# globc/mrAudio

Hardware: AMD Instinct MI355X
Metric: clips/s encode+fuse+score, 32-clip x 32-frame synthetic (higher is better)
Workload: dtype f16

## Files before the change

include/mra.h:

```cpp
#ifndef MRA_H_
#define MRA_H_

#include <stddef.h>
#include <stdint.h>

#ifdef __cplusplus
extern "C" {
#endif

#define MRA_OK 0
#define MRA_EINVAL (-1)
#define MRA_ESTATE (-2)
#define MRA_EHIP (-3)
#define MRA_ENOMEM (-4)
#define MRA_ENAME (-5)

#define MRA_F32 0
#define MRA_F16 1
#define MRA_BF16 2

typedef struct mra_qformer mra_qformer;

typedef struct mra_cfg {
  int32_t hidden;
// ... 112 lines not shown
typedef struct mra_vit_cfg {
  int32_t dim;
  int32_t heads;
  int32_t mlp;
  int32_t depth;
  int32_t patch;
  int32_t img;
  float ln_eps;
  int32_t op_dtype;
  int32_t residual_dtype;
} mra_vit_cfg;
void mra_vit_cfg_default(mra_vit_cfg* cfg);
int mra_vit_create(const mra_vit_cfg* cfg, mra_vit** out);
void mra_vit_destroy(mra_vit* h);
int mra_vit_load(mra_vit* h, const char* name, const void* src, int32_t dtype, const int64_t* shape, int32_t ndim, void* stream);
int mra_vit_missing(mra_vit* h);
size_t mra_vit_workspace_bytes(mra_vit* h, int32_t frames);
int mra_vit_forward(mra_vit* h, const void* frames, int32_t dtype, int32_t n, void* out, void* workspace, size_t workspace_bytes,
                    void* stream);
double mra_vit_flops(mra_vit* h, int32_t frames);
int mra_vit_set_option(mra_vit* h, const char* name, int32_t value);

#define MRA_BEATS_GATE_Q 0
#define MRA_BEATS_GATE_INPUT 1
typedef struct mra_beats mra_beats;
typedef struct mra_beats_cfg {
  int32_t dim;
  int32_t heads;
  int32_t ffn;
  int32_t layers;
  int32_t embed_dim;
  int32_t patch;
  int32_t mel_bins;
  int32_t conv_pos;
  int32_t conv_pos_groups;
  int32_t num_buckets;
  int32_t max_distance;
  float ln_eps;
  float deep_norm_alpha;
  int32_t gate_from;
  int32_t op_dtype;
} mra_beats_cfg;
void mra_beats_cfg_default(mra_beats_cfg* cfg);
int mra_beats_create(const mra_beats_cfg* cfg, mra_beats** out);
void mra_beats_destroy(mra_beats* h);
int mra_beats_load(mra_beats* h, const char* name, const void* src, int32_t dtype, const int64_t* shape, int32_t ndim, void* stream);
int mra_beats_missing(mra_beats* h);
size_t mra_beats_workspace_bytes(mra_beats* h, int32_t n, int32_t frames);
int mra_beats_forward(mra_beats* h, const void* fbank, int32_t dtype, int32_t n, int32_t frames, void* out, void* workspace,
                      size_t workspace_bytes, void* stream);
double mra_beats_flops(mra_beats* h, int32_t n, int32_t frames);
int mra_beats_set_option(mra_beats* h, const char* name, int32_t value);

typedef struct mra_fbank mra_fbank;
int mra_fbank_create(mra_fbank** out);
void mra_fbank_destroy(mra_fbank* h);
int mra_fbank_forward(mra_fbank* h, const float* wave, int64_t total_samples, const int64_t* segs, int32_t n_seg, int32_t frame_length,
                      void* out, int32_t out_dtype, void* stream);
double mra_fbank_flops(mra_fbank* h, int32_t n_seg, int32_t frame_length);

int64_t mra_debug_gemm_launches(int32_t family, int32_t epilogue);

int mra_debug_vit_attention(mra_vit* h, const void* qkv, int32_t n, void* ctx, void* stream);
size_t mra_debug_shared_kv_workspace_bytes(int32_t enc_items, int32_t prompts, int32_t heads, int32_t kv, int32_t core);
int mra_debug_shared_kv_attention(const void* q, const void* k, const void* v, int32_t dtype, int32_t enc_items, int32_t prompts,
                                  int32_t heads, int32_t kv, int32_t core, void* ctx, void* workspace, size_t workspace_bytes, void* stream);
int mra_debug_beats_attention(mra_beats* h, int32_t layer, const void* qkv, const void* gate_src, int32_t n, int32_t tokens, void* ctx,
                              void* stream);
int mra_debug_beats_posconv(mra_beats* h, float* x, int32_t n, int32_t tokens, void* stream);
int mra_debug_attention_bwd(const void* q, const void* k, const void* v, const void* o, const void* d_o, const float* lse, int32_t dtype,
                            int32_t kv_items, int32_t share, int32_t heads, int32_t q_rows, int32_t kv, void* dq, void* dk, void* dv, void* stream);

int mra_debug_self_attention(const void* qkv, const int64_t* mask, int32_t dtype, int32_t items, int32_t S, int32_t heads, void* ctx, float* lse,
                             void* stream);
int mra_debug_ln_rows(const float* x, const int64_t* x_view, int32_t rows, int32_t H, const float* const* params, int32_t lane_rows, int32_t period,
                      int32_t split, float eps, float* y32, const int64_t* y32_view, void* y16, const int64_t* y16_view, int32_t dtype, void* stream);
int mra_debug_embed_ln(const int64_t* ids, int32_t items, int32_t L, int32_t Q, int32_t H, int32_t vocab, const float* query, int64_t query_item_stride,
                       const float* word, const float* pos, const float* gain, const float* bias, float eps, float* h32, void* h16, float* pre32,
                       int32_t dtype, void* stream);
int mra_debug_modality_ln(const void* x, int32_t x_dtype, const int64_t* item_index, int32_t items, int32_t tokens, int32_t E, const float* gain,
                          const float* bias, float eps, void* out, int32_t dtype, void* stream);
int mra_debug_softmax_rows(const float* S, int64_t ld_s, void* P, int64_t ld_p, int32_t rows, int32_t kv, int32_t kvp, float scale, int32_t dtype,
                           void* stream);
int mra_debug_fold_rowfactor(const float* stat_m, const float* stat_l, float* factors, int32_t rows, int32_t R, int32_t ntiles, void* P, int64_t ld_p,
                             int32_t tile_cols, int32_t kvp, int32_t* hist, void* stream);
int mra_debug_softmax_rescale(void* P, int64_t ld_p, const float* stat_m, const float* stat_l, int32_t rows, int32_t ntiles, int32_t tile_cols,
                              int32_t kvp, int32_t dtype, int32_t* hist, void* stream);
int mra_debug_transpose_pad(const void* src, void* dst, int32_t R, int32_t C, int32_t ld_d, int64_t src_bs, int64_t dst_bs, int32_t batch, int32_t dtype,
                            void* stream);
int mra_debug_split(int32_t kind, const float* src, const int64_t* src_view, int32_t rows, int32_t C, int32_t chunk, int32_t parts, void* dst,
                    int32_t dtype, void* stream);

int mra_debug_gemm_tn_group(int32_t njobs, const void* const* dY, const int64_t* y_views, const int64_t* y_block_stride, const void* const* X,
                            const int64_t* x_views, const int64_t* x_block_stride, float* const* dW, float* const* db, const int32_t* M,
                            const int32_t* N, const int32_t* K, const int32_t* ldw, const int32_t* accumulate, int32_t dtype, void* stream);
int mra_debug_ln_bwd(const void* const* ptrs_a, const int64_t* views_a, int32_t rows_a, float eps_a, const void* const* ptrs_b, const int64_t* views_b,
                     int32_t rows_b, float eps_b, int32_t H, int32_t dtype, void* stream);
int mra_debug_embed_bwd(const float* demb, const int64_t* ids, int32_t items, int32_t L, int32_t Q, int32_t H, int32_t vocab, float* dquery, float* dpos,
                        float* dword, void* stream);
size_t mra_debug_transpose16_batch_scratch_bytes(int32_t njobs);
int mra_debug_transpose16_batch(const void* const* src, void* const* dst, const int32_t* R, const int32_t* C, int32_t njobs, int32_t dtype, void* scratch,
                                size_t scratch_bytes, void* stream);
int mra_debug_gemm_gelu(int32_t nprob, const void* const* A, const int64_t* a_views, const void* const* W, const float* const* bias, void* const* C,
                        const int64_t* c_views, void* const* aux, const int32_t* M, const int32_t* N, const int32_t* K, int32_t backward, int32_t tile_cfg,
                        int32_t dtype, void* stream);

typedef struct mra_gemm_desc {
  uint64_t struct_bytes;
  const void* A; const void* W; const float* bias; void* C; const float* R;
  int64_t a_view[3], c_view[3], r_view[3];
  int32_t M, N, K;
  int32_t kv_tokens, kv_items, kv_heads;
  int32_t batch, bias_bs;
  int64_t a_bs, w_bs, c_bs_bytes;
  int32_t n_ragged, w_ld, k_rows, w_kwrap;
  const float* ln_gain; const float* ln_bias; float* ln_y32; void* ln_y16; uint32_t* ln_counter;
  int64_t ln_y32_view[3], ln_y16_view[3];
  float ln_eps, alpha;
  float* stat_m; float* stat_l; const float* pscale;
  int32_t ps_ntiles, tile_cfg, persist, reserved;
  uint64_t a_bytes, w_bytes, bias_bytes, c_bytes, r_bytes, ln_gain_bytes, ln_bias_bytes, ln_y32_bytes, ln_y16_bytes, ln_counter_bytes, stat_m_bytes,
      stat_l_bytes, pscale_bytes;
  float* col_scale; int64_t cs_bs; int32_t col_stats; float cs_eps;
  uint64_t col_scale_bytes;
  void* aux; uint64_t aux_bytes;
} mra_gemm_desc;
int mra_debug_gemm(const mra_gemm_desc* probs, int32_t nprob, int32_t epilogue, int32_t dtype, void* stream);
int mra_debug_gemm_plan(const mra_gemm_desc* probs, int32_t nprob, int32_t epilogue, int32_t dtype, int32_t cus, int32_t* out);

int mra_debug_vit_fold_weight(const void* W, size_t w_bytes, const float* gain, size_t gain_bytes, const float* beta, size_t beta_bytes, const float* bias,
                              size_t bias_bytes, void* Wf, size_t wf_bytes, float* cs, size_t cs_bytes, float* bf, size_t bf_bytes, int32_t N, int32_t K,
                              int32_t dtype, void* stream);
int mra_debug_vit_group_stats(const float* groups, size_t groups_bytes, int64_t M, int32_t G, int32_t group_cols, float eps, float* stats,
                              size_t stats_bytes, void* stream);
int mra_debug_vit_row_stats(const void* x, size_t x_bytes, int32_t x_dtype, int64_t M, int32_t D, float eps, float* stats, size_t stats_bytes, void* x16,
                            size_t x16_bytes, int32_t dtype, void* stream);

#ifdef __cplusplus
}
#endif
#endif
```

mraudio_amd/_lib.py:

```python
from __future__ import annotations

import ctypes as C
import os

import torch

MRA_F32, MRA_F16, MRA_BF16 = 0, 1, 2
_ERR = {-1: "MRA_EINVAL", -2: "MRA_ESTATE", -3: "MRA_EHIP", -4: "MRA_ENOMEM", -5: "MRA_ENAME"}

LIB_NAME = "libmra_hip.so"
LIB_PATH = os.path.join(os.path.dirname(os.path.abspath(__file__)), LIB_NAME)


class mra_cfg(C.Structure):
    _fields_ = [
        ("hidden", C.c_int32), ("heads", C.c_int32), ("inter", C.c_int32), ("layers", C.c_int32),
        ("cross_freq", C.c_int32), ("enc_width", C.c_int32), ("n_query", C.c_int32), ("vocab", C.c_int32),
        ("max_pos", C.c_int32), ("ln_eps", C.c_float), ("enc_ln_eps", C.c_float), ("llm_hidden", C.c_int32),
        ("op_dtype", C.c_int32),
    ]


class mra_vit_cfg(C.Structure):
    _fields_ = [("dim", C.c_int32), ("heads", C.c_int32), ("mlp", C.c_int32), ("depth", C.c_int32), ("patch", C.c_int32),
                ("img", C.c_int32), ("ln_eps", C.c_float), ("op_dtype", C.c_int32), ("residual_dtype", C.c_int32)]


MRA_BEATS_GATE_Q, MRA_BEATS_GATE_INPUT = 0, 1


class mra_beats_cfg(C.Structure):
    _fields_ = [("dim", C.c_int32), ("heads", C.c_int32), ("ffn", C.c_int32), ("layers", C.c_int32), ("embed_dim", C.c_int32),
                ("patch", C.c_int32), ("mel_bins", C.c_int32), ("conv_pos", C.c_int32), ("conv_pos_groups", C.c_int32),
                ("num_buckets", C.c_int32), ("max_distance", C.c_int32), ("ln_eps", C.c_float), ("deep_norm_alpha", C.c_float),
                ("gate_from", C.c_int32), ("op_dtype", C.c_int32)]


class mra_gemm_desc(C.Structure):
    _fields_ = [
        ("struct_bytes", C.c_uint64),
        ("A", C.c_void_p), ("W", C.c_void_p), ("bias", C.c_void_p), ("C", C.c_void_p), ("R", C.c_void_p),
        ("a_view", C.c_int64 * 3), ("c_view", C.c_int64 * 3), ("r_view", C.c_int64 * 3),
        ("M", C.c_int32), ("N", C.c_int32), ("K", C.c_int32),
        ("kv_tokens", C.c_int32), ("kv_items", C.c_int32), ("kv_heads", C.c_int32),
        ("batch", C.c_int32), ("bias_bs", C.c_int32),
        ("a_bs", C.c_int64), ("w_bs", C.c_int64), ("c_bs_bytes", C.c_int64),
        ("n_ragged", C.c_int32), ("w_ld", C.c_int32), ("k_rows", C.c_int32), ("w_kwrap", C.c_int32),
        ("ln_gain", C.c_void_p), ("ln_bias", C.c_void_p), ("ln_y32", C.c_void_p), ("ln_y16", C.c_void_p), ("ln_counter", C.c_void_p),
        ("ln_y32_view", C.c_int64 * 3), ("ln_y16_view", C.c_int64 * 3),
        ("ln_eps", C.c_float), ("alpha", C.c_float),
        ("stat_m", C.c_void_p), ("stat_l", C.c_void_p), ("pscale", C.c_void_p),
        ("ps_ntiles", C.c_int32), ("tile_cfg", C.c_int32), ("persist", C.c_int32), ("reserved", C.c_int32),
        ("a_bytes", C.c_uint64), ("w_bytes", C.c_uint64), ("bias_bytes", C.c_uint64), ("c_bytes", C.c_uint64), ("r_bytes", C.c_uint64),
        ("ln_gain_bytes", C.c_uint64), ("ln_bias_bytes", C.c_uint64), ("ln_y32_bytes", C.c_uint64), ("ln_y16_bytes", C.c_uint64),
        ("ln_counter_bytes", C.c_uint64), ("stat_m_bytes", C.c_uint64), ("stat_l_bytes", C.c_uint64), ("pscale_bytes", C.c_uint64),
        ("col_scale", C.c_void_p), ("cs_bs", C.c_int64), ("col_stats", C.c_int32), ("cs_eps", C.c_float),
        ("col_scale_bytes", C.c_uint64),
        ("aux", C.c_void_p), ("aux_bytes", C.c_uint64),
    ]


PROTOTYPES = {
    "mra_cfg_default": (None, [C.POINTER(mra_cfg), C.c_int32]),
    "mra_last_error": (C.c_char_p, []),
    "mra_version": (C.c_char_p, []),
    "mra_qformer_create": (C.c_int, [C.POINTER(mra_cfg), C.POINTER(C.c_void_p)]),
    "mra_qformer_destroy": (None, [C.c_void_p]),
    "mra_qformer_load": (C.c_int, [C.c_void_p, C.c_char_p, C.c_void_p, C.c_int32, C.POINTER(C.c_int64), C.c_int32,
                                   C.c_void_p]),
    "mra_qformer_missing": (C.c_int, [C.c_void_p, C.c_char_p, C.c_size_t]),
    "mra_modality_ln": (C.c_int, [C.c_void_p, C.c_void_p, C.c_int32, C.c_void_p, C.c_int32, C.c_int32, C.c_void_p,
                                  C.c_void_p]),
    "mra_qformer_workspace_bytes": (C.c_size_t, [C.c_void_p, C.c_int32, C.c_int32, C.c_int32]),
    "mra_qformer_forward": (C.c_int, [C.c_void_p, C.c_void_p, C.c_void_p, C.c_void_p, C.c_int32, C.c_void_p, C.c_int32,
                                      C.c_int32, C.c_int32, C.c_void_p, C.c_void_p, C.c_void_p, C.c_void_p, C.c_size_t,
                                      C.c_void_p]),
    "mra_qformer_raw_features_ok": (C.c_int, [C.c_void_p, C.c_int32, C.c_int32]),
    "mra_qformer_forward_raw": (C.c_int, [C.c_void_p, C.c_void_p, C.c_void_p, C.c_void_p, C.c_int32, C.c_void_p, C.c_int32,
                                          C.c_int32, C.c_int32, C.c_void_p, C.c_void_p, C.c_void_p, C.c_void_p, C.c_size_t,
                                          C.c_void_p]),
    "mra_qformer_pair_workspace_bytes": (C.c_size_t, [C.c_void_p, C.c_void_p, C.c_int32, C.c_int32, C.c_int32, C.c_int32]),
    "mra_qformer_forward_pair": (C.c_int, [C.c_void_p, C.c_void_p, C.c_void_p, C.c_void_p, C.c_void_p, C.c_void_p, C.c_int32, C.c_int32, C.c_int32, C.c_int32,
                                           C.c_void_p, C.c_void_p, C.c_void_p, C.c_void_p, C.c_void_p, C.c_size_t, C.c_void_p]),
    "mra_qformer_forward_pair_raw": (C.c_int, [C.c_void_p, C.c_void_p, C.c_void_p, C.c_void_p, C.c_void_p, C.c_void_p, C.c_int32, C.c_int32, C.c_int32, C.c_int32,
                                               C.c_int32, C.c_void_p, C.c_void_p, C.c_void_p, C.c_void_p, C.c_void_p, C.c_size_t, C.c_void_p]),
    "mra_qformer_multi_workspace_bytes": (C.c_size_t, [C.c_void_p, C.c_int32, C.c_int32, C.c_int32, C.c_int32]),
    "mra_qformer_forward_multi": (C.c_int, [C.c_void_p, C.c_void_p, C.c_void_p, C.c_void_p, C.c_int32, C.c_int32, C.c_int32, C.c_int32,
                                            C.c_void_p, C.c_void_p, C.c_void_p, C.c_size_t, C.c_void_p]),
    "mra_qformer_set_kv_events": (C.c_int, [C.c_void_p, C.c_void_p, C.c_void_p]),
    "mra_qformer_set_kv_done_event": (C.c_int, [C.c_void_p, C.c_void_p]),
    "mra_qformer_set_cross_mode": (C.c_int, [C.c_void_p, C.c_int32]),
    "mra_qformer_set_cross_precision": (C.c_int, [C.c_void_p, C.c_int32]),
    "mra_qformer_cross_precision_report": (C.c_int, [C.c_void_p, C.POINTER(C.c_int32), C.POINTER(C.c_int32), C.POINTER(C.c_float), C.c_int32]),
    "mra_qformer_set_option": (C.c_int, [C.c_void_p, C.c_char_p, C.c_int32]),
    "mra_qformer_prepare": (C.c_int, [C.c_void_p, C.c_void_p]),
    "mra_kv_cache_bytes": (C.c_size_t, [C.c_void_p, C.c_int32, C.c_int32]),
    "mra_kv_project": (C.c_int, [C.c_void_p, C.c_void_p, C.c_int32, C.c_int32, C.c_void_p, C.c_void_p]),
    "mra_llm_proj": (C.c_int, [C.c_void_p, C.c_void_p, C.c_int32, C.c_void_p, C.c_int32, C.c_void_p, C.c_size_t,
                               C.c_void_p]),
    "mra_cosine_score": (C.c_int, [C.c_void_p, C.c_void_p, C.c_int32, C.c_int32, C.c_int32, C.c_int32, C.c_void_p,
                                   C.c_void_p, C.c_void_p]),
    "mra_fuse_logits": (C.c_int, [C.POINTER(C.c_void_p), C.POINTER(C.c_float), C.c_int32, C.c_int32, C.c_void_p,
                                  C.c_void_p]),
    "mra_span_from_logits": (C.c_int, [C.c_void_p, C.c_int32, C.c_int32, C.c_float, C.c_void_p, C.c_void_p]),
    "mra_windows_from_logits": (C.c_int, [C.c_void_p, C.c_int32, C.c_int32, C.c_float, C.c_int32, C.c_float, C.c_int32, C.c_void_p,
                                          C.c_void_p, C.c_void_p, C.c_void_p]),
    "mra_qformer_grad_bytes": (C.c_size_t, [C.c_void_p]),
    "mra_qformer_load_flat": (C.c_int32, [C.c_void_p, C.c_void_p, C.c_size_t, C.c_void_p]),
    "mra_qformer_grad_offset": (C.c_int, [C.c_void_p, C.c_char_p, C.POINTER(C.c_size_t), C.POINTER(C.c_int64)]),
    "mra_qformer_enable_training": (C.c_int, [C.c_void_p, C.c_void_p]),
    "mra_qformer_adam_step": (C.c_int, [C.c_void_p, C.c_void_p, C.c_void_p, C.c_void_p, C.c_void_p, C.c_size_t, C.c_float, C.c_float, C.c_float,
                                        C.c_float, C.c_float, C.c_int32, C.c_int32, C.c_void_p]),
    "mra_qformer_train_workspace_bytes": (C.c_size_t, [C.c_void_p, C.c_int32, C.c_int32, C.c_int32]),
    "mra_qformer_forward_train": (C.c_int, [C.c_void_p, C.c_void_p, C.c_void_p, C.c_void_p, C.c_int32, C.c_int32, C.c_int32,
                                            C.c_void_p, C.c_void_p, C.c_void_p, C.c_size_t, C.c_void_p]),
    "mra_qformer_backward": (C.c_int, [C.c_void_p, C.c_void_p, C.c_void_p, C.c_void_p, C.c_int32, C.c_int32, C.c_int32,
                                       C.c_void_p, C.c_void_p, C.c_void_p, C.c_void_p, C.c_size_t, C.c_void_p]),
    "mra_qformer_multi_train_workspace_bytes": (C.c_size_t, [C.c_void_p, C.c_int32, C.c_int32, C.c_int32, C.c_int32]),
    "mra_qformer_forward_multi_train": (C.c_int, [C.c_void_p, C.c_void_p, C.c_void_p, C.c_void_p, C.c_int32, C.c_int32, C.c_int32, C.c_int32,
                                                  C.c_void_p, C.c_void_p, C.c_void_p, C.c_size_t, C.c_void_p]),
    "mra_qformer_backward_multi": (C.c_int, [C.c_void_p, C.c_void_p, C.c_void_p, C.c_void_p, C.c_int32, C.c_int32, C.c_int32, C.c_int32,
                                             C.c_void_p, C.c_void_p, C.c_void_p, C.c_void_p, C.c_size_t, C.c_void_p]),
    "mra_qformer_backward_enc": (C.c_int, [C.c_void_p, C.c_int32, C.c_int32, C.c_int32, C.c_int32, C.c_void_p, C.c_size_t, C.c_void_p, C.c_void_p]),
    "mra_modality_ln_backward": (C.c_int, [C.c_void_p, C.c_void_p, C.c_int32, C.c_int32, C.c_int32, C.c_void_p, C.c_void_p, C.c_void_p, C.c_void_p,
                                           C.c_void_p]),
    "mra_debug_kvgrad_gemm": (C.c_int, [C.c_void_p, C.c_void_p, C.c_size_t, C.c_int32, C.c_int32, C.c_void_p, C.c_size_t, C.c_void_p]),
    "mra_qformer_flops": (C.c_double, [C.c_void_p, C.c_int32, C.c_int32, C.c_int32, C.c_int32]),
    "mra_vit_cfg_default": (None, [C.POINTER(mra_vit_cfg)]),
    "mra_vit_create": (C.c_int, [C.POINTER(mra_vit_cfg), C.POINTER(C.c_void_p)]),
    "mra_vit_destroy": (None, [C.c_void_p]),
    "mra_vit_load": (C.c_int, [C.c_void_p, C.c_char_p, C.c_void_p, C.c_int32, C.POINTER(C.c_int64), C.c_int32, C.c_void_p]),
    "mra_vit_missing": (C.c_int, [C.c_void_p]),
    "mra_vit_workspace_bytes": (C.c_size_t, [C.c_void_p, C.c_int32]),
    "mra_vit_forward": (C.c_int, [C.c_void_p, C.c_void_p, C.c_int32, C.c_int32, C.c_void_p, C.c_void_p, C.c_size_t, C.c_void_p]),
    "mra_vit_flops": (C.c_double, [C.c_void_p, C.c_int32]),
    "mra_vit_set_option": (C.c_int, [C.c_void_p, C.c_char_p, C.c_int32]),
    "mra_beats_cfg_default": (None, [C.POINTER(mra_beats_cfg)]),
    "mra_beats_create": (C.c_int, [C.POINTER(mra_beats_cfg), C.POINTER(C.c_void_p)]),
    "mra_beats_destroy": (None, [C.c_void_p]),
    "mra_beats_load": (C.c_int, [C.c_void_p, C.c_char_p, C.c_void_p, C.c_int32, C.POINTER(C.c_int64), C.c_int32, C.c_void_p]),
    "mra_beats_missing": (C.c_int, [C.c_void_p]),
    "mra_beats_workspace_bytes": (C.c_size_t, [C.c_void_p, C.c_int32, C.c_int32]),
    "mra_beats_forward": (C.c_int, [C.c_void_p, C.c_void_p, C.c_int32, C.c_int32, C.c_int32, C.c_void_p, C.c_void_p, C.c_size_t, C.c_void_p]),
    "mra_beats_flops": (C.c_double, [C.c_void_p, C.c_int32, C.c_int32]),
    "mra_beats_set_option": (C.c_int, [C.c_void_p, C.c_char_p, C.c_int32]),
    "mra_fbank_create": (C.c_int, [C.POINTER(C.c_void_p)]),
    "mra_fbank_destroy": (None, [C.c_void_p]),
    "mra_fbank_forward": (C.c_int, [C.c_void_p, C.c_void_p, C.c_int64, C.c_void_p, C.c_int32, C.c_int32, C.c_void_p, C.c_int32, C.c_void_p]),
    "mra_fbank_flops": (C.c_double, [C.c_void_p, C.c_int32, C.c_int32]),
    "mra_debug_gemm_launches": (C.c_int64, [C.c_int32, C.c_int32]),
    "mra_debug_vit_attention": (C.c_int, [C.c_void_p, C.c_void_p, C.c_int32, C.c_void_p, C.c_void_p]),
    "mra_debug_shared_kv_workspace_bytes": (C.c_size_t, [C.c_int32, C.c_int32, C.c_int32, C.c_int32, C.c_int32]),
    "mra_debug_shared_kv_attention": (C.c_int, [C.c_void_p, C.c_void_p, C.c_void_p, C.c_int32, C.c_int32, C.c_int32, C.c_int32, C.c_int32, C.c_int32,
                                                C.c_void_p, C.c_void_p, C.c_size_t, C.c_void_p]),
    "mra_debug_attention_bwd": (C.c_int, [C.c_void_p, C.c_void_p, C.c_void_p, C.c_void_p, C.c_void_p, C.c_void_p, C.c_int32, C.c_int32, C.c_int32,
                                          C.c_int32, C.c_int32, C.c_int32, C.c_void_p, C.c_void_p, C.c_void_p, C.c_void_p]),
    "mra_debug_beats_attention": (C.c_int, [C.c_void_p, C.c_int32, C.c_void_p, C.c_void_p, C.c_int32, C.c_int32, C.c_void_p, C.c_void_p]),
    "mra_debug_beats_posconv": (C.c_int, [C.c_void_p, C.c_void_p, C.c_int32, C.c_int32, C.c_void_p]),
    "mra_debug_self_attention": (C.c_int, [C.c_void_p, C.c_void_p, C.c_int32, C.c_int32, C.c_int32, C.c_int32, C.c_void_p, C.c_void_p, C.c_void_p]),
    "mra_debug_ln_rows": (C.c_int, [C.c_void_p, C.POINTER(C.c_int64), C.c_int32, C.c_int32, C.POINTER(C.c_void_p), C.c_int32, C.c_int32, C.c_int32,
                                    C.c_float, C.c_void_p, C.POINTER(C.c_int64), C.c_void_p, C.POINTER(C.c_int64), C.c_int32, C.c_void_p]),
    "mra_debug_embed_ln": (C.c_int, [C.c_void_p, C.c_int32, C.c_int32, C.c_int32, C.c_int32, C.c_int32, C.c_void_p, C.c_int64, C.c_void_p, C.c_void_p,
                                     C.c_void_p, C.c_void_p, C.c_float, C.c_void_p, C.c_void_p, C.c_void_p, C.c_int32, C.c_void_p]),
    "mra_debug_modality_ln": (C.c_int, [C.c_void_p, C.c_int32, C.c_void_p, C.c_int32, C.c_int32, C.c_int32, C.c_void_p, C.c_void_p, C.c_float,
                                        C.c_void_p, C.c_int32, C.c_void_p]),
    "mra_debug_softmax_rows": (C.c_int, [C.c_void_p, C.c_int64, C.c_void_p, C.c_int64, C.c_int32, C.c_int32, C.c_int32, C.c_float, C.c_int32,
                                         C.c_void_p]),
    "mra_debug_fold_rowfactor": (C.c_int, [C.c_void_p, C.c_void_p, C.c_void_p, C.c_int32, C.c_int32, C.c_int32, C.c_void_p, C.c_int64, C.c_int32,
                                           C.c_int32, C.c_void_p, C.c_void_p]),
    "mra_debug_softmax_rescale": (C.c_int, [C.c_void_p, C.c_int64, C.c_void_p, C.c_void_p, C.c_int32, C.c_int32, C.c_int32, C.c_int32, C.c_int32,
                                            C.c_void_p, C.c_void_p]),
    "mra_debug_transpose_pad": (C.c_int, [C.c_void_p, C.c_void_p, C.c_int32, C.c_int32, C.c_int32, C.c_int64, C.c_int64, C.c_int32, C.c_int32,
                                          C.c_void_p]),
    "mra_debug_split": (C.c_int, [C.c_int32, C.c_void_p, C.POINTER(C.c_int64), C.c_int32, C.c_int32, C.c_int32, C.c_int32, C.c_void_p, C.c_int32,
                                  C.c_void_p]),
    "mra_debug_gemm_tn_group": (C.c_int, [C.c_int32, C.POINTER(C.c_void_p), C.POINTER(C.c_int64), C.POINTER(C.c_int64), C.POINTER(C.c_void_p),
                                          C.POINTER(C.c_int64), C.POINTER(C.c_int64), C.POINTER(C.c_void_p), C.POINTER(C.c_void_p), C.POINTER(C.c_int32),
                                          C.POINTER(C.c_int32), C.POINTER(C.c_int32), C.POINTER(C.c_int32), C.POINTER(C.c_int32), C.c_int32, C.c_void_p]),
    "mra_debug_ln_bwd": (C.c_int, [C.POINTER(C.c_void_p), C.POINTER(C.c_int64), C.c_int32, C.c_float, C.POINTER(C.c_void_p), C.POINTER(C.c_int64),
                                   C.c_int32, C.c_float, C.c_int32, C.c_int32, C.c_void_p]),
    "mra_debug_embed_bwd": (C.c_int, [C.c_void_p, C.c_void_p, C.c_int32, C.c_int32, C.c_int32, C.c_int32, C.c_int32, C.c_void_p, C.c_void_p, C.c_void_p,
                                      C.c_void_p]),
    "mra_debug_transpose16_batch_scratch_bytes": (C.c_size_t, [C.c_int32]),
    "mra_debug_transpose16_batch": (C.c_int, [C.POINTER(C.c_void_p), C.POINTER(C.c_void_p), C.POINTER(C.c_int32), C.POINTER(C.c_int32), C.c_int32,
                                              C.c_int32, C.c_void_p, C.c_size_t, C.c_void_p]),
    "mra_debug_gemm_gelu": (C.c_int, [C.c_int32, C.POINTER(C.c_void_p), C.POINTER(C.c_int64), C.POINTER(C.c_void_p), C.POINTER(C.c_void_p),
                                      C.POINTER(C.c_void_p), C.POINTER(C.c_int64), C.POINTER(C.c_void_p), C.POINTER(C.c_int32), C.POINTER(C.c_int32),
                                      C.POINTER(C.c_int32), C.c_int32, C.c_int32, C.c_int32, C.c_void_p]),
    "mra_debug_gemm": (C.c_int, [C.POINTER(mra_gemm_desc), C.c_int32, C.c_int32, C.c_int32, C.c_void_p]),
    "mra_debug_gemm_plan": (C.c_int, [C.POINTER(mra_gemm_desc), C.c_int32, C.c_int32, C.c_int32, C.c_int32, C.POINTER(C.c_int32)]),
    "mra_debug_vit_fold_weight": (C.c_int, [C.c_void_p, C.c_size_t, C.c_void_p, C.c_size_t, C.c_void_p, C.c_size_t, C.c_void_p, C.c_size_t, C.c_void_p,
                                            C.c_size_t, C.c_void_p, C.c_size_t, C.c_void_p, C.c_size_t, C.c_int32, C.c_int32, C.c_int32, C.c_void_p]),
    "mra_debug_vit_group_stats": (C.c_int, [C.c_void_p, C.c_size_t, C.c_int64, C.c_int32, C.c_int32, C.c_float, C.c_void_p, C.c_size_t, C.c_void_p]),
    "mra_debug_vit_row_stats": (C.c_int, [C.c_void_p, C.c_size_t, C.c_int32, C.c_int64, C.c_int32, C.c_float, C.c_void_p, C.c_size_t, C.c_void_p,
                                          C.c_size_t, C.c_int32, C.c_void_p]),
}

GF_V1_64, GF_V1_128, GF_WS_256, GF_P8_256, GF_WS_128x384, GF_WS_176x384, GF_K128_64x128, GF_P8_TAIL, GF_P8_MIXED, GF_K128_64x64 = 0, 1, 3, 4, 5, 6, 7, 8, 9, 10
GF_RING_144x128, GF_RING_192x128, GF_RING_96x64 = 11, 12, 13
GEMM_FAMILIES = 14
EPI_OP, EPI_GELU_OP, EPI_RES_F32, EPI_F32, EPI_KV, EPI_SOFTPART, EPI_RES_OP = 0, 1, 2, 3, 4, 5, 8
EPI_RES_F32_STAT, EPI_LNF_OP, EPI_LNF_GELU_OP, EPI_RES_OP_STAT = 10, 11, 12, 13
EPI_GELU_BOTH, EPI_GELU_BWD = 6, 7
EPI_RES_LN = 9
GT_AUTO, GT_64, GT_128, GT_256 = 0, 1, 2, 3
GT_WS_128x384, GT_WS_176x384, GT_K128_64x128, GT_P8_TAIL, GT_P8_MIXED = 4, 5, 6, 7, 8
GT_RING_144x128, GT_RING_192x128, GT_RING_96x64 = 9, 10, 11
GEMM_TN_MAX_JOBS = 4


def gemm_launches(family: int, epi: int) -> int:
    return int(lib().mra_debug_gemm_launches(family, epi))

_lib = None


class MraError(RuntimeError):
    pass


def lib() -> C.CDLL:
    global _lib
    if _lib is None:
        if not os.path.exists(LIB_PATH):
            raise MraError(
                f"{LIB_PATH} is missing: build the HIP extension first "
                "(python -c 'import __graft_entry__ as g; g.build()' or make -C mraudio_amd/csrc). "
                "mraudio_amd has no CPU fallback."
            )
        handle = C.CDLL(LIB_PATH)
        for name, (res, args) in PROTOTYPES.items():
            fn = getattr(handle, name)
            fn.restype = res
            fn.argtypes = args
        _lib = handle
    return _lib


def check(rc: int, what: str) -> None:
    if rc != 0:
        msg = lib().mra_last_error().decode("utf-8", "replace")
        raise MraError(f"{what}: {_ERR.get(rc, rc)}: {msg}")


def ptr(t) -> C.c_void_p:
    return C.c_void_p(0 if t is None else t.data_ptr())


def current_stream() -> C.c_void_p:
    return C.c_void_p(torch.cuda.current_stream().cuda_stream)
# ... 15 lines not shown
```

mraudio_amd/csrc/fold.hip:

```cpp
#include "kernels.h"
#include "mra_common.h"

namespace mra {

namespace {

constexpr float LOG2E_F = 1.4426950408889634f;

template <typename T, int NV>
__global__ void __launch_bounds__(256) softmax_rows_kernel(const float* S, long long ld_s, T* P, long long ld_p, int kv, int kvp,
                                                           float sl2) {
  __shared__ float red[8];
  const int tid = threadIdx.x, lane = tid & 63, wave = tid >> 6;
  const float* s = S + (long long)blockIdx.x * ld_s;
  T* p = P + (long long)blockIdx.x * ld_p;
  constexpr int NR = NV > 0 ? NV : 1;
  f32x4 v[NR];
  float m = -3.0e38f;
  if constexpr (NV > 0) {
#pragma unroll
    for (int j = 0; j < NV; ++j) {
      const int c = 4 * (tid + j * 256);
      if (c + 3 < kv) {
        v[j] = *reinterpret_cast<const f32x4*>(s + c);
      } else {
#pragma unroll
        for (int e = 0; e < 4; ++e) v[j][e] = c + e < kv ? s[c + e] : -3.0e38f;
      }
      m = fmaxf(fmaxf(m, fmaxf(v[j][0], v[j][1])), fmaxf(v[j][2], v[j][3]));
    }
  } else {
    for (int i = tid; i < kv; i += 256) m = fmaxf(m, s[i]);
  }
  m = wave_max(m);
  if (lane == 0) red[wave] = m;
  __syncthreads();
  m = fmaxf(fmaxf(red[0], red[1]), fmaxf(red[2], red[3])) * sl2;
  float l = 0.f;
  if constexpr (NV > 0) {
#pragma unroll
    for (int j = 0; j < NV; ++j)
#pragma unroll
      for (int e = 0; e < 4; ++e) {
        v[j][e] = __builtin_amdgcn_exp2f(v[j][e] * sl2 - m);
        l += v[j][e];
      }
  } else {
    for (int i = tid; i < kv; i += 256) l += __builtin_amdgcn_exp2f(s[i] * sl2 - m);
  }
  l = wave_sum(l);
  if (lane == 0) red[4 + wave] = l;
  __syncthreads();
  const float inv = 1.0f / ((red[4] + red[5]) + (red[6] + red[7]));
  if constexpr (NV > 0) {
#pragma unroll
    for (int j = 0; j < NV; ++j) {
      const int c = 4 * (tid + j * 256);
      if (c < kvp) {
        typename Vec4<T>::type o;
#pragma unroll
        for (int e = 0; e < 4; ++e) o[e] = from_f32<T>(v[j][e] * inv);
        *reinterpret_cast<typename Vec4<T>::type*>(p + c) = o;
      }
    }
  } else {
    for (int i = tid; i < kvp; i += 256) p[i] = from_f32<T>(i < kv ? __builtin_amdgcn_exp2f(s[i] * sl2 - m) * inv : 0.f);
  }
}

template <typename T, bool PROBE>
__global__ void __launch_bounds__(256) softmax_rescale_kernel(T* P, long long ld_p, const float* stat_m, const float* stat_l, int ntiles,
                                                              int tile_cols, int kvp, int* hist) {
  __shared__ float g[128];
  const int tid = threadIdx.x;
  const float* sm = stat_m + (long long)blockIdx.x * ntiles;
  const float* sl = stat_l + (long long)blockIdx.x * ntiles;
  if (tid < 64) {
    float m = -3.0e38f;
    for (int t = tid; t < ntiles; t += 64) m = fmaxf(m, sm[t]);
    m = wave_max(m);
    float l = 0.f;
    for (int t = tid; t < ntiles; t += 64) l += __builtin_amdgcn_exp2f(sm[t] - m) * sl[t];
// ... 23 lines not shown
    *reinterpret_cast<V8*>(p + 8 * c) = v;
  }
}

template <bool PROBE>
__global__ void __launch_bounds__(256) fold_rowfactor_kernel(const float* stat_m, const float* stat_l, float* factors, int rows, int R, int ntiles,
                                                             unsigned short* P, long long ld_p, int tile_cols, int kvp, int* hist) {
  const int row = blockIdx.x * 4 + (threadIdx.x >> 6), lane = threadIdx.x & 63;
  __shared__ int bins[PROBE ? 256 : 1];
  if constexpr (PROBE) {
    bins[threadIdx.x] = 0;
    __syncthreads();
  }
  if (row < rows) {
    for (int c = ntiles * tile_cols + lane; c < kvp; c += 64) P[(long long)row * ld_p + c] = 0;
    const float* sm = stat_m + (long long)row * ntiles;
    const float* sl = stat_l + (long long)row * ntiles;
    float m = -3.0e38f;
    for (int t = lane; t < ntiles; t += 64) m = fmaxf(m, sm[t]);
    m = wave_max(m);
    float l = 0.f;
    for (int t = lane; t < ntiles; t += 64) l += __builtin_amdgcn_exp2f(sm[t] - m) * sl[t];
    l = wave_sum(l);
    const float inv = 1.0f / l;
    const int item = row / R, r = row - item * R;
    for (int t = lane; t < ntiles; t += 64) factors[((long long)item * ntiles + t) * 512 + r] = __builtin_amdgcn_exp2f(sm[t] - m) * inv;
    if constexpr (PROBE) {
      if (lane == 0) atomicAdd(&bins[(int)fminf(fmaxf(inv * 256.f, 0.f), 255.f)], 1);
    }
  }
  if constexpr (PROBE) {
    __syncthreads();
    const int n = bins[threadIdx.x];
    if (n) atomicAdd(hist + threadIdx.x, n);
  }
}

template <typename T>
__global__ void __launch_bounds__(256) transpose_pad_kernel(const T* src, T* dst, int R, int C, int ld_d, long long src_bs,
                                                            long long dst_bs) {
  __shared__ T tile[32][33];
  src += (long long)blockIdx.z * src_bs;
  dst += (long long)blockIdx.z * dst_bs;
  const int bx = blockIdx.x * 32, by = blockIdx.y * 32;
  const int tx = threadIdx.x & 31, ty = threadIdx.x >> 5;
  for (int j = ty; j < 32; j += 8)
    tile[j][tx] = (by + j < R && bx + tx < C) ? src[(long long)(by + j) * C + bx + tx] : from_f32<T>(0.f);
  __syncthreads();
  for (int j = ty; j < 32; j += 8)
    if (bx + j < C && by + tx < ld_d) dst[(long long)(bx + j) * ld_d + by + tx] = tile[tx][j];
}

template <typename T>
__global__ void __launch_bounds__(256) transpose_pad64_kernel(const T* src, T* dst, int R, int C, int ld_d, long long src_bs,
                                                              long long dst_bs) {
  __shared__ T tile[64][72];
  src += (long long)blockIdx.z * src_bs;
  dst += (long long)blockIdx.z * dst_bs;
  const int bx = blockIdx.x * 64, by = blockIdx.y * 64;
  const int ch = (threadIdx.x & 7) * 8, r0 = threadIdx.x >> 3;
  using V8 = typename Vec8<T>::type;
#pragma unroll
  for (int i = 0; i < 2; ++i) {
    const int r = r0 + 32 * i;
    V8 v;
#pragma unroll
    for (int e = 0; e < 8; ++e) v[e] = from_f32<T>(0.f);
    if (by + r < R && bx + ch < C) v = *reinterpret_cast<const V8*>(src + (long long)(by + r) * C + bx + ch);
    *reinterpret_cast<V8*>(&tile[r][ch]) = v;
  }
  __syncthreads();
#pragma unroll
  for (int i = 0; i < 2; ++i) {
    const int c = r0 + 32 * i;
    if (bx + c < C && by + ch < ld_d) {
      V8 v;
#pragma unroll
      for (int e = 0; e < 8; ++e) v[e] = tile[ch + e][c];
      *reinterpret_cast<V8*>(dst + (long long)(bx + c) * ld_d + by + ch) = v;
    }
  }
}

}

int launch_softmax_rows(const float* S, long long ld_s, void* P, long long ld_p, int rows, int kv, int kvp, float scale, int op_dtype,
                        hipStream_t stream) {
  if (rows <= 0) return 0;
  if (kv <= 0 || kvp < kv || (kvp & 3) || (ld_s & 3) || (ld_p & 3) || ld_p < kvp || ld_s < kv) return -1;
  const float sl2 = scale * LOG2E_F;
  const int nv = (kvp + 1023) / 1024;
#define MRA_SM(T, NV) hipLaunchKernelGGL((softmax_rows_kernel<T, NV>), dim3(rows), dim3(256), 0, stream, S, ld_s, (T*)P, ld_p, kv, kvp, sl2)
#define MRA_SM_T(T)                                                                                   \
  do {                                                                                                \
    if (nv <= 1) MRA_SM(T, 1); else if (nv <= 2) MRA_SM(T, 2); else if (nv <= 4) MRA_SM(T, 4);          \
    else if (nv <= 9) MRA_SM(T, 9); else if (nv <= 16) MRA_SM(T, 16); else MRA_SM(T, 0);               \
  } while (0)
  if (op_dtype == OP_F16) MRA_SM_T(f16); else MRA_SM_T(bf16);
#undef MRA_SM_T
#undef MRA_SM
  return hipGetLastError() == hipSuccess ? 0 : -4;
}

int launch_fold_rowfactor(const float* stat_m, const float* stat_l, float* factors, int rows, int R, int ntiles, void* P, long long ld_p, int tile_cols,
                          int kvp, hipStream_t stream, int* hist) {
  if (rows <= 0) return 0;
  if (ntiles <= 0 || R <= 0 || R > 512 || rows % R || !P || ld_p < kvp || ntiles * tile_cols > kvp) return -1;
  if (hist)
    hipLaunchKernelGGL(fold_rowfactor_kernel<true>, dim3((rows + 3) / 4), dim3(256), 0, stream, stat_m, stat_l, factors, rows, R, ntiles,
                       (unsigned short*)P, ld_p, tile_cols, kvp, hist);
  else
    hipLaunchKernelGGL(fold_rowfactor_kernel<false>, dim3((rows + 3) / 4), dim3(256), 0, stream, stat_m, stat_l, factors, rows, R, ntiles,
                       (unsigned short*)P, ld_p, tile_cols, kvp, (int*)nullptr);
  return hipGetLastError() == hipSuccess ? 0 : -4;
}

int launch_softmax_rescale(void* P, long long ld_p, const float* stat_m, const float* stat_l, int rows, int ntiles, int tile_cols, int kvp,
                           int op_dtype, hipStream_t stream, int* hist) {
  if (rows <= 0) return 0;
  if (ntiles <= 0 || ntiles > 128 || (tile_cols & 7) || (kvp & 7) || (ld_p & 7) || ld_p < kvp) return -1;
#define MRA_RS(T, PR) hipLaunchKernelGGL((softmax_rescale_kernel<T, PR>), dim3(rows), dim3(256), 0, stream, (T*)P, ld_p, stat_m, stat_l, ntiles, tile_cols, kvp, hist)
  if (op_dtype == OP_F16) { if (hist) MRA_RS(f16, true); else MRA_RS(f16, false); }
  else { if (hist) MRA_RS(bf16, true); else MRA_RS(bf16, false); }
#undef MRA_RS
  return hipGetLastError() == hipSuccess ? 0 : -4;
}

int launch_transpose_pad(const void* src, void* dst, int R, int C, int ld_d, long long src_bs, long long dst_bs, int batch, int op_dtype,
                         hipStream_t stream) {
  if (batch <= 0 || R <= 0 || C <= 0) return 0;
  if (ld_d < R || batch > 65535) return -1;
  if (C % 8 == 0 && ld_d % 8 == 0 && C >= 64 && ld_d >= 64) {
    const dim3 grid64((C + 63) / 64, (ld_d + 63) / 64, batch);
    if (op_dtype == OP_F16) hipLaunchKernelGGL(transpose_pad64_kernel<f16>, grid64, dim3(256), 0, stream, (const f16*)src, (f16*)dst, R, C, ld_d, src_bs, dst_bs);
    else hipLaunchKernelGGL(transpose_pad64_kernel<bf16>, grid64, dim3(256), 0, stream, (const bf16*)src, (bf16*)dst, R, C, ld_d, src_bs, dst_bs);
    return hipGetLastError() == hipSuccess ? 0 : -4;
  }
  const dim3 grid((C + 31) / 32, (ld_d + 31) / 32, batch), block(256);
  if (op_dtype == OP_F16) hipLaunchKernelGGL(transpose_pad_kernel<f16>, grid, block, 0, stream, (const f16*)src, (f16*)dst, R, C, ld_d, src_bs, dst_bs);
  else hipLaunchKernelGGL(transpose_pad_kernel<bf16>, grid, block, 0, stream, (const bf16*)src, (bf16*)dst, R, C, ld_d, src_bs, dst_bs);
  return hipGetLastError() == hipSuccess ? 0 : -4;
}

namespace {
template <typename T, typename TW, bool KEY>
__global__ void __launch_bounds__(256) fold_ln_weight_kernel(const TW* W, int E, const float* gain, const float* ln_bias, const float* bias_in,
                                                             T* dst, float* bias_out) {
  __shared__ float red[8];
  const int tid = threadIdx.x, lane = tid & 63, wave = tid >> 6;
  const int n = blockIdx.x;
  const TW* w = W + (long long)n * E;
  float s = 0.f, sb = 0.f;
  for (int e = tid; e < E; e += 256) {
    const float we = (float)w[e];
    s += we * gain[e];
    sb = __builtin_fmaf(we, ln_bias[e], sb);
  }
  s = wave_sum(s);
  sb = wave_sum(sb);
  if (lane == 0) { red[wave] = s; red[4 + wave] = sb; }
  __syncthreads();
  const float mean = ((red[0] + red[1]) + (red[2] + red[3])) / (float)E;
  if (tid == 0 && bias_out) bias_out[n] = (bias_in ? bias_in[n] : 0.f) + ((red[4] + red[5]) + (red[6] + red[7]));
  for (int e = tid; e < E; e += 256) {
    const T o = from_f32<T>((float)w[e] * gain[e] - mean);
    if (KEY) dst[((long long)(n >> 6) * E + e) * 64 + (n & 63)] = o;
    else dst[(long long)n * E + e] = o;
  }
}
}

int launch_fold_ln_weight(const void* W, int w32, int rows, int E, const float* gain, const float* ln_bias, const float* bias_in, void* dst,
                          int key_layout, float* bias_out, int op_dtype, hipStream_t stream) {
  if (rows <= 0 || E <= 0 || !W || !gain || !ln_bias || !dst || (key_layout && rows % 64)) return -1;
#define MRA_FL(T, TW, KEY) hipLaunchKernelGGL((fold_ln_weight_kernel<T, TW, KEY>), dim3(rows), dim3(256), 0, stream, (const TW*)W, E, gain, ln_bias, bias_in, (T*)dst, bias_out)
#define MRA_FL_T(T)                                                          \
  do {                                                                       \
    if (w32) { if (key_layout) MRA_FL(T, float, true); else MRA_FL(T, float, false); } \
    else { if (key_layout) MRA_FL(T, T, true); else MRA_FL(T, T, false); }   \
  } while (0)
  if (op_dtype == OP_F16) MRA_FL_T(f16); else MRA_FL_T(bf16);
#undef MRA_FL_T
#undef MRA_FL
  return hipGetLastError() == hipSuccess ? 0 : -4;
}

}
```

mraudio_amd/csrc/gemm.hip:

```cpp
#include <atomic>
#include <cstdlib>
#include <initializer_list>
#include <mutex>
#include <set>
#include <type_traits>
#include <utility>

#include "kernels.h"
#include "mra_common.h"

namespace mra {

namespace {

__device__ __forceinline__ long long view_off(const RowView& v, int m) {
  int item = m / v.rpi;
  int r = m - item * v.rpi;
  return (long long)item * v.item_stride + (long long)r * v.ld;
}

template <int TN, int TM>
__device__ __forceinline__ GemmProb tile_of(const GemmArgs& args, int id, int& n0, int& m0);

template <int TN, int TM>
// ... 475 lines not shown
  constexpr int NT = WGN * WGM * 64;
  constexpr int WTN = TN / WGN, WTM = TM / WGM;
  constexpr int FN = WTN / 16, FM = WTM / 16;
  constexpr int IW = TN * 8 / NT, IX = TM * 8 / NT;
  static_assert(TN * 8 % NT == 0 && TM * 8 % NT == 0, "tile/threads mismatch");
  constexpr int BUF = (TN + TM) * ROWB;
  extern __shared__ __attribute__((aligned(16))) char smem[];
  const int tid = threadIdx.x;
  const int lane = tid & 63;
  const int wave = __builtin_amdgcn_readfirstlane(tid >> 6);
  const int wn0 = (wave / WGM) * WTN;
  const int wm0 = (wave % WGM) * WTM;
  int n0, m0;
  const GemmProb& P = pick_tile<TN, TM>(args, n0, m0);
  const int K = P.K, M = P.M;

  const char* srcW[IW];
  const char* srcX[IX];
#pragma unroll
  for (int i = 0; i < IW; ++i) {
    const int q = tid + i * NT;
    const int row = q >> 3, c = (q & 7) ^ ((row >> 1) & 7);
    srcW[i] = (const char*)P.W + ((long long)min(n0 + row, P.N - 1) * K + c * 8) * 2;
  }
#pragma unroll
  for (int i = 0; i < IX; ++i) {
    const int q = tid + i * NT;
    const int row = q >> 3, c = (q & 7) ^ ((row >> 1) & 7);
    const int m = min(m0 + row, M - 1);
    srcX[i] = (const char*)P.A + (view_off(P.a, m) + c * 8) * 2;
  }
  const int wave_q0 = wave * 64;
  auto stage = [&](int buf, int kt) {
    char* base = smem + buf * BUF;
    const long long koff = (long long)kt * ROWB;
#pragma unroll
    for (int i = 0; i < IW; ++i) glds16(srcW[i] + koff, base + (wave_q0 + i * NT) * 16);
#pragma unroll
    for (int i = 0; i < IX; ++i) glds16(srcX[i] + koff, base + TN * ROWB + (wave_q0 + i * NT) * 16);
  };
  int foff[2];
#pragma unroll
  for (int ks = 0; ks < 2; ++ks) {
    const int r = lane & 15;
    const int c = (4 * ks + (lane >> 4)) ^ ((r >> 1) & 7);
    foff[ks] = r * ROWB + c * 16;
  }
  f32x4 acc[FN][FM];
#pragma unroll
  for (int i = 0; i < FN; ++i)
#pragma unroll
    for (int j = 0; j < FM; ++j) acc[i][j] = f32x4{0.f, 0.f, 0.f, 0.f};

  const int nk = K / BK;
  stage(0, 0);
  for (int kt = 0; kt < nk; ++kt) {
    asm volatile("s_waitcnt vmcnt(0)" ::: "memory");
    __syncthreads();
    if (kt + 1 < nk) stage((kt + 1) & 1, kt + 1);
    const char* wb = smem + (kt & 1) * BUF + wn0 * ROWB;
    const char* xb = smem + (kt & 1) * BUF + TN * ROWB + wm0 * ROWB;
#pragma unroll
    for (int ks = 0; ks < 2; ++ks) {
      typename Vec8<T>::type a[FN], b[FM];
#pragma unroll
      for (int i = 0; i < FN; ++i) a[i] = lds_read8<T>(wb + i * 16 * ROWB + foff[ks]);
#pragma unroll
      for (int j = 0; j < FM; ++j) b[j] = lds_read8<T>(xb + j * 16 * ROWB + foff[ks]);
#pragma unroll
      for (int i = 0; i < FN; ++i)
#pragma unroll
        for (int j = 0; j < FM; ++j) acc[i][j] = mfma16<T>(a[i], b[j], acc[i][j]);
    }
  }
  if constexpr (EPI == EPI_OP || EPI == EPI_GELU_OP || EPI == EPI_KV || EPI == EPI_RES_OP) {
    __syncthreads();
    epilogue_lds16<T, TN, TM, FN, FM, NT, EPI, (FN * FM <= 16)>(P, acc, smem, n0, m0, wn0, wm0, tid);
  } else {
    if constexpr (FN * FM > 16) epilogue_lean<T, FN, FM, EPI>(P, acc, n0 + wn0, m0 + wm0, lane);
    else epilogue<T, FN, FM, EPI>(P, acc, n0 + wn0, m0 + wm0, lane);
  }
}

template <typename T, int EPI, bool NODMA = false, int TN = 256, int TM = 256, int WGM = 4, bool NTW = false, bool WKM = false, bool PSC = false, int CS = 0>
__global__ void __launch_bounds__(768) gemm_ws_kernel(const GemmArgs args) {
  constexpr int BK = 64, ROWB = BK * 2;
  constexpr int WGN = 8 / WGM, WTN = TN / WGN, WTM = TM / WGM, FN = WTN / 16, FM = WTM / 16;
  constexpr int BUF = (TN + TM) * ROWB;
  constexpr int PS_TILE = 176, GT_OFF = 2 * BUF, GT_SLICE = 2048;
  static_assert(!PSC || (TM <= 512 && PS_TILE % 8 == 0), "factor slices hold 512 rows; an 8-k fragment piece never straddles a tile");
  constexpr int NCHUNK = (TN + TM) * 8, NLD = (NCHUNK + 255) / 256;
  constexpr bool STAGED = (EPI == EPI_OP || EPI == EPI_GELU_OP || EPI == EPI_KV || EPI == EPI_RES_OP) && TN % 64 == 0;
  static_assert(WTN % 16 == 0 && WTM % 16 == 0 && TN % 16 == 0 && NCHUNK % 64 == 0, "tile must split over the waves; whole waves per DMA piece");
  static_assert(CS == 0 || (EPI == EPI_SOFTPART && !WKM && !PSC && TN * 4 <= BUF && TN <= 192), "column factors: the scores launch only; three per lane of one wave");
  constexpr int NWS = (TN * 8 + 255) / 256;
  extern __shared__ __attribute__((aligned(16))) char smem[];
  const int tid = threadIdx.x;
  const int lane = tid & 63;
  const int wave = __builtin_amdgcn_readfirstlane(tid >> 6);
  int n0, m0;
  const GemmProb& P = pick_tile<TN, TM>(args, n0, m0);
  const int K = P.K, M = P.M;
  const int nk = K / BK;

  if (wave >= 8) {
    const int lt = tid - 512;
    const char* src[NLD];
    int wrow[NLD];
#pragma unroll
    for (int i = 0; i < NLD; ++i) {
      const int q = min(lt + i * 256, NCHUNK - 1);
      const int row = q >> 3, c = (q & 7) ^ ((row >> 1) & 7);
      wrow[i] = 0;
      if (WKM && q < TN * 8) {
        wrow[i] = q / (TN / 8);
        src[i] = (const char*)P.W + ((long long)n0 + (q - wrow[i] * (TN / 8)) * 8) * 2;
      } else if (row < TN) {
        const long long ldw = P.w_kwrap > 0 ? (long long)P.w_kwrap * BK : K;
        src[i] = (const char*)P.W + ((long long)min(n0 + row, P.N - 1) * ldw + c * 8) * 2;
      } else {
        const int m = min(m0 + row - TN, M - 1);
        src[i] = (const char*)P.A + (view_off(P.a, m) + c * 8) * 2;
      }
    }
    const int wq0 = (wave - 8) * 64;
    const int kwrap = P.w_kwrap > 0 ? P.w_kwrap : 0x7fffffff;
    auto stage = [&](int buf, int kt) {
      char* base = smem + buf * BUF;
      const long long koff = (long long)kt * ROWB;
      const long long koffw = (long long)(kt >= kwrap ? kt - kwrap : kt) * ROWB;
#pragma unroll
      for (int i = 0; i < NLD; ++i)
        if (i * 256 + wq0 < NCHUNK) {
          if (WKM && i * 256 + wq0 < TN * 8) {
            const long long krow = min(kt * BK + wrow[i], P.k_rows - 1);
            glds16_nt(src[i] + krow * P.w_ld * 2, base + (wq0 + i * 256) * 16);
          } else if ((i * 256 + wq0) / 8 < TN) {
            if (NTW) glds16_nt(src[i] + koffw, base + (wq0 + i * 256) * 16);
            else glds16(src[i] + koffw, base + (wq0 + i * 256) * 16);
          } else {
            glds16(src[i] + koff, base + (wq0 + i * 256) * 16);
          }
        }
    };
    int gt_next = 0;
    auto stage_factors = [&](int kt) {
      if constexpr (PSC) {
        if (wave != 8) return;
        const int t_hi = (kt * BK + BK - 1) / PS_TILE;
        for (; gt_next <= t_hi; ++gt_next) {
          const char* sg = (const char*)(P.pscale + (long long)min(gt_next, P.ps_ntiles - 1) * 512) + lane * 16;
          char* dg = smem + GT_OFF + (gt_next & 3) * GT_SLICE;
          glds16(sg, dg);
          glds16(sg + 1024, dg + 1024);
        }
      }
    };
    float* const cscale = CS != 0 ? P.col_scale + (long long)(P.batch_row0 / M) * P.cs_bs : nullptr;
    float csv[3] = {0.f, 0.f, 0.f};
    if constexpr (CS == 1) {
      if (wave == 8) {
#pragma unroll
        for (int k = 0; k < 3; ++k) csv[k] = cscale[min(n0 + min(lane + 64 * k, TN - 1), P.N - 1)];
      }
    }
    float cmean[NWS], cm2[NWS];
#pragma unroll
    for (int i = 0; i < NWS; ++i) cmean[i] = cm2[i] = 0.f;
    stage(0, 0);
    stage_factors(0);
    for (int kt = 0; kt < nk; ++kt) {
      asm volatile("s_waitcnt vmcnt(0)" ::: "memory");
      __builtin_amdgcn_s_barrier();
      asm volatile("" ::: "memory");
      if (kt + 1 < nk && !(NODMA && kt >= 1)) { stage((kt + 1) & 1, kt + 1); stage_factors(kt + 1); }
      if constexpr (CS == 2) {
        const unsigned cb = (unsigned)(size_t)(__attribute__((address_space(3))) char*)smem + (kt & 1) * BUF + lt * 16;
        i32x4 raw[NWS];
#pragma unroll
        for (int i = 0; i < NWS; ++i)
          if (i * 256 + wq0 < TN * 8) asm volatile("ds_read_b128 %0, %1 offset:%2" : "=v"(raw[i]) : "v"(cb), "n"(i * 4096) : "memory");
        const float fk = 1.0f / (float)(kt + 1), fq = 8.0f * (float)kt * fk;
#pragma unroll
        for (int i = 0; i < NWS; ++i)
          if (i * 256 + wq0 < TN * 8) {
            asm volatile("s_waitcnt lgkmcnt(0)" : "+v"(raw[i])::"memory");
            const typename Vec8<T>::type v = __builtin_bit_cast(typename Vec8<T>::type, raw[i]);
            float x[8], sum = 0.f;
#pragma unroll
            for (int e = 0; e < 8; ++e) { x[e] = (float)v[e]; sum += x[e]; }
            const float m8 = sum * 0.125f;
            float q8 = 0.f;
#pragma unroll
            for (int e = 0; e < 8; ++e) { const float d = x[e] - m8; q8 = __builtin_fmaf(d, d, q8); }
            const float dl = m8 - cmean[i];
            cmean[i] = __builtin_fmaf(dl, fk, cmean[i]);
            cm2[i] = cm2[i] + q8 + dl * dl * fq;
          }
      }
    }
    if constexpr (CS != 0) {
      float* scol = reinterpret_cast<float*>(smem + (nk & 1) * BUF);
      if constexpr (CS == 2) {
        float cnt = 8.0f * (float)nk;
#pragma unroll
        for (int sw = 1; sw < 8; sw <<= 1) {
#pragma unroll
          for (int i = 0; i < NWS; ++i) {
            const float om = __shfl_xor(cmean[i], sw), oq = __shfl_xor(cm2[i], sw);
            const float dl = om - cmean[i];
            cmean[i] = __builtin_fmaf(dl, 0.5f, cmean[i]);
            cm2[i] = cm2[i] + oq + dl * dl * (0.5f * cnt);
          }
          cnt *= 2.0f;
        }
#pragma unroll
        for (int i = 0; i < NWS; ++i)
          if (i * 256 + wq0 < TN * 8 && (lane & 7) == 0) scol[(lt + i * 256) >> 3] = 1.0f / __builtin_sqrtf(cm2[i] / cnt + P.cs_eps);
      } else if (wave == 8) {
#pragma unroll
        for (int k = 0; k < 3; ++k)
          if (lane + 64 * k < TN) scol[lane + 64 * k] = csv[k];
      }
      __syncthreads();
      if constexpr (CS == 2) {
        if (wave == 8) {
#pragma unroll
          for (int k = 0; k < 3; ++k)
            if (lane + 64 * k < TN && n0 + lane + 64 * k < P.N) cscale[n0 + lane + 64 * k] = scol[lane + 64 * k];
        }
      }
    }
    if constexpr (STAGED) {
      __syncthreads();
      __syncthreads();
    }
    return;
  }

  const int wn0 = (wave / WGM) * WTN;
  const int wm0 = (wave % WGM) * WTM;
  int foff[2];
#pragma unroll
  for (int ks = 0; ks < 2; ++ks) {
    const int r = lane & 15;
    const int c = (4 * ks + (lane >> 4)) ^ ((r >> 1) & 7);
    foff[ks] = r * ROWB + c * 16;
  }
  const unsigned wtr = (unsigned)(size_t)(__attribute__((address_space(3))) char*)smem +
                       (8 * (lane >> 4) + ((lane & 15) >> 2)) * (TN * 2) + (lane & 3) * 8;
  static_assert(!WKM || WGN == 1, "K-major weights: one column of compute waves");
  f32x4 acc[FN][FM];
  if constexpr (EPI == EPI_RES_F32) {
    accumulators_from_residual<FN, FM>(P, acc, n0 + wn0, m0 + wm0, lane);
  } else {
#pragma unroll
    for (int i = 0; i < FN; ++i)
#pragma unroll
      for (int j = 0; j < FM; ++j) acc[i][j] = f32x4{0.f, 0.f, 0.f, 0.f};
  }

  for (int kt = 0; kt < nk; ++kt) {
    __builtin_amdgcn_s_barrier();
    asm volatile("" ::: "memory");
    const char* wb = smem + (kt & 1) * BUF + wn0 * ROWB;
    const char* xb = smem + (kt & 1) * BUF + TN * ROWB + wm0 * ROWB;
#pragma unroll
    for (int ks = 0; ks < 2; ++ks) {
      typename Vec8<T>::type b[FM];
#pragma unroll
      for (int j = 0; j < FM; ++j) b[j] = lds_read8<T>(xb + j * 16 * ROWB + foff[ks]);
      if constexpr (PSC) {
        const int t = (kt * BK + ks * 32 + 8 * (lane >> 4)) / PS_TILE;
        const float* gt = reinterpret_cast<const float*>(smem + GT_OFF + (t & 3) * GT_SLICE) + wm0 + (lane & 15);
#pragma unroll
        for (int j = 0; j < FM; ++j) {
          const float gf = gt[j * 16];
          if constexpr (sizeof(T) == 2 && __is_same(T, f16)) {
            b[j] = b[j] * (f16)gf;
          } else {
#pragma unroll
            for (int e = 0; e < 8; ++e) b[j][e] = from_f32<T>((float)b[j][e] * gf);
          }
        }
      }
      if constexpr (WKM) {
        constexpr int WP = TN * 2;
        const unsigned tb = wtr + (kt & 1) * BUF + ks * 32 * WP;
        i16x4 f[2][2];
        asm volatile("ds_read_b64_tr_b16 %0, %2\n\tds_read_b64_tr_b16 %1, %2 offset:%3" : "=&v"(f[0][0]), "=&v"(f[0][1]) : "v"(tb), "n"(4 * WP) : "memory");
        static_assert(FN * 32 + 4 * WP < 65536, "fragment offsets must fit the ds_read offset field");
#pragma unroll
        for (int i = 0; i < FN; ++i) {
          if (i + 1 < FN) {
            asm volatile("ds_read_b64_tr_b16 %0, %2 offset:%3\n\tds_read_b64_tr_b16 %1, %2 offset:%4"
                         : "=&v"(f[(i + 1) & 1][0]), "=&v"(f[(i + 1) & 1][1]) : "v"(tb), "n"((i + 1) * 32), "n"((i + 1) * 32 + 4 * WP) : "memory");
            asm volatile("s_waitcnt lgkmcnt(2)" : "+v"(f[i & 1][0]), "+v"(f[i & 1][1])::"memory");
          } else {
            asm volatile("s_waitcnt lgkmcnt(0)" : "+v"(f[i & 1][0]), "+v"(f[i & 1][1])::"memory");
          }
          const i16x4 c0 = f[i & 1][0], c1 = f[i & 1][1];
          i16x8 v;
          v[0] = c0[0]; v[1] = c0[1]; v[2] = c0[2]; v[3] = c0[3]; v[4] = c1[0]; v[5] = c1[1]; v[6] = c1[2]; v[7] = c1[3];
          const typename Vec8<T>::type a_cur = __builtin_bit_cast(typename Vec8<T>::type, v);
#pragma unroll
          for (int j = 0; j < FM; ++j) acc[i][j] = mfma16<T>(a_cur, b[j], acc[i][j]);
        }
      } else {
      typename Vec8<T>::type a_cur = lds_read8<T>(wb + foff[ks]);
#pragma unroll
      for (int i = 0; i < FN; ++i) {
        typename Vec8<T>::type a_nxt = a_cur;
        if (i + 1 < FN) a_nxt = lds_read8<T>(wb + (i + 1) * 16 * ROWB + foff[ks]);
#pragma unroll
        for (int j = 0; j < FM; ++j) acc[i][j] = mfma16<T>(a_cur, b[j], acc[i][j]);
        a_cur = a_nxt;
      }
      }
    }
  }
  if constexpr (EPI == EPI_SOFTPART) {
    static_assert(EPI != EPI_SOFTPART || WGN == 1, "the softmax-partial epilogue needs whole tile rows in one wave");
    if constexpr (CS != 0) {
      __syncthreads();
      epilogue_softpart<T, FN, FM, true>(P, acc, n0, m0 + wm0, n0 / TN, P.batch_row0, lane, reinterpret_cast<const float*>(smem + (nk & 1) * BUF));
    } else {
    epilogue_softpart<T, FN, FM>(P, acc, n0, m0 + wm0, n0 / TN, P.batch_row0, lane);
    }
  } else if constexpr (STAGED) {
    __syncthreads();
    epilogue_lds16<T, TN, TM, FN, FM, 512, EPI>(P, acc, smem, n0, m0, wn0, wm0, tid);
  } else {
    epilogue_lean<T, FN, FM, EPI, EPI == EPI_RES_F32>(P, acc, n0 + wn0, m0 + wm0, lane);
  }
}

template <typename T, int EPI, bool TAIL>
__device__ __forceinline__ void gemm_p8_tile(const GemmProb& P, int n0, int m0, unsigned long long* dbg = nullptr) {
  constexpr int TN = TAIL ? 128 : 256, TM = TAIL ? 512 : 256, BK = 64, ROWB = BK * 2, WTN = 128, WTM = 64, FN = 8, FM = 4;
  constexpr int WHALF = (TAIL ? 64 : 128) * ROWB, XHALF = (TAIL ? 256 : 128) * ROWB;
  constexpr int BUF = 2 * WHALF + 2 * XHALF;
  constexpr int WP = WHALF / 8192, XP = XHALF / 8192;
  constexpr bool STAGED = EPI == EPI_OP || EPI == EPI_GELU_OP || EPI == EPI_KV || EPI == EPI_RES_OP || EPI == EPI_RES_OP_STAT || EPI == EPI_LNF_OP || EPI == EPI_LNF_GELU_OP;
  constexpr bool RESF32 = EPI == EPI_RES_F32 || EPI == EPI_RES_F32_STAT;
// ... 619 lines not shown
constexpr bool has_epi(unsigned mask, int epi) { return epi >= 0 && epi < 16 && (mask >> epi & 1); }
template <int... E, typename F>
int with_epi(Epis<E...>, int epi, F&& f) {
  int rc = -2;
  (void)((epi == E && ((rc = f(std::integral_constant<int, E>{})), true)) || ...);
  return rc;
}
using EpiDirect = Epis<EPI_OP, EPI_GELU_OP, EPI_RES_F32, EPI_F32, EPI_KV, EPI_GELU_BOTH, EPI_GELU_BWD, EPI_RES_OP>;
#ifdef MRA_GEMM_EXPERIMENTS
using EpiV1_256 = EpiDirect;
#else
using EpiV1_256 = Epis<>;
#endif
using EpiP8 = Epis<EPI_OP, EPI_GELU_OP, EPI_KV, EPI_RES_OP, EPI_RES_OP_STAT, EPI_RES_F32, EPI_RES_F32_STAT, EPI_LNF_OP, EPI_LNF_GELU_OP, EPI_F32>;
using EpiP8Persist = Epis<EPI_OP, EPI_GELU_OP, EPI_LNF_OP, EPI_LNF_GELU_OP, EPI_KV>;
using EpiP8Tail = Epis<EPI_RES_OP, EPI_RES_F32, EPI_F32>;
using EpiP8Mixed = Epis<EPI_OP, EPI_RES_OP, EPI_RES_OP_STAT, EPI_RES_F32, EPI_RES_F32_STAT, EPI_F32>;
using EpiWs128 = Epis<EPI_OP, EPI_F32>;
using EpiWs176 = Epis<EPI_F32, EPI_SOFTPART, EPI_OP>;
using EpiRing16 = Epis<EPI_OP, EPI_GELU_OP>;
using EpiRing96 = Epis<EPI_OP, EPI_GELU_OP, EPI_RES_F32, EPI_F32, EPI_RES_LN>;

template <int TN, int TM, int WGN, int WGM, int STAGES, int EPI>
constexpr bool ring_fits() {
  constexpr int osz = (EPI == EPI_RES_F32 || EPI == EPI_F32 || EPI == EPI_RES_LN) ? 4 : 2;
  return WGN * WGM * (TN / WGN / 16) * (TM / WGM / 16) * 1024 + TM * (TN * osz + 16) <= STAGES * (TN + TM) * 128 && STAGES * (TN + TM) * 128 <= 160 * 1024;
}
template <int TN, int TM, int WGN, int WGM, int STAGES, int... E>
constexpr bool ring_fits(Epis<E...>) { return (ring_fits<TN, TM, WGN, WGM, STAGES, E>() && ...); }
static_assert(ring_fits<144, 128, 1, 4, 4>(EpiRing16{}) && !ring_fits<144, 128, 1, 4, 4, EPI_F32>(), "ring 144 x 128");
static_assert(ring_fits<192, 128, 2, 2, 4>(EpiRing16{}) && !ring_fits<192, 128, 2, 2, 4, EPI_F32>(), "ring 192 x 128");
static_assert(ring_fits<96, 64, 2, 2, 7>(EpiRing96{}), "ring 96 x 64");

enum : unsigned {
  T_RAGGED = 1, T_MASK = 2, T_BATCH = 4, T_GROUPS = 8,
  T_WLD = 16, T_KWRAP = 32,
  T_F32_16B = 64,
  T_PLAIN = T_RAGGED | T_MASK | T_BATCH | T_GROUPS,
};
struct TileDesc {
  int tile;
  int tn, tm;
  int threads, lds;
  int kstep;
  unsigned allow;
  unsigned epis;
};
constexpr TileDesc kTiles[GEMM_FAMILIES] = {
     {GT_64, 64, 64, 256, 2 * (64 + 64) * 128, 64, T_PLAIN, epi_mask(EpiDirect{})},
     {GT_128, 128, 128, 256, 2 * (128 + 128) * 128, 64, T_PLAIN, epi_mask(EpiDirect{})},
     {GT_256, 256, 256, 512, 2 * (256 + 256) * 128, 64, T_PLAIN, epi_mask(EpiV1_256{})},
     {GT_256, 256, 256, 768, 2 * (256 + 256) * 128, 64, T_PLAIN, epi_mask(EpiDirect{})},
     {GT_256, 256, 256, 512, 2 * (256 + 256) * 128 + 8 * 256, 128, T_PLAIN, epi_mask(EpiP8{})},
     {GT_WS_128x384, 128, 384, 768, 2 * (128 + 384) * 128, 64, T_PLAIN | T_KWRAP, epi_mask(EpiWs128{})},
     {GT_WS_176x384, 176, 384, 768, 2 * (176 + 384) * 128, 64, T_PLAIN | T_KWRAP | T_WLD, epi_mask(EpiWs176{})},
     {GT_K128_64x128, 64, 128, 256, 2 * (64 + 128) * 256, 128, T_PLAIN, epi_mask(EpiDirect{})},
     {GT_P8_TAIL, 128, 512, 512, 2 * (128 + 512) * 128, 128, T_GROUPS, epi_mask(EpiP8Tail{})},
     {GT_P8_MIXED, 256, 256, 512, 2 * (128 + 512) * 128, 128, 0, epi_mask(EpiP8Mixed{})},
     {GT_64, 64, 64, 256, 2 * (64 + 64) * 256, 128, T_PLAIN, epi_mask(EpiDirect{})},
     {GT_RING_144x128, 144, 128, 512, 4 * (144 + 128) * 128, 64, T_GROUPS | T_F32_16B, epi_mask(EpiRing16{})},
     {GT_RING_192x128, 192, 128, 512, 4 * (192 + 128) * 128, 64, T_GROUPS | T_F32_16B, epi_mask(EpiRing16{})},
     {GT_RING_96x64, 96, 64, 512, 7 * (96 + 64) * 128, 64, T_GROUPS | T_F32_16B, epi_mask(EpiRing96{})},
};

#ifdef MRA_GEMM_EXPERIMENTS
#include "gemm_experiments.inc"
#endif

template <typename T>
int launch_family(const GemmPlan& pl, int epi, hipStream_t stream) {
  const GemmArgs& a = pl.args;
  auto go = [&](auto kfn) { return launch_k(kfn, a, pl.threads, pl.lds, stream, pl.grid); };
  switch (pl.family) {
    case GF_V1_64: return with_epi(EpiDirect{}, epi, [&](auto e) { return go(gemm_kernel<T, 64, 64, 2, 2, e()>); });
    case GF_V1_128: return with_epi(EpiDirect{}, epi, [&](auto e) { return go(gemm_kernel<T, 128, 128, 2, 2, e()>); });
    case GF_V1_256: return with_epi(EpiV1_256{}, epi, [&](auto e) { return go(gemm_kernel<T, 256, 256, 2, 4, e()>); });
    case GF_WS_256: return with_epi(EpiDirect{}, epi, [&](auto e) { return go(gemm_ws_kernel<T, e()>); });
    case GF_P8_256:
      if (pl.persistent) return with_epi(EpiP8Persist{}, epi, [&](auto e) { return go(gemm_p8_persist_kernel<T, e()>); });
      return with_epi(EpiP8{}, epi, [&](auto e) { return go(gemm_p8_kernel<T, e()>); });
    case GF_WS_128x384: return with_epi(EpiWs128{}, epi, [&](auto e) { return go(gemm_ws_kernel<T, e(), false, 128, 384>); });
    case GF_WS_176x384:
      if (a.p[0].w_ld > 0) {
        if (a.p[0].pscale) return go(gemm_ws_kernel<T, EPI_OP, false, 176, 384, 8, true, true, true>);
        return go(gemm_ws_kernel<T, EPI_OP, false, 176, 384, 8, true, true>);
      }
      if (a.p[0].col_scale) {
        if (a.p[0].col_stats) return go(gemm_ws_kernel<T, EPI_SOFTPART, false, 176, 384, 8, true, false, false, 2>);
        return go(gemm_ws_kernel<T, EPI_SOFTPART, false, 176, 384, 8, true, false, false, 1>);
      }
      return with_epi(EpiWs176{}, epi, [&](auto e) { return go(gemm_ws_kernel<T, e(), false, 176, 384, 8, true>); });
    case GF_K128_64x128: return with_epi(EpiDirect{}, epi, [&](auto e) { return go(gemm_k128_kernel<T, 64, 128, 2, 2, e()>); });
    case GF_P8_TAIL: return with_epi(EpiP8Tail{}, epi, [&](auto e) { return go(gemm_p8_kernel<T, e(), true>); });
    case GF_P8_MIXED: return with_epi(EpiP8Mixed{}, epi, [&](auto e) { return go(gemm_p8_mixed_kernel<T, e()>); });
    case GF_K128_64x64: return with_epi(EpiDirect{}, epi, [&](auto e) { return go(gemm_k128_kernel<T, 64, 64, 2, 2, e()>); });
    case GF_RING_144x128: return with_epi(EpiRing16{}, epi, [&](auto e) { return go(gemm_ring_kernel<T, 144, 128, 1, 4, 4, e()>); });
    case GF_RING_192x128: return with_epi(EpiRing16{}, epi, [&](auto e) { return go(gemm_ring_kernel<T, 192, 128, 2, 2, 4, e()>); });
    case GF_RING_96x64: return with_epi(EpiRing96{}, epi, [&](auto e) { return go(gemm_ring_kernel<T, 96, 64, 2, 2, 7, e()>); });
  }
  return -2;
}

template <typename T>
int launch_t(const GemmPlan& pl, int epi, hipStream_t stream) {
#ifdef MRA_GEMM_EXPERIMENTS
  int rc;
  if (g_variant != 5 && g_variant != 1 && pl.tile <= GT_256 && launch_experiment<T>(pl.args, pl.tile, epi, g_variant, stream, &rc)) return rc;
#endif
  return counted(pl.family, epi, launch_family<T>(pl, epi, stream));
}

int device_cus() {
  static std::atomic<int> memo[64];
  int dev = 0;
  if (hipGetDevice(&dev) != hipSuccess || dev < 0 || dev >= 64) return 0;
  int cus = memo[dev].load(std::memory_order_relaxed);
  if (!cus && hipDeviceGetAttribute(&cus, hipDeviceAttributeMultiprocessorCount, dev) == hipSuccess) memo[dev].store(cus, std::memory_order_relaxed);
  return cus;
}

int pick_tile(const GemmProb* probs, int ngroups) {
  if (g_force_tile > GT_AUTO) return g_force_tile;
  if (probs[0].tile_cfg > GT_AUTO) return probs[0].tile_cfg;
  for (int t : {256, 128}) {
    long long tiles = 0;
    bool ok = true;
    for (int g = 0; g < ngroups; ++g) {
      if (probs[g].N % t && !probs[g].n_ragged && !probs[g].n_mask) ok = false;
      tiles += (long long)((probs[g].M + t - 1) / t) * ((probs[g].N + t - 1) / t) * (probs[g].batch > 1 ? probs[g].batch : 1);
    }
    if (ok && tiles >= (t == 256 ? 512 : 384)) return t == 256 ? GT_256 : GT_128;
  }
  return GT_64;
}

int pick_family(int tile, const GemmProb* probs, int ngroups, int epi) {
  bool even = true, deep = true;
  for (int g = 0; g < ngroups; ++g) {
    even = even && probs[g].K % 128 == 0;
    deep = deep && probs[g].K % 128 == 0 && probs[g].K >= 2048;
  }
  if (tile == GT_256) {
    if (g_variant == 1) return GF_V1_256;
    return g_p8 && even && has_epi(kTiles[GF_P8_256].epis, epi) ? GF_P8_256 : GF_WS_256;
  }
  if (tile == GT_64 && g_variant != 1 && deep) return GF_K128_64x64;
  for (int f = 0; f < GEMM_FAMILIES; ++f)
    if (kTiles[f].tile == tile) return f;
  return -1;
}

inline bool misaligned(const RowView& v, int mask) { return (v.ld & mask) || (v.item_stride & mask); }

bool operand_rules(const GemmProb& p, int epi) {
  if (p.M <= 0 || p.N <= 0 || p.K <= 0 || p.K % 64 || p.batch < 0) return false;
  if (p.a.rpi <= 0 || (epi != EPI_KV && p.c.rpi <= 0)) return false;
  if ((epi == EPI_OP || epi == EPI_GELU_OP || epi == EPI_RES_OP) && misaligned(p.c, 7)) return false;
  if (p.n_ragged && (p.bias || p.n_mask)) return false;
  if (p.n_mask && (p.N & 3)) return false;
  return true;
}

bool epilogue_rules(const GemmProb& p, int ngroups, int epi) {
  const bool f32 = epi == EPI_RES_F32 || epi == EPI_F32;
  if (p.n_mask && !f32 && ((epi != EPI_RES_OP && epi != EPI_OP && epi != EPI_GELU_OP) || (p.N & 63))) return false;
  if (p.n_ragged && (epi == EPI_KV || epi == EPI_RES_F32)) return false;
  switch (epi) {
    case EPI_KV: return p.kv_tokens > 0 && p.kv_heads > 0 && p.kv_items > 0;
    case EPI_RES_F32: return p.R && p.r.rpi > 0;
    case EPI_RES_OP: return p.aux && !p.n_ragged;
    case EPI_GELU_BOTH:
    case EPI_GELU_BWD: return p.aux && !misaligned(p.c, 3) && !p.n_ragged;
    case EPI_SOFTPART: return p.stat_m && p.stat_l && !p.bias && !(p.c.ld & 3) && (!p.col_stats || (p.col_scale && !p.w_kwrap && p.cs_eps >= 0.f));
    case EPI_RES_LN:
      return p.R && p.r.rpi > 0 && p.ln_gain && p.ln_bias && p.ln_counter && (p.ln_y32 || p.ln_y16) && p.N % 256 == 0 && p.N <= 1024 &&
             (!p.ln_y32 || (p.ln_y32v.rpi > 0 && !misaligned(p.ln_y32v, 3))) && (!p.ln_y16 || (p.ln_y16v.rpi > 0 && !misaligned(p.ln_y16v, 3)));
    case EPI_RES_F32_STAT:
    case EPI_RES_OP_STAT:
    case EPI_LNF_OP:
    case EPI_LNF_GELU_OP:
      if (ngroups != 1 || p.batch > 1 || p.n_mask || p.n_ragged || !p.ln_y32) return false;
      if (epi == EPI_RES_OP_STAT) return p.N % 64 == 0 && p.aux && !misaligned(p.c, 7);
      if (epi == EPI_RES_F32_STAT) return p.R && p.r.rpi > 0 && p.N % 128 == 0 && p.ln_y16 && p.ln_y16v.rpi > 0 && !misaligned(p.ln_y16v, 7) && !misaligned(p.c, 3);
      return p.ln_gain && !misaligned(p.c, 7);
  }
  return true;
}

bool tile_rules(const TileDesc& d, int family, const GemmProb& p, int ngroups, int epi) {
  if (p.K % d.kstep) return false;
  if ((p.n_ragged && !(d.allow & T_RAGGED)) || (p.n_mask && !(d.allow & T_MASK)) || (p.batch > 1 && !(d.allow & T_BATCH)) || (ngroups > 1 && !(d.allow & T_GROUPS))) return false;
  if (family == GF_P8_TAIL ? p.N != 128 : family == GF_P8_MIXED ? (p.N % 256 != 128 || p.N < 384) : (p.N % d.tn && !p.n_ragged && !p.n_mask)) return false;
  if ((d.allow & T_F32_16B) && (epi == EPI_RES_F32 || epi == EPI_F32 || epi == EPI_RES_LN) && misaligned(p.c, 3)) return false;
  if (p.w_ld && (!(d.allow & T_WLD) || epi != EPI_OP || (p.w_ld & 7) || p.k_rows <= 0 || p.N % d.tn)) return false;
  if (p.w_kwrap && (!(d.allow & T_KWRAP) || p.w_kwrap < 0 || p.w_ld || 2 * p.w_kwrap * 64 != p.K)) return false;
  if (p.col_scale && (epi != EPI_SOFTPART || family != GF_WS_176x384 || p.w_ld || ngroups != 1)) return false;
  if (p.pscale && (!p.w_ld || p.M > d.tm || p.ps_ntiles <= 0 || p.K > p.ps_ntiles * d.tn + 4 * d.tn)) return false;
  return true;
}

}

bool ensure_lds(const void* fn, size_t lds) {
  static std::mutex mu;
  static std::set<std::pair<const void*, int>> done;
  int dev = 0;
  (void)hipGetDevice(&dev);
  std::lock_guard<std::mutex> g(mu);
  if (done.count({fn, dev})) return true;
  if (hipFuncSetAttribute(fn, hipFuncAttributeMaxDynamicSharedMemorySize, (int)lds) != hipSuccess) return false;
  done.insert({fn, dev});
  return true;
}

long long gemm_launch_count(int family, int epi) {
  if (family < 0 || family >= GEMM_FAMILIES || epi < 0 || epi >= 16) return -1;
  return g_launches[family][epi].load(std::memory_order_relaxed);
}
#ifdef MRA_GEMM_EXPERIMENTS
void gemm_force_config(int tile) { g_force_tile = tile; }
void gemm_force_variant(int v) { g_variant = v; }
void gemm_set_tile_order(int order) { g_order = order; }
void gemm_set_eight_phase(int on) { g_p8 = on; }
void gemm_set_debug_buffer(unsigned long long* p) { g_dbg = p; }
#endif

int gemm_plan(const GemmProb* probs, int ngroups, int epi, int op_dtype, GemmPlan* out) {
  if (ngroups < 1 || ngroups > GEMM_MAX_GROUPS) return -1;
  (void)op_dtype;
  GemmPlan& pl = *out;
  pl.tile = pick_tile(probs, ngroups);
  if (pl.tile >= GEMM_TILES) return -1;
  for (int g = 0; g < ngroups; ++g)
    if (!operand_rules(probs[g], epi) || !epilogue_rules(probs[g], ngroups, epi)) return -1;
  pl.family = pick_family(pl.tile, probs, ngroups, epi);
  const TileDesc& d = kTiles[pl.family];
  GemmArgs& a = pl.args;
  a.ngroups = ngroups;
  int tiles = 0;
  for (int g = 0; g < ngroups; ++g) {
    GemmProb& p = a.p[g] = probs[g];
    if (!tile_rules(d, pl.family, p, ngroups, epi)) return -1;
    p.mtiles = (p.M + d.tm - 1) / d.tm;
    p.ntiles = (p.N + d.tn - 1) / d.tn;
    p.tile_begin = tiles;
    if (pl.family == GF_P8_MIXED) tiles += (p.mtiles + 1) / 2 * (2 * (p.N >> 8) + 1);
    else tiles += p.mtiles * p.ntiles * (p.batch > 1 ? p.batch : 1);
  }
  if (!has_epi(d.epis, epi)) return -2;
  for (int g = ngroups; g < GEMM_MAX_GROUPS; ++g) a.p[g] = a.p[0];
  a.total_tiles = tiles;
  a.dbg = g_dbg;
  a.order = g_order ? g_order : probs[0].order;
  pl.threads = d.threads;
  pl.lds = d.lds + (a.p[0].pscale ? 4 * 2048 : 0);
  pl.persistent = pl.family == GF_P8_256 && a.p[0].persist && ngroups == 1 && a.p[0].batch <= 1 && has_epi(epi_mask(EpiP8Persist{}), epi) && pl.cus >= 8 && tiles > pl.cus;
  pl.grid = pl.persistent ? pl.cus & ~7 : tiles;
  return 0;
}

int launch_gemm(const GemmProb* probs, int ngroups, int epi, int op_dtype, hipStream_t stream) {
  GemmPlan pl;
  pl.cus = ngroups >= 1 && probs[0].persist ? device_cus() : 0;
  const int rc = gemm_plan(probs, ngroups, epi, op_dtype, &pl);
  if (rc) return rc;
  return op_dtype == OP_F16 ? launch_t<f16>(pl, epi, stream) : launch_t<bf16>(pl, epi, stream);
}

}
```

mraudio_amd/csrc/kernels.h:

```cpp
#pragma once
#include <hip/hip_runtime.h>
#include <stdint.h>

namespace mra {

enum OpDtype { OP_F16 = 0, OP_BF16 = 1 };

enum GemmEpi {
  EPI_OP = 0,
  EPI_GELU_OP = 1,
  EPI_RES_F32 = 2,
  EPI_F32 = 3,
  EPI_KV = 4,
  EPI_GELU_BOTH = 6,
  EPI_GELU_BWD = 7,
  EPI_RES_OP = 8,
  EPI_RES_LN = 9,
  EPI_RES_F32_STAT = 10,
  EPI_RES_OP_STAT = 13,
  EPI_LNF_OP = 11,
  EPI_LNF_GELU_OP = 12,
  EPI_SOFTPART = 5,
};

enum GemmTile {
  GT_AUTO = 0,
  GT_64 = 1,
  GT_128 = 2,
  GT_256 = 3,
  GT_WS_128x384 = 4,
  GT_WS_176x384 = 5,
  GT_K128_64x128 = 6,
  GT_P8_TAIL = 7,
  GT_P8_MIXED = 8,
  GT_RING_144x128 = 9,
  GT_RING_192x128 = 10,
  GT_RING_96x64 = 11,
  GEMM_TILES = 12
};

struct RowView {
  long long item_stride;
  int rpi;
  int ld;
};

struct GemmProb {
  const void* A;
  const void* W;
  const float* bias;
  void* C;
  const float* R;
  void* aux;
  RowView a, c, r;
  int M, N, K;
  int kv_tokens, kv_items, kv_heads;
  int batch;
  long long a_bs, w_bs, c_bs_bytes;
  int bias_bs;
  int n_ragged;
  int n_mask;
  int w_ld, k_rows;
  const float* ln_gain;
  const float* ln_bias;
  float ln_eps;
  float* ln_y32;
  void* ln_y16;
  RowView ln_y32v, ln_y16v;
  unsigned* ln_counter;
  int w_kwrap;
  float alpha;
  float* stat_m;
  float* stat_l;
  const float* pscale;
  int ps_ntiles;
  float* col_scale;
  long long cs_bs;
  int col_stats;
  float cs_eps;
  int tile_cfg;
  int order;
  int persist;
  int tile_begin;
  int mtiles, ntiles;
  int batch_row0;
};

constexpr int GEMM_MAX_GROUPS = 4;
struct GemmArgs {
  GemmProb p[GEMM_MAX_GROUPS];
  int ngroups;
  int total_tiles;
  unsigned long long* dbg;
  int order;
};

int launch_gemm(const GemmProb* probs, int ngroups, int epi, int op_dtype, hipStream_t stream);
struct GemmPlan {
  int cus;
  int tile;
  int family;
  int threads, lds;
  int persistent;
  int grid;
  GemmArgs args;
};
int gemm_plan(const GemmProb* probs, int ngroups, int epi, int op_dtype, GemmPlan* out);
enum GemmFamily {
  GF_V1_64 = 0, GF_V1_128 = 1, GF_V1_256 = 2,
  GF_WS_256 = 3,
  GF_P8_256 = 4,
  GF_WS_128x384 = 5, GF_WS_176x384 = 6,
  GF_K128_64x128 = 7,
  GF_P8_TAIL = 8, GF_P8_MIXED = 9,
  GF_K128_64x64 = 10,
  GF_RING_144x128 = 11, GF_RING_192x128 = 12, GF_RING_96x64 = 13,
  GEMM_FAMILIES = 14
};
long long gemm_launch_count(int family, int epi);
#ifdef MRA_GEMM_EXPERIMENTS
void gemm_force_config(int tile);
void gemm_set_debug_buffer(unsigned long long* dev_buf);
void gemm_set_eight_phase(int on);
void gemm_set_tile_order(int order);
void gemm_force_variant(int v);
#endif

struct GemmTnArgs {
  const void* dY;
  const void* X;
  float* dW;
  RowView yv, xv;
  long long y_block_stride, x_block_stride;
  int M, N, K;
  int ldw;
  int accumulate;
  float* db;
};
int launch_gemm_tn(const GemmTnArgs& a, int op_dtype, hipStream_t stream);
constexpr int GEMM_TN_MAX_JOBS = 4;
struct GemmTnGroup {
  GemmTnArgs j[GEMM_TN_MAX_JOBS];
  int njobs;
  int nb_begin[GEMM_TN_MAX_JOBS + 1];
};
int launch_gemm_tn_group(const GemmTnArgs* jobs, int njobs, int op_dtype, hipStream_t stream);
int launch_kvgrad_gemm(const void* dkv, const void* W, float* d_enc, int Ne, int kv, int heads, int nsel, int E, int op_dtype, hipStream_t stream);
int launch_modality_ln_bwd(const void* x, int x_dtype, int items, int tokens, int E, const float* gain, float eps, const float* d_out, float* d_x,
                           float* d_gain, float* d_bias, hipStream_t stream);
int launch_colsum(const void* dY, long long block_stride, RowView yv, int M, int N, float* db, int accumulate, int op_dtype,
                  hipStream_t stream);

struct LnBwdArgs {
  const float* dy; RowView dyv;
  const float* x; RowView xv;
  const float* gamma;
  float eps;
  int rows;
  float* dx; RowView dxv;
  const float* add; RowView addv;
  void* dx16; RowView dx16v;
  float* dgamma; float* dbeta;
};
int launch_ln_bwd(const LnBwdArgs& a, int H, int op_dtype, hipStream_t stream);
int launch_ln_bwd2(const LnBwdArgs& a, const LnBwdArgs* b, int H, int op_dtype, hipStream_t stream);
int launch_gelu(const void* u, const void* df, void* out, long long n, int backward, int op_dtype, hipStream_t stream);
struct AttnBwdArgs {
  const void *Q, *K, *V, *O, *dO;
  void *dQ, *dK, *dV;
  long long q_item_stride, o_item_stride, dq_item_stride;
  int q_ld, o_ld, dq_ld;
  long long k_item_stride, k_head_stride, v_item_stride, v_head_stride;
  int k_ld, v_ld;
  long long dk_item_stride, dk_head_stride, dv_item_stride, dv_head_stride;
  int dk_ld, dv_ld;
  const long long* mask; int mask_ld;
  const float* lse;
  int items, heads, q_rows, kv_len;
  float scale;
  int kv_share;
};
int launch_attn_bwd(const AttnBwdArgs& a, int op_dtype, hipStream_t stream);
constexpr size_t ATTN_BWD_LDS_LIMIT = 160 * 1024;
size_t attn_bwd_mfma_lds_bytes(int q_rows, int kv_share);
int attn_bwd_max_share(int q_rows);
#ifdef MRA_GEMM_EXPERIMENTS
void attn_bwd_force_valu(int on);
#endif
int launch_embed_bwd(const float* demb, const long long* ids, int items, int L, int Q, int H, int vocab, float* dquery, float* dpos,
                     float* dword, hipStream_t stream);
int launch_transpose16(const void* src, void* dst, int R, int C, int op_dtype, hipStream_t stream);
struct TrJob { const void* src; void* dst; int R, C, tile_begin, tiles_x; };
int launch_transpose16_batch(const TrJob* jobs_dev, int njobs, int total_tiles, int op_dtype, hipStream_t stream);
int launch_add_f32(const float* x, float* y, long long n, hipStream_t stream);
struct FlatSeg;
struct AdamScalars { float beta1, beta2, eps, weight_decay, step_size, inv_sqrt_bc2; int zero_grad; };
struct AdamMatJob { unsigned long long off; void* dst; void* dstT; int R, C, ldT, tile_begin, tiles_x; };
int launch_adam_mats(float* master, float* grad, float* m, float* v, const AdamMatJob* jobs_dev, int njobs, int total_tiles, AdamScalars sc, int op_dtype,
                     hipStream_t stream);
int launch_adam_flat(float* master, float* grad, float* m, float* v, const FlatSeg* segs, int nseg, AdamScalars sc, hipStream_t stream);

int launch_softmax_rows(const float* S, long long ld_s, void* P, long long ld_p, int rows, int kv, int kvp, float scale, int op_dtype,
                        hipStream_t stream);
int launch_fold_rowfactor(const float* stat_m, const float* stat_l, float* factors, int rows, int R, int ntiles, void* P, long long ld_p, int tile_cols,
                          int kvp, hipStream_t stream, int* hist = nullptr);
int launch_softmax_rescale(void* P, long long ld_p, const float* stat_m, const float* stat_l, int rows, int ntiles, int tile_cols, int kvp,
                           int op_dtype, hipStream_t stream, int* hist = nullptr);
int launch_transpose_pad(const void* src, void* dst, int R, int C, int ld_d, long long src_bs, long long dst_bs, int batch, int op_dtype,
                         hipStream_t stream);

int launch_fold_ln_weight(const void* W, int w32, int rows, int E, const float* gain, const float* ln_bias, const float* bias_in, void* dst,
                          int key_layout, float* bias_out, int op_dtype, hipStream_t stream);

struct FoldStreamArgs {
  const void* qp;
  void* qpb;
  const void* enc;
  void* p;
  void* u;
  float* stat_m;
  float* stat_l;
  void* gexp;
  float* ginv;
  int items, kv, kvp, E;
  float alpha;
  int phase;
};
bool fold_stream_supported(int rows, int E, int kv, int kvp, int op_dtype);
int fold_stream_stat_ld(int kvp);
int launch_fold_stream(const FoldStreamArgs& a, hipStream_t stream);

struct AttnArgs {
  const void* Q;
  const void* K;
  const void* V;
  void* O;
  long long q_item_stride, o_item_stride;
  int q_ld, o_ld;
  long long k_item_stride, k_head_stride;
  long long v_item_stride, v_head_stride;
  int k_ld, v_ld;
  const long long* mask;
  int mask_ld;
  int items, heads, q_rows, kv_len;
  float scale;
  int nsplit;
  float* part;
  float* lse;
  int kv_share = 1;
};
size_t attn_partial_bytes(int items, int heads, int q_rows, int nsplit);
int attn_pick_split(int items, int heads, int q_rows, int kv_len);
int launch_attention(const AttnArgs& a, int op_dtype, hipStream_t stream);
int attn_shared_pick_split(int kv_items, int kv_share, int heads, int kv_len);
int launch_attention_shared(const AttnArgs& a, int op_dtype, hipStream_t stream);

int launch_ln_rows(const float* x, RowView xv, int rows, int H, const float* gain, const float* bias, float eps,
                   float* y32, RowView y32v, void* y16, RowView y16v, int op_dtype, hipStream_t stream);
int launch_ln_rows2(const float* x, RowView xv, int rows, int H, const float* gain, const float* bias, const float* gain2,
                    const float* bias2, int period, int split, float eps, float* y32, RowView y32v, void* y16, RowView y16v,
                    int op_dtype, hipStream_t stream);
int launch_ln_rows4(const float* x, RowView xv, int rows, int H, const float* gain, const float* bias, const float* gain2, const float* bias2,
                    int lane_rows, const float* gain3, const float* bias3, const float* gain4, const float* bias4, int period, int split,
                    float eps, float* y32, RowView y32v, void* y16, RowView y16v, int op_dtype, hipStream_t stream);
int launch_modality_ln(const void* x, int x_dtype, const long long* item_index, int items, int tokens, int E,
                       const float* gain, const float* bias, float eps, void* out, int op_dtype, hipStream_t stream);
int launch_embed_ln(const long long* ids, int items, int L, int Q, int H, int vocab, const float* query,
                    long long query_item_stride, const float* word,
                    const float* pos, const float* gain, const float* bias, float eps, float* h32, void* h16,
                    float* pre32 , int op_dtype, hipStream_t stream);
struct FlatSeg { unsigned long long src_off; void* dst; int n; int dtype; };
constexpr int FLAT_SEG = 16384;
int launch_convert_flat(const float* master, const FlatSeg* segs, int nseg, hipStream_t stream);
int launch_convert(const void* src, int src_dtype, void* dst, int dst_dtype , long long n,
                   hipStream_t stream);
int launch_copy_rows_f32(const float* src, RowView sv, float* dst, RowView dv, int rows, int H, hipStream_t stream);
int launch_split_rows(const float* src, RowView sv, int rows, int C, int chunk, int parts, void* dst, int op_dtype, hipStream_t stream);
int launch_split_weight(const float* W, int rows, int C, void* dst, int op_dtype, hipStream_t stream);
int launch_split_key_weight(const float* W, int heads, int E, void* dst, int op_dtype, hipStream_t stream);

bool ensure_lds(const void* fn, size_t lds);

int launch_cosine_score(const float* z, const float* t, int t_rows, int items, int Q, int H, float eps, float* sim,
                        float* logit, hipStream_t stream);
int launch_fuse_logits(const float* const* logits, const float* weights, int nmod, int n, float* out,
                       hipStream_t stream);
int launch_span(const float* logits, int videos, int clips, float alpha, int* spans, hipStream_t stream);
int launch_windows(const float* logits, int videos, int clips, float alpha, int top_k, float nms_thd, int max_len, int* windows,
// ... 4 lines not shown
```

mraudio_amd/csrc/mra_abi.hip:

```cpp
#include <cstdio>
#include <cstdlib>

#include "mra_handle.h"

using namespace mra;
using namespace mra_host;

namespace mra_host {
thread_local std::string g_err;
}

namespace {

size_t layout_params(mra_qformer* h, char* base) {
  const mra_cfg& c = h->cfg;
  const size_t H = c.hidden, I = c.inter, E = c.enc_width;
  Carver cv(base);
  size_t goff = 0;
  auto reg = [&](const std::string& name, void* p, int dtype, long long numel) {
    Param pr;
    pr.ptr = p;
    pr.dtype = dtype;
    pr.numel = numel;
    pr.goff = goff;
// ... 31 lines not shown
  }
  int cl = 0;
  for (int i = 0; i < c.layers; ++i) {
    LayerW& L = h->layers[i];
    const std::string p = "bert.encoder.layer." + std::to_string(i) + ".";
    char* wqkv = cv.take<char>(3 * H * H, 2);
    L.wqkv = wqkv;
    L.bqkv = cv.take<float>(3 * H);
    const char* names[3] = {"query", "key", "value"};
    for (int j = 0; j < 3; ++j) {
      reg(p + "attention.self." + names[j] + ".weight", wqkv ? wqkv + (size_t)j * H * H * 2 : nullptr, opd, H * H);
      reg(p + "attention.self." + names[j] + ".bias", L.bqkv ? L.bqkv + j * H : nullptr, MRA_F32, H);
    }
    L.wo = cv.take<char>(H * H, 2);
    L.bo = cv.take<float>(H);
    L.ln1g = cv.take<float>(H);
    L.ln1b = cv.take<float>(H);
    reg(p + "attention.output.dense.weight", L.wo, opd, H * H);
    reg(p + "attention.output.dense.bias", L.bo, MRA_F32, H);
    reg(p + "attention.output.LayerNorm.weight", L.ln1g, MRA_F32, H);
    reg(p + "attention.output.LayerNorm.bias", L.ln1b, MRA_F32, H);
    L.cross_index = -1;
    if (i % c.cross_freq == 0) {
      L.cross_index = cl;
      L.wcq = cv.take<char>(H * H, 2);
      L.wcq32 = cv.take<float>(H * H);
      L.bcq = cv.take<float>(H);
      L.wco = cv.take<char>(H * H, 2);
      L.bco = cv.take<float>(H);
      L.lncg = cv.take<float>(H);
      L.lncb = cv.take<float>(H);
      reg(p + "crossattention.self.query.weight", L.wcq, opd, H * H);
      h->params[p + "crossattention.self.query.weight"].copy32 = L.wcq32;
      reg(p + "crossattention.self.query.bias", L.bcq, MRA_F32, H);
      char* wkv = (char*)h->wkv;
      reg(p + "crossattention.self.key.weight", wkv ? wkv + (size_t)(cl * 2 + 0) * H * E * 2 : nullptr, opd, H * E);
      h->params[p + "crossattention.self.key.weight"].copy32 = h->wk32 ? h->wk32 + (size_t)cl * H * E : nullptr;
      reg(p + "crossattention.self.key.bias", h->bkv ? h->bkv + (size_t)(cl * 2 + 0) * H : nullptr, MRA_F32, H);
      reg(p + "crossattention.self.value.weight", wkv ? wkv + (size_t)(cl * 2 + 1) * H * E * 2 : nullptr, opd, H * E);
      reg(p + "crossattention.self.value.bias", h->bkv ? h->bkv + (size_t)(cl * 2 + 1) * H : nullptr, MRA_F32, H);
      reg(p + "crossattention.output.dense.weight", L.wco, opd, H * H);
      reg(p + "crossattention.output.dense.bias", L.bco, MRA_F32, H);
      reg(p + "crossattention.output.LayerNorm.weight", L.lncg, MRA_F32, H);
      reg(p + "crossattention.output.LayerNorm.bias", L.lncb, MRA_F32, H);
      ++cl;
    }
    L.wit = cv.take<char>(I * H, 2);
    L.bit = cv.take<float>(I);
    L.wot = cv.take<char>(H * I, 2);
    L.bot = cv.take<float>(H);
    L.lntg = cv.take<float>(H);
    L.lntb = cv.take<float>(H);
    L.wiq = cv.take<char>(I * H, 2);
    L.biq = cv.take<float>(I);
    L.woq = cv.take<char>(H * I, 2);
    L.boq = cv.take<float>(H);
    L.lnqg = cv.take<float>(H);
    L.lnqb = cv.take<float>(H);
    reg(p + "intermediate.dense.weight", L.wit, opd, I * H);
    reg(p + "intermediate.dense.bias", L.bit, MRA_F32, I);
    reg(p + "output.dense.weight", L.wot, opd, H * I);
    reg(p + "output.dense.bias", L.bot, MRA_F32, H);
    reg(p + "output.LayerNorm.weight", L.lntg, MRA_F32, H);
    reg(p + "output.LayerNorm.bias", L.lntb, MRA_F32, H);
    reg(p + "intermediate_query.dense.weight", L.wiq, opd, I * H);
    reg(p + "intermediate_query.dense.bias", L.biq, MRA_F32, I);
    reg(p + "output_query.dense.weight", L.woq, opd, H * I);
    reg(p + "output_query.dense.bias", L.boq, MRA_F32, H);
    reg(p + "output_query.LayerNorm.weight", L.lnqg, MRA_F32, H);
    reg(p + "output_query.LayerNorm.bias", L.lnqb, MRA_F32, H);
  }
  h->grad_bytes = goff;
  return cv.off;
}

struct CrossPlan {
  enum Form { KV_CACHE, FOLD, FOLD_STREAM } form;
  bool precise;
  bool probe;
  bool kmajor;
  bool softpart;
  bool inreg;
  bool raw;
  int scores_tile, penc_tile;
};

CrossPlan cross_plan(const mra_qformer* h, int kv, bool precise, bool probe, bool raw = false) {
  const mra_cfg& c = h->cfg;
  const int R = c.heads * c.n_query;
  CrossPlan x{};
  x.precise = precise;
  x.probe = probe;
  const bool fold = h->ncross > 0 && (precise || probe || h->cross_mode == 2 || (h->cross_mode == 0 && kv >= 2048));
  const bool stream = fold && !precise && !probe && h->fold_stream && fold_stream_supported(R, c.enc_width, kv, fold_kvp(kv), h->op());
  x.form = stream ? CrossPlan::FOLD_STREAM : fold ? CrossPlan::FOLD : CrossPlan::KV_CACHE;
  x.kmajor = R == 384 && c.enc_width % 176 == 0;
  x.softpart = R == 384;
  x.inreg = (h->inreg_rescale || probe) && x.softpart && x.kmajor;
  x.scores_tile = R == 384 ? GT_WS_176x384 : GT_128;
  x.penc_tile = x.kmajor ? GT_WS_176x384 : (R == 384 ? h->fold_tile : GT_128);
  x.raw = raw && x.form == CrossPlan::FOLD && x.softpart && x.kmajor && x.inreg && !precise && !probe;
  return x;
}

struct Work {
  float *hA32, *hB32, *pre32, *hC32, *part;
  char *hA16, *hB16, *qkv16, *ctx16, *qc16, *hC16, *ffn16, *kv16;
  char *encT, *qp16, *p16, *u16;
  char* qpb16;
  char *hs16, *qs16;
  float *qc32, *qp32;
  unsigned* lncnt;
  size_t lncnt_bytes;
  float* s32;
  float* stat;
  float* gfac;
  float* rt;
  float *st_m, *st_l, *ginv;
  char* gexp;
  int nsplit;
};

struct Lane {
  mra_qformer* h;
  const void* enc;
  int kv;
  CrossPlan plan;
  const float* query;
  long long query_stride;
  float *out_query, *out_full, *out_cls;
  Work w;
  int share = 1;
};

void layout_chain(Carver& cv, Work& w, size_t NN, size_t n0, size_t S, size_t H, size_t I, size_t Q) {
  auto f32 = [&](size_t per_item) { float* p = cv.take<float>(NN * per_item); return p ? p + n0 * per_item : p; };
  auto op = [&](size_t per_item) { char* p = cv.take<char>(NN * per_item, 2); return p ? p + n0 * per_item * 2 : p; };
  w.hA32 = f32(S * H);
  w.hB32 = f32(S * H);
  w.pre32 = f32(S * H);
  w.hC32 = f32(Q * H);
  w.hA16 = op(S * H);
  w.hB16 = op(S * H);
  w.qkv16 = op(S * 3 * H);
  w.ctx16 = op(S * H);
  w.qc16 = op(Q * H);
  w.hC16 = op(Q * H);
  w.ffn16 = op(S * I);
  w.lncnt_bytes = 2 * (NN * S / 64 + 2) * sizeof(unsigned);
  w.lncnt = cv.take<unsigned>(w.lncnt_bytes / sizeof(unsigned));
}

void layout_cross(const mra_qformer* h, const CrossPlan& x, Carver& cv, Work& w, int N, int Kv, int share = 1) {
  const mra_cfg& c = h->cfg;
  const size_t H = c.hidden, Q = c.n_query, E = c.enc_width, R = (size_t)c.heads * Q, kvp = fold_kvp(Kv);
  if (x.form == CrossPlan::FOLD_STREAM) {
    const size_t sld = fold_stream_stat_ld((int)kvp);
    w.qp16 = cv.take<char>((size_t)N * R * E, 2);
    w.qpb16 = cv.take<char>((size_t)N * R * E, 2);
    w.st_m = cv.take<float>((size_t)N * R * sld);
    w.st_l = cv.take<float>((size_t)N * R * sld);
    w.gexp = cv.take<char>((size_t)N * R * sld, 2);
    w.ginv = cv.take<float>((size_t)N * R);
    w.p16 = cv.take<char>((size_t)N * R * kvp, 2);
    w.u16 = cv.take<char>((size_t)N * R * E, 2);
  } else if (x.form == CrossPlan::FOLD) {
    if (!x.kmajor) w.encT = cv.take<char>((size_t)N * E * kvp, 2);
    w.qp16 = cv.take<char>((size_t)N * R * E * (x.precise ? 2 : 1), 2);
    if (x.precise) {
      w.hs16 = cv.take<char>((size_t)N * Q * 3 * H, 2);
      w.qs16 = cv.take<char>((size_t)N * Q * 3 * H, 2);
      w.qc32 = cv.take<float>((size_t)N * Q * H);
      w.qp32 = cv.take<float>((size_t)N * R * E);
    }
    if (!x.softpart) w.s32 = cv.take<float>((size_t)N * R * kvp);
    w.stat = cv.take<float>((size_t)2 * N * R * ((Kv + 175) / 176));
    if (x.inreg) w.gfac = cv.take<float>((size_t)N * ((Kv + 175) / 176) * 512);
    w.p16 = cv.take<char>((size_t)N * R * kvp, 2);
    w.u16 = cv.take<char>((size_t)N * R * E, 2);
    if (x.raw) w.rt = cv.take<float>((size_t)N * kvp);
  } else {
    w.kv16 = cv.take<char>((size_t)h->ncross * 2 * N * Kv * H, 2);
  }
  w.nsplit = share > 1 && h->multi_core == 1 ? attn_shared_pick_split(N, share, c.heads, Kv) : attn_pick_split(N * share, c.heads, (int)Q, Kv);
}

size_t layout_lanes(Lane* lanes, int nl, char* base, int N, int L, long long** mask2 = nullptr) {
  const mra_cfg& c = lanes[0].h->cfg;
  const size_t S = (size_t)c.n_query + L;
  Carver cv(base);
  const Carver chain = cv;
  for (int l = 0; l < nl; ++l) {
    lanes[l].w = Work{};
    cv = chain;
    layout_chain(cv, lanes[l].w, (size_t)nl * N, (size_t)l * N, S, c.hidden, c.inter, c.n_query);
  }
  for (int l = 0; l < nl; ++l) {
    Work& w = lanes[l].w;
    layout_cross(lanes[l].h, lanes[l].plan, cv, w, N / lanes[l].share, lanes[l].kv, lanes[l].share);
    float* part = cv.take<float>(attn_partial_bytes(N, c.heads, c.n_query, w.nsplit) / sizeof(float) + (nl > 1 ? 64 : 0));
    w.part = w.nsplit > 1 ? part : nullptr;
  }
  long long* m2 = nl > 1 ? cv.take<long long>((size_t)nl * N * S) : nullptr;
  if (mask2) *mask2 = m2;
  return cv.off;
}

Lane make_lane(mra_qformer* h, const void* enc, int kv, bool precise, bool probe, bool raw = false) {
  Lane x{};
  x.h = h;
  x.enc = enc;
  x.kv = kv;
  x.plan = cross_plan(h, kv, precise, probe, raw);
  x.query = h->query;
  return x;
}

size_t work_bytes(Lane x, int N, int L) { return layout_lanes(&x, 1, nullptr, N, L); }

int cross_core(const Lane& lane, const LayerW& Lw, int N, hipStream_t stream) {
  const mra_qformer* h = lane.h;
  const CrossPlan& x = lane.plan;
  const Work& w = lane.w;
  const void* enc = lane.enc;
  const int kv = lane.kv;
  const mra_cfg& c = h->cfg;
  const int Q = c.n_query, H = c.hidden, E = c.enc_width, R = c.heads * Q, kvp = fold_kvp(kv), op = h->op();
  const size_t esz = 2;
  const RowView qc_rows = plain(N * Q, H);
  const int ci = Lw.cross_index;
  int rc = 0;
  if (x.form == CrossPlan::KV_CACHE) {
    AttnArgs a = kv_cross_attn_args(c, w.qc16, w.kv16, ci, w.ctx16, N / lane.share, kv, w.nsplit, w.part);
    a.items = N;
    a.kv_share = lane.share;
    rc = lane.share > 1 && h->multi_core == 1 ? launch_attention_shared(a, op, stream) : launch_attention(a, op, stream);
    return rc ? chk(rc, "cross attention") : MRA_OK;
  }
  const bool timed = ci == 0 && h->kv_ev0 && h->kv_ev1;
  if (timed) (void)hipEventRecord(h->kv_ev0, stream);
  int* hist = x.probe ? h->auto_hist + (size_t)ci * 256 : nullptr;
  GemmProb d{};
  if (x.precise) {
    rc = launch_split_rows(w.qc32, qc_rows, N * Q, H, 64, 3, w.qs16, op, stream);
    if (rc) return chk(rc, "split cross query");
    d.A = w.qs16; d.a = plain(N * Q, 3 * H); d.a_bs = 192;
    d.W = h->arena_p + (size_t)ci * precise_layer_bytes(h) + precise_wk_off(h); d.w_bs = (long long)E * 192;
    d.C = w.qp32; d.c = items_view((long long)R * E, Q, E); d.c_bs_bytes = (long long)Q * E * 4;
    d.M = N * Q; d.N = E; d.K = 192; d.batch = c.heads; d.tile_cfg = (N * Q) % 128 == 0 && E % 128 == 0 ? GT_128 : GT_64;
    rc = launch_gemm(&d, 1, EPI_F32, op, stream);
    if (rc) return chk(rc, "fold q' gemm (split precision)");
    rc = launch_split_rows(w.qp32, plain(N * R, E), N * R, E, E, 2, w.qp16, op, stream);
    if (rc) return chk(rc, "split q'");
  } else {
    d.A = w.qc16; d.a = qc_rows; d.a_bs = 64;
    d.W = x.raw ? fold_raw_wk(h, ci) : h->arena_f + (size_t)ci * H * E * esz; d.w_bs = (long long)E * 64;
    d.C = w.qp16; d.c = items_view((long long)R * E, Q, E); d.c_bs_bytes = (long long)Q * E * esz;
    d.M = N * Q; d.N = E; d.K = 64; d.batch = c.heads; d.tile_cfg = (N * Q) % 128 == 0 && E % 128 == 0 ? GT_128 : GT_64;
    rc = launch_gemm(&d, 1, EPI_OP, op, stream);
    if (rc) return chk(rc, "fold q' gemm");
  }
  if (x.form == CrossPlan::FOLD_STREAM) {
    FoldStreamArgs fs{};
    fs.qp = w.qp16; fs.qpb = w.qpb16; fs.enc = enc; fs.p = w.p16; fs.u = w.u16;
    fs.stat_m = w.st_m; fs.stat_l = w.st_l; fs.gexp = w.gexp; fs.ginv = w.ginv;
    fs.items = N; fs.kv = kv; fs.kvp = kvp; fs.E = E;
    fs.alpha = 0.125f * 1.4426950408889634f; fs.phase = 3;
    rc = launch_fold_stream(fs, stream);
    if (rc) return chk(rc, "fold scores / P.enc (streaming kernels)");
  } else {
    GemmProb sc{};
    sc.A = w.qp16; sc.a = plain(R, E); sc.a_bs = (long long)R * E;
    sc.W = enc; sc.w_bs = (long long)kv * E;
    sc.M = R; sc.N = kv; sc.K = E; sc.batch = N; sc.n_ragged = 1;
    if (x.precise) {
      sc.a = plain(R, 2 * E); sc.a_bs = (long long)R * 2 * E; sc.K = 2 * E; sc.w_kwrap = E / 64;
    }
    sc.tile_cfg = x.scores_tile;
    const int ntiles = (kv + 175) / 176;
    if (x.softpart) {
      sc.C = w.p16; sc.c = plain(R, kvp); sc.c_bs_bytes = (long long)R * kvp * esz;
      sc.alpha = 0.125f * 1.4426950408889634f;
      sc.stat_m = w.stat; sc.stat_l = w.stat + (size_t)N * R * ntiles;
      if (x.raw) {
        sc.col_scale = w.rt; sc.cs_bs = kvp; sc.col_stats = ci == 0; sc.cs_eps = c.enc_ln_eps;
      }
      rc = launch_gemm(&sc, 1, EPI_SOFTPART, op, stream);
      if (rc) return chk(rc, "fold scores gemm (softmax partials)");
      if (x.inreg) {
        rc = launch_fold_rowfactor(sc.stat_m, sc.stat_l, w.gfac, N * R, R, ntiles, w.p16, kvp, 176, kvp, stream, hist);
        if (rc) return chk(rc, "fold row factors");
      } else {
        rc = launch_softmax_rescale(w.p16, kvp, sc.stat_m, sc.stat_l, N * R, ntiles, 176, kvp, op, stream, hist);
        if (rc) return chk(rc, "fold softmax rescale");
      }
    } else {
      sc.C = w.s32; sc.c = plain(R, kvp); sc.c_bs_bytes = (long long)R * kvp * 4;
      rc = launch_gemm(&sc, 1, EPI_F32, op, stream);
      if (rc) return chk(rc, "fold scores gemm");
      rc = launch_softmax_rows(w.s32, kvp, w.p16, kvp, N * R, kv, kvp, 0.125f, op, stream);
      if (rc) return chk(rc, "fold softmax");
    }
    GemmProb pv{};
    pv.A = w.p16; pv.a = plain(R, kvp); pv.a_bs = (long long)R * kvp;
    if (x.kmajor) {
      pv.W = enc; pv.w_bs = (long long)kv * E; pv.w_ld = E; pv.k_rows = kv;
    } else {
      pv.W = w.encT; pv.w_bs = (long long)E * kvp;
    }
    pv.C = w.u16; pv.c = plain(R, E); pv.c_bs_bytes = (long long)R * E * esz;
    pv.M = R; pv.N = E; pv.K = kvp; pv.batch = N;
    pv.tile_cfg = x.penc_tile;
    if (x.inreg) { pv.pscale = w.gfac; pv.ps_ntiles = ntiles; }
    rc = launch_gemm(&pv, 1, EPI_OP, op, stream);
    if (rc) return chk(rc, "fold p.enc gemm");
  }
  GemmProb cx{};
  cx.A = w.u16; cx.a = items_view((long long)R * E, Q, E); cx.a_bs = (long long)Q * E;
  cx.W = (const char*)h->wkv + (size_t)(ci * 2 + 1) * H * E * esz; cx.w_bs = (long long)64 * E;
  cx.bias = h->bkv + (size_t)(ci * 2 + 1) * H; cx.bias_bs = 64;
  if (x.raw) { cx.W = fold_raw_wv(h, ci); cx.bias = fold_raw_bv(h, ci); }
  cx.C = w.ctx16; cx.c = qc_rows; cx.c_bs_bytes = 64 * esz;
  cx.M = N * Q; cx.N = 64; cx.K = E; cx.batch = c.heads; cx.tile_cfg = E % 128 == 0 && N * Q >= 512 ? GT_K128_64x128 : GT_64;
  rc = launch_gemm(&cx, 1, EPI_OP, op, stream);
  if (rc) return chk(rc, "fold context gemm");
  if (timed) (void)hipEventRecord(h->kv_ev1, stream);
  return MRA_OK;
}

}

namespace mra_host {
int kv_project(const mra_qformer* h, const void* enc, int N, int kv, void* kv_cache, hipStream_t stream) {
  const mra_cfg& c = h->cfg;
  GemmProb p{};
  p.A = enc;
  p.a = plain(N * kv, c.enc_width);
  p.W = h->wkv;
  p.bias = h->bkv;
  p.C = kv_cache;
  p.c = plain(1, 1);
  p.M = N * kv;
  p.N = h->ncross * 2 * c.hidden;
  p.K = c.enc_width;
  p.kv_tokens = kv;
  p.kv_items = N;
  p.kv_heads = c.heads;
  p.persist = 1;
  return launch_gemm(&p, 1, EPI_KV, h->op(), stream);
}

}

extern "C" {

const char* mra_last_error(void) { return g_err.c_str(); }
const char* mra_version(void) { return "mraudio_amd 0.1 (gfx950)"; }
int64_t mra_debug_gemm_launches(int32_t family, int32_t epilogue) { return gemm_launch_count(family, epilogue); }

void mra_cfg_default(mra_cfg* c, int32_t enc_width) {
  c->hidden = 768;
  c->heads = 12;
  c->inter = 3072;
  c->layers = 12;
  c->cross_freq = 2;
  c->enc_width = enc_width;
  c->n_query = 32;
  c->vocab = 30523;
  c->max_pos = 512;
  c->ln_eps = 1e-12f;
  c->enc_ln_eps = 1e-5f;
  c->llm_hidden = 4096;
  c->op_dtype = MRA_F16;
}

int mra_qformer_create(const mra_cfg* cfg, mra_qformer** out) {
  if (!cfg || !out) return fail(MRA_EINVAL, "null argument");
  const mra_cfg& c = *cfg;
  if (c.hidden <= 0 || c.hidden % 256 || c.hidden > 1024) return fail(MRA_EINVAL, "hidden must be a multiple of 256, <= 1024");
  if (c.heads <= 0 || c.hidden != c.heads * 64) return fail(MRA_EINVAL, "head_dim must be 64");
  if (c.n_query != 32) return fail(MRA_EINVAL, "n_query must be 32");
  if (c.inter <= 0 || c.inter % 256) return fail(MRA_EINVAL, "inter must be a multiple of 256");
  if (c.enc_width <= 0 || c.enc_width % 64) return fail(MRA_EINVAL, "enc_width must be a multiple of 64");
  if (c.layers <= 0 || c.cross_freq <= 0 || c.vocab <= 0 || c.max_pos <= 0) return fail(MRA_EINVAL, "bad layer/vocab config");
  if (c.llm_hidden < 0 || c.llm_hidden % 256) return fail(MRA_EINVAL, "llm_hidden must be 0 or a multiple of 256");
  if (c.op_dtype != MRA_F16 && c.op_dtype != MRA_BF16) return fail(MRA_EINVAL, "op_dtype must be MRA_F16 or MRA_BF16");
  mra_qformer* h = new mra_qformer();
  h->cfg = c;
  HIP_TRY(hipGetDevice(&h->device));
  h->arena_bytes = layout_params(h, nullptr);
  hipError_t e = hipMalloc((void**)&h->arena, h->arena_bytes);
  if (e != hipSuccess) {
    delete h;
    return fail(MRA_ENOMEM, std::string("hipMalloc of parameter arena: ") + hipGetErrorString(e));
  }
  layout_params(h, h->arena);
  if (h->ncross > 0) {
    e = hipMalloc((void**)&h->arena_f, fold_arena_bytes(h));
    if (e != hipSuccess) {
      mra_qformer_destroy(h);
      return fail(MRA_ENOMEM, std::string("fold weight arena: ") + hipGetErrorString(e));
    }
  }
  std::vector<FlatSeg> segs;
  for (auto& kv : h->params) {
    if (kv.first.rfind("bert.", 0) != 0) continue;
// ... 175 lines not shown
    if (ln_fuse) HIP_TRY(hipMemsetAsync(w.lncnt, 0, w.lncnt_bytes, stream));
    if (x.plan.form != CrossPlan::KV_CACHE) {
      if (x.plan.form == CrossPlan::FOLD && !x.plan.kmajor) {
        const int E = hl->cfg.enc_width, kvp = fold_kvp(x.kv);
        rc = launch_transpose_pad(x.enc, x.w.encT, x.kv, E, kvp, (long long)x.kv * E, (long long)E * kvp, N, op, stream);
        if (rc) return chk(rc, "enc transpose");
      }
      if ((rc = mra_qformer_prepare(hl, stream))) return rc;
    } else if (hl->ncross > 0) {
      const bool timed = !pair && hl->kv_ev0 && hl->kv_ev1;
      if (timed) (void)hipEventRecord(hl->kv_ev0, stream);
      rc = kv_project(hl, x.enc, N / x.share, x.kv, x.w.kv16, stream);
      if (rc) return chk(rc, "kv projection gemm");
      if (timed) (void)hipEventRecord(hl->kv_ev1, stream);
    }
    if (!pair && hl->kv_done) (void)hipEventRecord(hl->kv_done, stream);
  }
  const long long* mask = (const long long*)attention_mask;
  if (pair && mask) {
    HIP_TRY(hipMemcpyAsync(mask2, mask, (size_t)N * S * 8, hipMemcpyDeviceToDevice, stream));
    HIP_TRY(hipMemcpyAsync(mask2 + (size_t)N * S, mask, (size_t)N * S * 8, hipMemcpyDeviceToDevice, stream));
    mask = mask2;
  }

  const bool want_text_last = lanes[0].out_full != nullptr;
  bool want_cls_last = false;
  for (int l = 0; l < nl; ++l) want_cls_last |= !want_text_last && lanes[l].out_cls;

  for (int i = 0; i < c.layers; ++i) {
    const LayerW* Lw[2] = {&lanes[0].h->layers[i], &lanes[nl - 1].h->layers[i]};
    const bool last = i == c.layers - 1;
    {
      GemmProb p[2] = {};
      for (int l = 0; l < nl; ++l) {
        p[l].A = lanes[l].w.hA16; p[l].a = all_rows;
        p[l].W = Lw[l]->wqkv; p[l].bias = Lw[l]->bqkv;
        p[l].C = lanes[l].w.qkv16; p[l].c = plain(N * S, 3 * H);
        p[l].M = N * S; p[l].N = 3 * H; p[l].K = H;
        p[l].tile_cfg = N * S >= 1024 ? GT_128 : GT_AUTO;
        if ((lanes[l].h->chain_ring & 1) && N * S >= 1024 && (3 * H) % 144 == 0) p[l].tile_cfg = GT_RING_144x128;
      }
      rc = launch_gemm(p, nl, EPI_OP, op, stream);
      if (rc) return chk(rc, "qkv gemm");
    }
    rc = launch_attention(self_attn_args(c, w.qkv16, w.ctx16, mask, nl * N, S), op, stream);
    if (rc) return chk(rc, "self attention");
    {
      GemmProb p[2] = {};
      for (int l = 0; l < nl; ++l) {
        p[l].A = lanes[l].w.ctx16; p[l].a = all_rows;
        p[l].W = Lw[l]->wo; p[l].bias = Lw[l]->bo;
        p[l].R = lanes[l].w.hA32; p[l].r = all_rows;
        p[l].C = lanes[l].w.pre32; p[l].c = all_rows;
        p[l].M = N * S; p[l].N = H; p[l].K = H;
        if ((lanes[l].h->chain_ring & 4) && N * S >= 1024 && H % 96 == 0) p[l].tile_cfg = GT_RING_96x64;
      }
      if (ln_fuse && p[0].tile_cfg == GT_RING_96x64) {
        p[0].ln_gain = Lw[0]->ln1g; p[0].ln_bias = Lw[0]->ln1b; p[0].ln_eps = c.ln_eps;
        p[0].ln_y32 = w.hB32; p[0].ln_y32v = all_rows; p[0].ln_y16 = w.hB16; p[0].ln_y16v = all_rows; p[0].ln_counter = w.lncnt;
        rc = launch_gemm(p, 1, EPI_RES_LN, op, stream);
        if (rc) return chk(rc, "attn out gemm + ln");
      } else {
        rc = launch_gemm(p, nl, EPI_RES_F32, op, stream);
        if (rc) return chk(rc, "attn out gemm");
        rc = launch_ln_rows4(w.pre32, all_lanes, nl * N * S, H, Lw[0]->ln1g, Lw[0]->ln1b, nullptr, nullptr, N * S, Lw[1]->ln1g, Lw[1]->ln1b, nullptr,
                             nullptr, 1, 1, c.ln_eps, w.hB32, all_lanes, w.hB16, all_lanes, op, stream);
        if (rc) return chk(rc, "attn ln");
      }
    }
    const bool cross = Lw[0]->cross_index >= 0;
    const RowView fqv = cross ? qc_rows : q_view;
    if (cross) {
      if (lanes[0].plan.precise) {
        rc = launch_split_rows(w.hB32, q_view, N * Q, H, H, 3, w.hs16, op, stream);
        if (rc) return chk(rc, "split query rows");
        GemmProb p{};
        p.A = w.hs16; p.a = plain(N * Q, 3 * H);
        p.W = h->arena_p + (size_t)Lw[0]->cross_index * precise_layer_bytes(h); p.bias = Lw[0]->bcq;
        p.C = w.qc32; p.c = qc_rows;
        p.M = N * Q; p.N = H; p.K = 3 * H;
        rc = launch_gemm(&p, 1, EPI_F32, op, stream);
      } else {
        GemmProb p[2] = {};
        for (int l = 0; l < nl; ++l) {
          p[l].A = lanes[l].w.hB16; p[l].a = q_view;
          p[l].W = Lw[l]->wcq; p[l].bias = Lw[l]->bcq;
          p[l].C = lanes[l].w.qc16; p[l].c = qc_rows;
          p[l].M = N * Q; p[l].N = H; p[l].K = H;
        }
        rc = launch_gemm(p, nl, EPI_OP, op, stream);
      }
      if (rc) return chk(rc, "cross q gemm");
      for (int l = 0; l < nl; ++l)
        if ((rc = cross_core(lanes[l], *Lw[l], N, stream))) return rc;
      GemmProb o[2] = {};
      for (int l = 0; l < nl; ++l) {
        o[l].A = lanes[l].w.ctx16; o[l].a = qc_rows;
        o[l].W = Lw[l]->wco; o[l].bias = Lw[l]->bco;
        o[l].R = lanes[l].w.hB32; o[l].r = q_view;
        o[l].C = lanes[l].w.pre32; o[l].c = qc_rows;
        o[l].M = N * Q; o[l].N = H; o[l].K = H;
      }
      if (ln_fuse && N * Q >= 512) {
        o[0].tile_cfg = GT_RING_96x64;
        o[0].ln_gain = Lw[0]->lncg; o[0].ln_bias = Lw[0]->lncb; o[0].ln_eps = c.ln_eps;
        o[0].ln_y32 = w.hC32; o[0].ln_y32v = qc_rows; o[0].ln_y16 = w.hC16; o[0].ln_y16v = qc_rows; o[0].ln_counter = w.lncnt;
        rc = launch_gemm(o, 1, EPI_RES_LN, op, stream);
        if (rc) return chk(rc, "cross out gemm + ln");
      } else {
        rc = launch_gemm(o, nl, EPI_RES_F32, op, stream);
        if (rc) return chk(rc, "cross out gemm");
        const RowView pre_v = items_view((long long)N * S * H, N * Q, H), qc_lanes = plain(nl * N * Q, H);
        rc = launch_ln_rows4(w.pre32, pre_v, nl * N * Q, H, Lw[0]->lncg, Lw[0]->lncb, nullptr, nullptr, N * Q, Lw[1]->lncg, Lw[1]->lncb, nullptr, nullptr,
                             1, 1, c.ln_eps, w.hC32, qc_lanes, w.hC16, qc_lanes, op, stream);
        if (rc) return chk(rc, "cross ln");
      }
    }
    int text_rows = 0;
    RowView tv = t_view;
    if (L > 0) {
      if (!last || want_text_last) text_rows = N * L;
      else if (want_cls_last) { text_rows = N; tv = cls_view; }
    }
    const int ng = text_rows > 0 ? 2 * nl : nl;
    {
      GemmProb g[4] = {};
      for (int l = 0; l < nl; ++l) {
        const Work& v = lanes[l].w;
        GemmProb& q = g[l];
        q.A = cross ? v.hC16 : v.hB16; q.a = fqv;
        q.W = Lw[l]->wiq; q.bias = Lw[l]->biq;
        q.C = v.ffn16; q.c = plain(N * Q, I);
        q.M = N * Q; q.N = I; q.K = H;
        GemmProb& t = g[nl + l];
        t.A = v.hB16 + t_off16; t.a = tv;
        t.W = Lw[l]->wit; t.bias = Lw[l]->bit;
        t.C = v.ffn16 + (size_t)N * Q * I * esz; t.c = plain(text_rows, I);
        t.M = text_rows; t.N = I; t.K = H;
      }
      if ((h->chain_ring & 2) && N * Q >= 512 && I % 192 == 0) g[0].tile_cfg = GT_RING_192x128;
      rc = launch_gemm(g, ng, EPI_GELU_OP, op, stream);
      if (rc) return chk(rc, "ffn up gemm");
    }
    bool ffn_ln_fused = false;
    {
      GemmProb g[4] = {};
      for (int l = 0; l < nl; ++l) {
        const Work& v = lanes[l].w;
        GemmProb& q = g[l];
        q.A = v.ffn16; q.a = plain(N * Q, I);
        q.W = Lw[l]->woq; q.bias = Lw[l]->boq;
        q.R = cross ? v.hC32 : v.hB32; q.r = fqv;
        q.C = v.pre32; q.c = q_view;
        q.M = N * Q; q.N = H; q.K = I;
        GemmProb& t = g[nl + l];
        t.A = v.ffn16 + (size_t)N * Q * I * esz; t.a = plain(text_rows, I);
        t.W = Lw[l]->wot; t.bias = Lw[l]->bot;
        t.R = v.hB32 + t_off32; t.r = tv;
        t.C = v.pre32 + t_off32; t.c = tv;
        t.M = text_rows; t.N = H; t.K = I;
      }
      g[0].tile_cfg = N * Q >= 512 && I % 128 == 0 ? GT_K128_64x128 : GT_AUTO;
      if ((h->chain_ring & 4) && N * Q >= 512 && H % 96 == 0) g[0].tile_cfg = GT_RING_96x64;
      ffn_ln_fused = ln_fuse && !last && g[0].tile_cfg == GT_RING_96x64;
      if (ffn_ln_fused) {
        g[0].ln_gain = Lw[0]->lnqg; g[0].ln_bias = Lw[0]->lnqb; g[0].ln_eps = c.ln_eps;
        g[0].ln_y32 = w.hA32; g[0].ln_y32v = q_view; g[0].ln_y16 = w.hA16; g[0].ln_y16v = q_view; g[0].ln_counter = w.lncnt;
        g[1].ln_gain = Lw[0]->lntg; g[1].ln_bias = Lw[0]->lntb; g[1].ln_eps = c.ln_eps;
        g[1].ln_y32 = w.hA32 + t_off32; g[1].ln_y32v = tv; g[1].ln_y16 = w.hA16 + t_off16; g[1].ln_y16v = tv;
        g[1].ln_counter = w.lncnt + (N * Q + 63) / 64;
        rc = launch_gemm(g, ng, EPI_RES_LN, op, stream);
        if (rc) return chk(rc, "ffn down gemm + ln");
      } else {
// ... 354 lines not shown
  }
  h->fold_stale = false;
  return MRA_OK;
}

int mra_qformer_set_cross_mode(mra_qformer* h, int32_t mode) {
  if (!h) return fail(MRA_EINVAL, "null handle");
  if (mode < 0 || mode > 5)
    return fail(MRA_EINVAL, "cross mode must be 0 (automatic), 1 (K/V cache), 2 (folded), 3 (folded, 128x384 loader-wave tiles), 4 (folded, streaming kernels) or 5 (folded, separate rescale pass)");
  h->cross_mode = mode >= 3 ? 2 : mode;
  h->fold_tile = mode == 3 ? GT_WS_128x384 : GT_128;
  h->fold_stream = mode == 4;
  h->inreg_rescale = mode != 5;
  return MRA_OK;
}

int mra_qformer_set_cross_precision(mra_qformer* h, int32_t mode) {
  if (!h) return fail(MRA_EINVAL, "null handle");
  if (mode < 0 || mode > 2)
    return fail(MRA_EINVAL, "cross precision must be 0 (operand dtype), 1 (split: hi + lo pairs along the score chain) or 2 (auto: chosen by a probe)");
  if (mode >= 1) {
    const mra_cfg& c = h->cfg;
    if (h->ncross == 0) return fail(MRA_EINVAL, "no cross-attention layers");
    if (!cross_plan(h, 1, true, false).softpart)
      return fail(MRA_EINVAL, "split precision needs heads * n_query == 384 (the 176 x 384 scores tile)");
    if (!h->arena_p || (mode == 2 && !h->auto_hist)) {
      int dev = 0;
      HIP_TRY(hipGetDevice(&dev));
      if (dev != h->device) return fail(MRA_EINVAL, "handle belongs to another device");
    }
    if (!h->arena_p) {
      const hipError_t e = hipMalloc((void**)&h->arena_p, (size_t)h->ncross * precise_layer_bytes(h));
      if (e != hipSuccess) return fail(MRA_ENOMEM, std::string("split-precision weight arena: ") + hipGetErrorString(e));
      h->precise_stale = true;
    }
    if (mode == 2 && !h->auto_hist) {
      const size_t hist_bytes = (size_t)h->ncross * 256 * sizeof(int);
      hipError_t e = hipMalloc((void**)&h->auto_hist, hist_bytes);
      if (e != hipSuccess) return fail(MRA_ENOMEM, std::string("auto-precision histograms: ") + hipGetErrorString(e));
      e = hipHostMalloc((void**)&h->auto_hist_host, hist_bytes, hipHostMallocDefault);
      if (e != hipSuccess) return fail(MRA_ENOMEM, std::string("auto-precision pinned histograms: ") + hipGetErrorString(e));
      h->auto_median.assign(h->ncross, -1.f);
    }
  }
  h->cross_auto = mode == 2;
  h->auto_stale = true;
  h->cross_precise = mode == 1;
  return MRA_OK;
}

int mra_qformer_cross_precision_report(mra_qformer* h, int32_t* resolved, int32_t* probes, float* median_pmax, int32_t n_layers) {
  if (!h) return fail(MRA_EINVAL, "null handle");
  if (median_pmax && n_layers < h->ncross) return fail(MRA_EINVAL, "median_pmax needs one float per cross layer (" + std::to_string(h->ncross) + ")");
  if (resolved) *resolved = h->cross_auto ? (h->auto_stale ? -1 : h->auto_resolved) : h->cross_precise;
  if (probes) *probes = h->auto_probes;
  if (median_pmax)
    for (int ci = 0; ci < h->ncross; ++ci) median_pmax[ci] = ci < (int)h->auto_median.size() ? h->auto_median[ci] : -1.f;
  return MRA_OK;
}

int mra_qformer_set_option(mra_qformer* h, const char* name, int32_t value) {
  if (!h || !name) return fail(MRA_EINVAL, "null argument");
  const std::string key(name);
  if (key == "train_ring") {
    if (value < 0 || value > 7) return fail(MRA_EINVAL, "train_ring is a mask of bits 0-2");
    h->train_ring = value;
    return MRA_OK;
  }
  if (key == "raw_features") {
    if (value < 0 || value > 1) return fail(MRA_EINVAL, "raw_features is 0 or 1");
    h->raw_features = value != 0;
    return MRA_OK;
  }
  if (key == "auto_split_pmax_milli") {
    if (value < 0 || value > 1000) return fail(MRA_EINVAL, "auto_split_pmax_milli is a threshold on p_max in [0, 1000] thousandths");
    h->auto_tau_milli = value;
    return MRA_OK;
  }
  if (key == "chain_ring") {
    if (value < 0 || value > 15) return fail(MRA_EINVAL, "chain_ring is a mask of bits 0-3");
    h->chain_ring = value;
    return MRA_OK;
  }
  if (key == "multi_core") {
    if (value < 0 || value > 1) return fail(MRA_EINVAL, "multi_core is 0 (attn_kernel with kv_share) or 1 (shared-stream core)");
    h->multi_core = value;
    return MRA_OK;
  }
  return fail(MRA_ENAME, "unknown option: " + key);
}

int mra_qformer_set_kv_done_event(mra_qformer* h, void* ev) {
  if (!h) return fail(MRA_EINVAL, "null handle");
  h->kv_done = reinterpret_cast<hipEvent_t>(ev);
  return MRA_OK;
}

size_t mra_kv_cache_bytes(mra_qformer* h, int32_t items, int32_t kv) {
  if (!h || items <= 0 || kv <= 0) return 0;
  return (size_t)h->ncross * 2 * items * kv * h->cfg.hidden * 2;
}

int mra_kv_project(mra_qformer* h, const void* enc, int32_t items, int32_t kv, void* kv_cache, void* stream) {
  if (!h) return fail(MRA_EINVAL, "null handle");
  if (items < 0 || kv < 0) return fail(MRA_EINVAL, "negative size");
  if (items == 0 || kv == 0 || h->ncross == 0) return MRA_OK;
  if (!enc || !kv_cache) return fail(MRA_EINVAL, "null argument");
  if ((long long)items * kv > 0x7fffffffLL) return fail(MRA_EINVAL, "items * kv exceeds int32");
  return chk(kv_project(h, enc, items, kv, kv_cache, as_stream(stream)), "kv projection gemm");
}

int mra_llm_proj(mra_qformer* h, const float* z, int32_t rows, void* out, int32_t out_dtype, void* workspace,
                 size_t workspace_bytes, void* stream_) {
  if (!h) return fail(MRA_EINVAL, "null handle");
  if (rows < 0) return fail(MRA_EINVAL, "negative rows");
  if (rows == 0) return MRA_OK;
  const mra_cfg& c = h->cfg;
  if (c.llm_hidden <= 0 || !h->params["llm_proj.weight"].loaded || !h->params["llm_proj.bias"].loaded)
    return fail(MRA_ESTATE, "llm_proj not loaded");
  if (!z || !out || !workspace) return fail(MRA_EINVAL, "null argument");
  const size_t need = align_up((size_t)rows * c.hidden * 2);
  if (workspace_bytes < need) return fail(MRA_ENOMEM, "workspace too small: need " + std::to_string(need));
  const int op = h->op();
  if (out_dtype != MRA_F32 && out_dtype != c.op_dtype) return fail(MRA_EINVAL, "out_dtype must be f32 or the operand dtype");
  hipStream_t stream = as_stream(stream_);
  int rc = launch_convert(z, MRA_F32, workspace, c.op_dtype, (long long)rows * c.hidden, stream);
  if (rc) return chk(rc, "convert z");
  GemmProb p{};
  p.A = workspace; p.a = plain(rows, c.hidden);
  p.W = h->wllm; p.bias = h->bllm;
  p.C = out; p.c = plain(rows, c.llm_hidden);
  p.M = rows; p.N = c.llm_hidden; p.K = c.hidden;
  return chk(launch_gemm(&p, 1, out_dtype == MRA_F32 ? EPI_F32 : EPI_OP, op, stream), "llm_proj gemm");
}

int mra_cosine_score(const float* z, const float* t, int32_t t_rows, int32_t items, int32_t n_query, int32_t hidden,
                     float* sim, float* logit, void* stream) {
  if (items < 0) return fail(MRA_EINVAL, "negative items");
  if (items == 0) return MRA_OK;
  if (!z || !t || !logit) return fail(MRA_EINVAL, "null argument");
  return chk(launch_cosine_score(z, t, t_rows, items, n_query, hidden, 1e-8f, sim, logit, as_stream(stream)), "cosine_score");
}

int mra_fuse_logits(const float* const* logits, const float* weights, int32_t nmod, int32_t n, float* out, void* stream) {
  if (n < 0) return fail(MRA_EINVAL, "negative n");
  if (!logits || !out) return fail(MRA_EINVAL, "null argument");
  for (int m = 0; m < nmod && m < 4; ++m)
    if (!logits[m]) return fail(MRA_EINVAL, "null logits pointer");
  return chk(launch_fuse_logits(logits, weights, nmod, n, out, as_stream(stream)), "fuse_logits");
}

int mra_span_from_logits(const float* logits, int32_t videos, int32_t clips, float alpha, int32_t* spans, void* stream) {
  if (videos < 0) return fail(MRA_EINVAL, "negative videos");
  if (videos == 0) return MRA_OK;
  if (!logits || !spans) return fail(MRA_EINVAL, "null argument");
  return chk(launch_span(logits, videos, clips, alpha, spans, as_stream(stream)), "span_from_logits");
}

int mra_windows_from_logits(const float* logits, int32_t videos, int32_t clips, float alpha, int32_t top_k, float nms_thd,
                            int32_t max_len, int32_t* windows, float* scores, int32_t* counts, void* stream) {
  if (videos < 0) return fail(MRA_EINVAL, "negative videos");
  if (videos == 0) return MRA_OK;
  if (!logits || !windows || !scores || !counts) return fail(MRA_EINVAL, "null argument");
  if (clips < 1 || clips > 4096) return fail(MRA_EINVAL, "clips must be in 1..4096");
  if (top_k < 1 || top_k > 64) return fail(MRA_EINVAL, "top_k must be in 1..64");
  if (!(nms_thd >= 0.f && nms_thd < 1.f)) return fail(MRA_EINVAL, "nms_thd must be in [0, 1)");
// ... 264 lines not shown
    jobs[i] = TrJob{src[i], dst[i], R[i], C[i], (int)tiles, tx};
    tiles += (long long)tx * ty;
    if (tiles > 0x7fffffffLL) return fail(MRA_EINVAL, "too many tiles");
  }
  HIP_TRY(hipMemcpy(scratch, jobs, (size_t)njobs * sizeof(TrJob), hipMemcpyHostToDevice));
  return chk(launch_transpose16_batch((const TrJob*)scratch, njobs, (int)tiles, op, as_stream(stream)), "transpose16_batch");
}

int mra_debug_gemm_gelu(int32_t nprob, const void* const* A, const int64_t* a_views, const void* const* W, const float* const* bias, void* const* C,
                        const int64_t* c_views, void* const* aux, const int32_t* M, const int32_t* N, const int32_t* K, int32_t backward, int32_t tile_cfg,
                        int32_t dtype, void* stream) {
  int op;
  if (nprob < 1 || nprob > 2) return fail(MRA_EINVAL, "one or two problems");
  if (!dbg_op(dtype, &op)) return fail(MRA_EINVAL, "dtype must be f16 or bf16");
  if (tile_cfg != GT_AUTO && tile_cfg != GT_64 && tile_cfg != GT_128 && tile_cfg != GT_256) return fail(MRA_EINVAL, "tile_cfg must be GT_AUTO, GT_64, GT_128 or GT_256");
  if (!A || !a_views || !W || !C || !c_views || !aux || !M || !N || !K) return fail(MRA_EINVAL, "null argument array");
  GemmProb ps[2];
  for (int i = 0; i < nprob; ++i) {
    GemmProb& p = ps[i];
    p = GemmProb{};
    if (!A[i] || !W[i] || !C[i] || !aux[i]) return fail(MRA_EINVAL, "null A, W, C or aux");
    if (!dbg_view8(a_views + 3 * i, &p.a)) return fail(MRA_EINVAL, "the A view needs rows per item > 0 and strides that are multiples of 8");
    if (!dbg_view(c_views + 3 * i, &p.c)) return fail(MRA_EINVAL, "the C view needs rows per item > 0 and strides that are multiples of 4");
    if (!dbg_aligned(A[i], 16) || !dbg_aligned(W[i], 16) || !dbg_aligned(C[i], 8) || !dbg_aligned(aux[i], 8) || (bias && !dbg_aligned(bias[i], 16)))
      return fail(MRA_EINVAL, "misaligned buffer");
    p.A = A[i]; p.W = W[i]; p.bias = bias ? bias[i] : nullptr; p.C = C[i]; p.aux = aux[i];
    p.M = M[i]; p.N = N[i]; p.K = K[i];
    if (p.M > 0 && (p.a.ld < p.K || p.c.ld < p.N)) return fail(MRA_EINVAL, "row stride below the row length");
  }
  ps[0].tile_cfg = tile_cfg;
  const int epi = backward ? EPI_GELU_BWD : EPI_GELU_BOTH;
  GemmPlan pl;
  pl.cus = 0;
  const int rc = gemm_plan(ps, nprob, epi, op, &pl);
  if (rc) return fail(MRA_EINVAL, rc == -2 ? "the tile has no such epilogue" : "gemm_plan refuses the problem (M, N > 0, K % 64, N % tile)");
  return chk(launch_gemm(ps, nprob, epi, op, as_stream(stream)), "gemm gelu");
}

namespace {
typedef unsigned __int128 u128;

u128 dbg_extent(const RowView& v, long long rows, long long cols) {
  if (rows <= 0 || cols <= 0) return 0;
  const long long last_item = (rows - 1) / v.rpi, last_row = (rows - 1) % v.rpi;
  u128 far = (u128)last_item * (u128)v.item_stride + (u128)last_row * (u128)v.ld;
  if (last_item > 0) {
    const u128 full = (u128)(last_item - 1) * (u128)v.item_stride + (u128)(v.rpi - 1) * (u128)v.ld;
    if (full > far) far = full;
  }
  return far + (u128)cols;
}
bool dbg_fits(u128 elements, size_t esz, u128 extra_bytes, uint64_t have) { return elements * esz + extra_bytes <= (u128)have; }

const char* dbg_gemm_prob(const mra_gemm_desc& d, int epi, GemmProb* out) {
  GemmProb& p = *out;
  p = GemmProb{};
  if (d.struct_bytes != sizeof(mra_gemm_desc)) return "struct_bytes is not sizeof(mra_gemm_desc)";
  if (!d.A || !d.W || !d.C) return "null A, W or C";
  if (d.M <= 0 || d.N <= 0 || d.K <= 0) return "M, N and K must be positive";
  if (d.batch < 0 || d.batch > 65535 || d.a_bs < 0 || d.w_bs < 0 || d.c_bs_bytes < 0 || d.bias_bs < 0) return "negative batch count or batch stride (batch <= 65535)";
  if (d.n_ragged < 0 || d.n_ragged > 1 || d.persist < 0 || d.persist > 1 || d.w_ld < 0 || d.k_rows < 0 || d.w_kwrap < 0 || d.ps_ntiles < 0)
    return "n_ragged and persist are 0 or 1; w_ld, k_rows, w_kwrap and ps_ntiles are not negative";
  if (d.tile_cfg < GT_AUTO || d.tile_cfg >= GEMM_TILES || d.tile_cfg == GT_P8_TAIL) return "tile_cfg outside the forwards' tiles";
  if (!dbg_view8(d.a_view, &p.a)) return "the A view needs rows per item > 0 and strides that are non-negative multiples of 8";
  if (epi == EPI_KV) p.c = RowView{0, 1, 1};
  else if (!dbg_view(d.c_view, &p.c)) return "the C view needs rows per item > 0 and strides that are non-negative multiples of 4";
  const bool res = epi == EPI_RES_F32 || epi == EPI_RES_LN || epi == EPI_RES_F32_STAT;
  const bool resop = epi == EPI_RES_OP || epi == EPI_RES_OP_STAT, lnf = epi == EPI_LNF_OP || epi == EPI_LNF_GELU_OP;
  if ((resop || lnf || epi == EPI_RES_F32_STAT) && (d.batch > 1 || d.n_ragged)) return "the ViT's epilogues (8, 10 .. 13) take one plain problem: no batch, no n_ragged";
  if (res && (!d.R || !dbg_view(d.r_view, &p.r))) return "the residual needs a pointer and a view with strides that are multiples of 4";
  if (!dbg_aligned(d.A, 16) || !dbg_aligned(d.W, 16) || !dbg_aligned(d.C, 16) || !dbg_aligned(d.bias, 16) || (res && !dbg_aligned(d.R, 16)))
    return "A, W, C, R and bias must be 16-byte aligned";
  if (d.batch > 1 && ((d.a_bs & 7) || (d.w_bs & 7) || (d.c_bs_bytes & 15) || (d.bias_bs & 3)))
    return "batch strides: a_bs and w_bs multiples of 8 elements, c_bs_bytes of 16 bytes, bias_bs of 4 floats";
  if (d.batch > 1 && (epi == EPI_KV || epi == EPI_RES_LN)) return "EPI_KV and EPI_RES_LN take no batch";
  if (p.a.ld < d.K) return "A row stride below K";
  if (d.w_ld && d.w_ld < d.N) return "w_ld below N";
  p.A = d.A; p.W = d.W; p.bias = d.bias; p.C = d.C; p.R = res ? d.R : nullptr;
  p.M = d.M; p.N = d.N; p.K = d.K;
  p.kv_tokens = d.kv_tokens; p.kv_items = d.kv_items; p.kv_heads = d.kv_heads;
  p.batch = d.batch; p.a_bs = d.a_bs; p.w_bs = d.w_bs; p.c_bs_bytes = d.c_bs_bytes; p.bias_bs = d.bias_bs;
  p.n_ragged = d.n_ragged; p.w_ld = d.w_ld; p.k_rows = d.k_rows; p.w_kwrap = d.w_kwrap;
  p.tile_cfg = d.tile_cfg; p.persist = d.persist;
  if (epi == EPI_KV) {
    if (d.kv_tokens <= 0 || d.kv_items <= 0 || d.kv_heads <= 0 || d.kv_heads > 1024) return "EPI_KV needs kv_tokens, kv_items and kv_heads > 0";
    if (d.N % (d.kv_heads * 64)) return "EPI_KV: N must be a multiple of kv_heads * 64";
    if ((long long)d.M > (long long)d.kv_items * d.kv_tokens) return "EPI_KV: M exceeds kv_items * kv_tokens";
  }
  if (epi == EPI_RES_LN) {
    if (!d.ln_gain || !d.ln_bias || !d.ln_counter || (!d.ln_y32 && !d.ln_y16)) return "EPI_RES_LN needs gain, bias, counters and an output";
    if ((d.ln_y32 && !dbg_view(d.ln_y32_view, &p.ln_y32v)) || (d.ln_y16 && !dbg_view(d.ln_y16_view, &p.ln_y16v)))
      return "a LayerNorm output view needs rows per item > 0 and strides that are multiples of 4";
    if (!dbg_aligned(d.ln_gain, 16) || !dbg_aligned(d.ln_bias, 16) || !dbg_aligned(d.ln_y32, 16) || !dbg_aligned(d.ln_y16, 16) || !dbg_aligned(d.ln_counter, 4))
      return "the LayerNorm buffers must be 16-byte aligned (counters: 4)";
    if (!(d.ln_eps >= 0.f)) return "ln_eps must not be negative";
    p.ln_gain = d.ln_gain; p.ln_bias = d.ln_bias; p.ln_eps = d.ln_eps; p.ln_y32 = d.ln_y32; p.ln_y16 = d.ln_y16; p.ln_counter = d.ln_counter;
  }
  if (resop) {
    if (!d.aux || !dbg_aligned(d.aux, 16)) return "EPI_RES_OP / EPI_RES_OP_STAT need aux (16-byte aligned)";
    p.aux = d.aux;
  }
  if (epi == EPI_RES_F32_STAT || epi == EPI_RES_OP_STAT) {
    if (!d.ln_y32 || !dbg_aligned(d.ln_y32, 8)) return "the statistics epilogues need ln_y32 (8-byte aligned)";
    if (!d.bias) return "the statistics epilogues need a bias";
    p.ln_y32 = d.ln_y32;
  }
  if (epi == EPI_RES_F32_STAT) {
    if (!d.ln_y16 || !dbg_aligned(d.ln_y16, 16) || !dbg_view8(d.ln_y16_view, &p.ln_y16v))
      return "EPI_RES_F32_STAT needs ln_y16 (16-byte aligned) and a view of it with strides that are multiples of 8";
    p.ln_y16 = d.ln_y16;
  }
  if (lnf) {
    if (!d.ln_y32 || !dbg_aligned(d.ln_y32, 8)) return "EPI_LNF_* need ln_y32 = (mean, rstd) per row (8-byte aligned)";
    if (!d.ln_gain || !dbg_aligned(d.ln_gain, 16)) return "EPI_LNF_* need ln_gain = the column sums (16-byte aligned)";
    p.ln_y32 = d.ln_y32; p.ln_gain = d.ln_gain;
  }
  if (epi == EPI_SOFTPART) {
    if (!d.stat_m || !d.stat_l || !dbg_aligned(d.stat_m, 4) || !dbg_aligned(d.stat_l, 4)) return "EPI_SOFTPART needs stat_m and stat_l (4-byte aligned)";
    if (!(d.alpha > 0.f) || !(d.alpha < 3.0e38f)) return "EPI_SOFTPART needs a finite alpha > 0";
    p.alpha = d.alpha; p.stat_m = d.stat_m; p.stat_l = d.stat_l;
  }
  if (d.pscale) {
    if (!dbg_aligned(d.pscale, 16)) return "pscale must be 16-byte aligned";
    if (d.M > 384) return "pscale needs M <= 384 (one row tile)";
    p.pscale = d.pscale; p.ps_ntiles = d.ps_ntiles;
  }
  if (d.col_scale || d.col_stats) {
    if (epi != EPI_SOFTPART) return "col_scale belongs to EPI_SOFTPART";
    if (!d.col_scale || !dbg_aligned(d.col_scale, 4)) return "col_scale must be given (4-byte aligned) with col_stats";
    if (d.col_stats < 0 || d.col_stats > 1 || d.cs_bs < 0 || !(d.cs_eps >= 0.f)) return "col_stats is 0 or 1; cs_bs and cs_eps are not negative";
    if (d.batch > 1 && d.cs_bs < d.N) return "cs_bs below N";
    p.col_scale = d.col_scale; p.cs_bs = d.cs_bs; p.col_stats = d.col_stats; p.cs_eps = d.cs_eps;
  }
  return nullptr;
}

const char* dbg_gemm_epi_ok(int epi) {
  switch (epi) {
    case EPI_OP: case EPI_GELU_OP: case EPI_RES_F32: case EPI_F32: case EPI_KV: case EPI_SOFTPART: case EPI_RES_LN: return nullptr;
    case EPI_RES_OP: case EPI_RES_F32_STAT: case EPI_LNF_OP: case EPI_LNF_GELU_OP: case EPI_RES_OP_STAT: return nullptr;
  }
  return "epilogue must be one of 0 .. 5 and 8 .. 13 (csrc/kernels.h): the training step's EPI_GELU_BOTH / EPI_GELU_BWD have an entry of their own";
}

int dbg_tile_cols(int family) {
  switch (family) {
    case GF_V1_64: case GF_K128_64x128: case GF_K128_64x64: return 64;
    case GF_V1_128: case GF_WS_128x384: case GF_P8_TAIL: return 128;
    case GF_V1_256: case GF_WS_256: case GF_P8_256: case GF_P8_MIXED: return 256;
    case GF_WS_176x384: return 176;
    case GF_RING_144x128: return 144;
    case GF_RING_192x128: return 192;
    case GF_RING_96x64: return 96;
  }
  return 0;
}

const char* dbg_gemm_footprint(const mra_gemm_desc& d, const GemmProb& p, const GemmPlan& pl, int g, int epi) {
  const long long nb = d.batch > 1 ? d.batch : 1;
  const long long ntiles = pl.args.p[g].ntiles;
  const long long cols = (d.n_ragged || epi == EPI_SOFTPART) ? ntiles * dbg_tile_cols(pl.family) : d.N;
  const size_t csz = (epi == EPI_RES_F32 || epi == EPI_F32 || epi == EPI_RES_LN || epi == EPI_RES_F32_STAT) ? 4 : 2;
  if ((d.n_ragged || epi == EPI_SOFTPART) && (cols < d.N || ntiles != (d.N + dbg_tile_cols(pl.family) - 1) / dbg_tile_cols(pl.family))) return "unknown tile";
  if (!dbg_fits(dbg_extent(p.a, d.M, d.K) + (u128)(nb - 1) * (u128)d.a_bs, 2, 0, d.a_bytes)) return "A: the view, K and the batch stride leave a_bytes";
  u128 w = d.w_ld ? (u128)(d.k_rows - 1) * (u128)d.w_ld + (u128)d.N : (u128)d.N * (u128)(d.w_kwrap ? d.K / 2 : d.K);
  if (!dbg_fits(w + (u128)(nb - 1) * (u128)d.w_bs, 2, 0, d.w_bytes)) return "W: N, K (w_ld, k_rows, w_kwrap) and the batch stride leave w_bytes";
  if (d.bias && !dbg_fits((u128)d.N + (u128)(nb - 1) * (u128)d.bias_bs, 4, 0, d.bias_bytes)) return "bias: N and the batch stride leave bias_bytes";
  if (epi == EPI_KV) {
    const u128 n = (u128)(d.N / (d.kv_heads * 64)) * (u128)d.kv_items * (u128)d.kv_heads * (u128)d.kv_tokens * 64;
    if (!dbg_fits(n, 2, 0, d.c_bytes)) return "C: the head-major scatter leaves c_bytes";
  } else {
    if (p.c.ld < cols) return "C row stride below the columns written (ceil(N / tile) * tile with n_ragged and EPI_SOFTPART)";
    if (!dbg_fits(dbg_extent(p.c, d.M, cols), csz, (u128)(nb - 1) * (u128)d.c_bs_bytes, d.c_bytes)) return "C: the view, the columns written and the batch stride leave c_bytes";
  }
  if (p.R) {
    if (p.r.ld < d.N) return "R row stride below N";
    if (!dbg_fits(dbg_extent(p.r, d.M, d.N), 4, 0, d.r_bytes)) return "R: the view leaves r_bytes";
  }
  if (p.aux) {
    if (!dbg_fits(dbg_extent(p.c, d.M, cols), 2, 0, d.aux_bytes)) return "aux: the C view and the columns written leave aux_bytes";
    const uintptr_t c0 = (uintptr_t)d.C, a0 = (uintptr_t)d.aux;
    const u128 span = dbg_extent(p.c, d.M, cols) * 2;
    if (a0 != c0 && (u128)a0 < (u128)c0 + span && (u128)c0 < (u128)a0 + span) return "aux overlaps C without being C";
  }
  if (epi == EPI_RES_F32_STAT || epi == EPI_RES_OP_STAT) {
    const int gw = epi == EPI_RES_F32_STAT ? 128 : 64;
    if (d.N % gw) return "the statistics epilogues need N to be a multiple of the group width (128 in fp32, 64 in the operand dtype)";
    if (!dbg_fits((u128)d.M * (u128)(d.N / gw) * 2, 4, 0, d.ln_y32_bytes)) return "ln_y32: M x (N / group width) x 2 floats leave ln_y32_bytes";
  }
  if (epi == EPI_RES_F32_STAT && (p.ln_y16v.ld < d.N || !dbg_fits(dbg_extent(p.ln_y16v, d.M, d.N), 2, 0, d.ln_y16_bytes)))
    return "ln_y16: row stride below N, or the view leaves ln_y16_bytes";
  if (epi == EPI_LNF_OP || epi == EPI_LNF_GELU_OP) {
    if (!dbg_fits((u128)d.M * 2, 4, 0, d.ln_y32_bytes)) return "ln_y32: M x 2 floats of (mean, rstd) leave ln_y32_bytes";
    if (!dbg_fits((u128)d.N, 4, 0, d.ln_gain_bytes)) return "ln_gain: N floats of column sums leave ln_gain_bytes";
  }
  if (epi == EPI_SOFTPART) {
    const u128 n = (u128)nb * (u128)d.M * (u128)ntiles;
    if (!dbg_fits(n, 4, 0, d.stat_m_bytes) || !dbg_fits(n, 4, 0, d.stat_l_bytes)) return "stat_m / stat_l: batch * M * ntiles floats leave their sizes";
  }
  if (p.pscale && !dbg_fits((u128)nb * (u128)d.ps_ntiles * 512, 4, 0, d.pscale_bytes)) return "pscale: batch * ps_ntiles * 512 floats leave pscale_bytes";
  if (p.col_scale && !dbg_fits((u128)d.N + (u128)(nb - 1) * (u128)d.cs_bs, 4, 0, d.col_scale_bytes)) return "col_scale: N floats and the batch stride leave col_scale_bytes";
  if (epi == EPI_RES_LN) {
    if (!dbg_fits((u128)d.N, 4, 0, d.ln_gain_bytes) || !dbg_fits((u128)d.N, 4, 0, d.ln_bias_bytes)) return "ln_gain / ln_bias: N floats leave their sizes";
    if (p.ln_y32 && (p.ln_y32v.ld < d.N || !dbg_fits(dbg_extent(p.ln_y32v, d.M, d.N), 4, 0, d.ln_y32_bytes))) return "ln_y32: row stride below N, or the view leaves ln_y32_bytes";
    if (p.ln_y16 && (p.ln_y16v.ld < d.N || !dbg_fits(dbg_extent(p.ln_y16v, d.M, d.N), 2, 0, d.ln_y16_bytes))) return "ln_y16: row stride below N, or the view leaves ln_y16_bytes";
    if (!dbg_fits((u128)((d.M + 63) / 64), 4, 0, d.ln_counter_bytes)) return "ln_counter: ceil(M / 64) counters leave ln_counter_bytes";
  }
  return nullptr;
}

int dbg_gemm_prepare(const mra_gemm_desc* probs, int32_t nprob, int32_t epi, int32_t dtype, int cus, GemmProb* ps, GemmPlan* pl, int* op) {
  if (nprob < 1 || nprob > GEMM_MAX_GROUPS) return fail(MRA_EINVAL, "1 .. 4 problems");
  if (!dbg_op(dtype, op)) return fail(MRA_EINVAL, "dtype must be f16 or bf16");
  if (const char* e = dbg_gemm_epi_ok(epi)) return fail(MRA_EINVAL, e);
  if (nprob > 1 && (epi == EPI_RES_OP || epi >= EPI_RES_F32_STAT)) return fail(MRA_EINVAL, "the ViT's epilogues (8, 10 .. 13) take one problem");
  if (!probs) return fail(MRA_EINVAL, "null descriptor array");
  for (int i = 0; i < nprob; ++i)
    if (const char* e = dbg_gemm_prob(probs[i], epi, &ps[i])) return fail(MRA_EINVAL, "problem " + std::to_string(i) + ": " + e);
  pl->cus = cus;
  const int rc = gemm_plan(ps, nprob, epi, *op, pl);
  if (rc) return fail(MRA_EINVAL, rc == -2 ? "the tile has no such epilogue" : "gemm_plan refuses the launch (K % 64, K % 128 on the 128-deep and eight-phase tiles, N % tile, N % 256 == 128 and N >= 384 on the mixed tile, what the tile or the epilogue allows)");
  for (int i = 0; i < nprob; ++i)
    if (const char* e = dbg_gemm_footprint(probs[i], ps[i], *pl, i, epi)) return fail(MRA_EINVAL, "problem " + std::to_string(i) + ": " + e);
  if (epi == EPI_RES_LN)
    for (int i = 0; i < nprob; ++i)
      for (int j = i + 1; j < nprob; ++j) {
        const uintptr_t a0 = (uintptr_t)ps[i].ln_counter, a1 = a0 + 4 * (uintptr_t)((ps[i].M + 63) / 64);
        const uintptr_t b0 = (uintptr_t)ps[j].ln_counter, b1 = b0 + 4 * (uintptr_t)((ps[j].M + 63) / 64);
        if (a0 < b1 && b0 < a1) return fail(MRA_EINVAL, "the counter ranges of two EPI_RES_LN problems overlap");
      }
  return MRA_OK;
}
}

int mra_debug_gemm(const mra_gemm_desc* probs, int32_t nprob, int32_t epilogue, int32_t dtype, void* stream) {
  GemmProb ps[GEMM_MAX_GROUPS];
  static thread_local GemmPlan pl;
  int op;
  if (const int rc = dbg_gemm_prepare(probs, nprob, epilogue, dtype, 0, ps, &pl, &op)) return rc;
  return chk(launch_gemm(ps, nprob, epilogue, op, as_stream(stream)), "debug gemm");
}

int mra_debug_kvgrad_gemm(mra_qformer* h, const void* dkv, size_t dkv_bytes, int32_t enc_items, int32_t kv, float* d_enc, size_t d_enc_bytes,
                          void* stream) {
  if (enc_items < 0 || kv < 0) return fail(MRA_EINVAL, "negative size");
  if (enc_items > 0 && kv > 0 && (!dkv || !d_enc)) return fail(MRA_EINVAL, "null dkv or d_enc");
  if (!h) return fail(MRA_EINVAL, "null handle");
  if (enc_items == 0 || kv == 0) return MRA_OK;
  if (h->ncross <= 0) return fail(MRA_ESTATE, "the handle has no cross-attention layer");
  if ((long long)enc_items * kv > 0x7fffffffLL - 64) return fail(MRA_EINVAL, "enc_items * kv exceeds int32");
  if (!dbg_aligned(dkv, 16) || !dbg_aligned(d_enc, 4)) return fail(MRA_EINVAL, "dkv must be 16-byte aligned (d_enc: 4)");
  const size_t rows = (size_t)enc_items * kv;
  const size_t need_dkv = (size_t)h->ncross * 2 * rows * h->cfg.hidden * 2, need_out = rows * h->cfg.enc_width * 4;
  if (dkv_bytes < need_dkv) return fail(MRA_EINVAL, "dkv_bytes below the cache's footprint of " + std::to_string(need_dkv) + " bytes");
  if (d_enc_bytes < need_out) return fail(MRA_EINVAL, "d_enc_bytes below the output's footprint of " + std::to_string(need_out) + " bytes");
  return chk(launch_kvgrad_gemm(dkv, h->wkv, d_enc, enc_items, kv, h->cfg.heads, h->ncross * 2, h->cfg.enc_width, h->op(), as_stream(stream)),
             "kvgrad gemm");
}

int mra_debug_gemm_plan(const mra_gemm_desc* probs, int32_t nprob, int32_t epilogue, int32_t dtype, int32_t cus, int32_t* out) {
  GemmProb ps[GEMM_MAX_GROUPS];
  static thread_local GemmPlan pl;
  int op;
  if (!out) return fail(MRA_EINVAL, "null out");
  if (cus < 0) return fail(MRA_EINVAL, "negative cus");
  if (const int rc = dbg_gemm_prepare(probs, nprob, epilogue, dtype, cus, ps, &pl, &op)) return rc;
  const int32_t r[7] = {pl.tile, pl.family, pl.threads, pl.lds, pl.grid, pl.persistent, pl.args.total_tiles};
  for (int i = 0; i < 7; ++i) out[i] = r[i];
  return MRA_OK;
}

}
```

mraudio_amd/csrc/mra_handle.h:

```cpp
#pragma once
#include <hip/hip_runtime.h>

#include <algorithm>
#include <cstdlib>
#include <cstring>
#include <map>
#include <string>
#include <vector>

#include "../../include/mra.h"
#include "kernels.h"
#include "mra_common.h"

namespace mra_host {

using namespace mra;

extern thread_local std::string g_err;

inline int fail(int code, const std::string& msg) {
  g_err = msg;
  return code;
}

// ... 36 lines not shown
    T* p = base ? reinterpret_cast<T*>(base + off) : nullptr;
    off += align_up(count * elem);
    return p;
  }
};

inline RowView plain(int rows, int ld) { return RowView{0, rows > 0 ? rows : 1, ld}; }
inline RowView items_view(long long item_stride, int rpi, int ld) { return RowView{item_stride, rpi, ld}; }
inline hipStream_t as_stream(void* s) { return reinterpret_cast<hipStream_t>(s); }
inline int chk(int rc, const char* what) {
  if (rc == 0) return 0;
  return fail(rc == -1 ? MRA_EINVAL : MRA_EHIP, std::string(what) + " failed (rc " + std::to_string(rc) + ")");
}

inline Param* find_param(Registry& reg, const std::string& key, const std::string& layer_prefix, int nlayers) {
  auto it = reg.find(key);
  if (it == reg.end() && key.rfind(layer_prefix, 0) == 0) {
    const size_t p0 = layer_prefix.size(), dot = key.find('.', p0);
    if (dot != std::string::npos) {
      const int li = atoi(key.substr(p0, dot - p0).c_str());
      if (li < 0 || li >= nlayers) { fail(MRA_ENAME, "layer index out of range: " + key); return nullptr; }
      it = reg.find(layer_prefix + std::to_string(li) + key.substr(dot));
    }
  }
  if (it == reg.end()) { fail(MRA_ENAME, "unknown parameter name: " + key); return nullptr; }
  return &it->second;
}
inline int check_numel(const std::string& key, const Param& pr, const int64_t* shape, int ndim) {
  long long numel = 1;
  for (int i = 0; i < ndim; ++i) numel *= shape[i];
  return numel == pr.numel ? 0 : fail(MRA_EINVAL, "parameter " + key + ": expected " + std::to_string(pr.numel) + " elements, got " + std::to_string(numel));
}
inline int count_missing(const Registry& reg) {
  int n = 0;
  for (auto& kv : reg) n += kv.second.required && !kv.second.loaded;
  return n;
}
template <typename H, typename Layout>
int create_arena(H* h, Layout layout, const char* what) {
  HIP_TRY(hipGetDevice(&h->device));
  h->arena_bytes = layout(h, nullptr);
  hipError_t e = hipMalloc((void**)&h->arena, h->arena_bytes);
  if (e != hipSuccess) { h->arena = nullptr; return fail(MRA_ENOMEM, std::string("hipMalloc of the ") + what + " parameter arena: " + hipGetErrorString(e)); }
  layout(h, h->arena);
  e = hipMemsetAsync(h->arena, 0, h->arena_bytes, 0);
  if (e != hipSuccess) { (void)hipFree(h->arena); h->arena = nullptr; return fail(MRA_EHIP, std::string("hipMemsetAsync: ") + hipGetErrorString(e)); }
  return MRA_OK;
}

template <typename T0, typename... Ts, typename F>
auto with_type(int i, F&& f) {
  if constexpr (sizeof...(Ts) == 0) return f(T0{});
  else return i == 0 ? f(T0{}) : with_type<Ts...>(i - 1, f);
}
template <typename F> auto with_op(int op, F&& f) { return with_type<f16, bf16>(op, f); }
template <typename F> auto with_src(int dtype, F&& f) { return with_type<float, f16, bf16>(dtype, f); }
template <typename F> auto with_f32_f16(int dtype, F&& f) { return with_type<float, f16>(dtype, f); }

}

struct mra_qformer {
  mra_cfg cfg;
  int device = 0;
  int ncross = 0;
  char* arena = nullptr;
  size_t arena_bytes = 0;
  std::map<std::string, mra_host::Param> params;
  std::vector<mra_host::LayerW> layers;
  float *word = nullptr, *pos = nullptr, *embg = nullptr, *embb = nullptr, *query = nullptr;
  float *encg = nullptr, *encb = nullptr;
  void* wkv = nullptr;
  float* bkv = nullptr;
  void* wllm = nullptr;
  float* bllm = nullptr;
  char* arena_f = nullptr;
  bool fold_stale = true;
  bool raw_features = true;
  bool inreg_rescale = true;
  int fold_tile = mra::GT_128;
  bool fold_stream = false;
  int cross_mode = 0;
  int chain_ring = 7;
  int train_ring = 4;
  int multi_core = 1;
  int cross_precise = 0;
  float* wk32 = nullptr;
  char* arena_p = nullptr;
  bool precise_stale = true;
  bool cross_auto = false;
  bool auto_stale = true;
  int auto_resolved = -1;
  int auto_probes = 0;
  int auto_tau_milli = 500;
  int* auto_hist = nullptr;
  int* auto_hist_host = nullptr;
  std::vector<float> auto_median;
  hipEvent_t kv_done = nullptr;
  hipEvent_t kv_ev0 = nullptr, kv_ev1 = nullptr;
  char* arena_t = nullptr;
  bool transposes_stale = true;
  mra::TrJob* tr_jobs = nullptr;
  int n_tr_jobs = 0, n_tr_tiles = 0;
  hipStream_t wg_stream = nullptr;
  hipEvent_t wg_ev[32] = {};
  mra::AdamMatJob* adam_jobs = nullptr;
  int n_adam_jobs = 0, n_adam_tiles = 0;
  mra::FlatSeg* adam_segs = nullptr;
  int n_adam_segs = 0;
  mra::FlatSeg* c32_segs = nullptr;
  int n_c32_segs = 0;
  size_t grad_bytes = 0;
  mra::FlatSeg* flat_segs = nullptr;
  int n_flat_segs = 0;
  int op() const { return cfg.op_dtype == MRA_BF16 ? mra::OP_BF16 : mra::OP_F16; }
};

namespace mra_host {
inline int fold_kvp(int kv) { return (std::max((kv + 127) / 128 * 128, (kv + 175) / 176 * 176) + 127) / 128 * 128; }
inline size_t fold_raw_layer_bytes(const mra_qformer* h) { return align_up((size_t)2 * h->cfg.hidden * h->cfg.enc_width * 2 + (size_t)h->cfg.hidden * 4); }
inline size_t fold_raw_off(const mra_qformer* h) { return align_up((size_t)h->ncross * h->cfg.hidden * h->cfg.enc_width * 2); }
inline char* fold_raw_wk(const mra_qformer* h, int ci) { return h->arena_f + fold_raw_off(h) + (size_t)ci * fold_raw_layer_bytes(h); }
inline char* fold_raw_wv(const mra_qformer* h, int ci) { return fold_raw_wk(h, ci) + (size_t)h->cfg.hidden * h->cfg.enc_width * 2; }
inline float* fold_raw_bv(const mra_qformer* h, int ci) { return (float*)(fold_raw_wv(h, ci) + (size_t)h->cfg.hidden * h->cfg.enc_width * 2); }
inline size_t fold_arena_bytes(const mra_qformer* h) { return fold_raw_off(h) + (size_t)h->ncross * fold_raw_layer_bytes(h); }
inline size_t precise_wk_off(const mra_qformer* h) { return align_up((size_t)h->cfg.hidden * 3 * h->cfg.hidden * 2); }
inline size_t precise_layer_bytes(const mra_qformer* h) {
  return precise_wk_off(h) + align_up((size_t)h->cfg.heads * h->cfg.enc_width * 192 * 2);
}
inline AttnArgs self_attn_args(const mra_cfg& c, const void* qkv16, void* ctx16, const long long* mask, int items, int S, float* lse = nullptr) {
  const int H = c.hidden;
  AttnArgs a{};
  a.Q = qkv16; a.K = (const char*)qkv16 + (size_t)H * 2; a.V = (const char*)qkv16 + (size_t)2 * H * 2; a.O = ctx16;
  a.q_item_stride = a.k_item_stride = a.v_item_stride = (long long)S * 3 * H; a.q_ld = a.k_ld = a.v_ld = 3 * H;
  a.k_head_stride = a.v_head_stride = 64; a.o_item_stride = (long long)S * H; a.o_ld = H;
  a.mask = mask; a.mask_ld = S;
  a.items = items; a.heads = c.heads; a.q_rows = S; a.kv_len = S; a.scale = 0.125f; a.nsplit = 1; a.lse = lse;
  return a;
}
inline AttnArgs kv_cross_attn_args(const mra_cfg& c, const void* q16, const char* kv16, int ci, void* ctx16, int items, int kv, int nsplit,
                                   float* part, float* lse = nullptr) {
  const int H = c.hidden, Q = c.n_query;
  const size_t per_sel = (size_t)items * c.heads * kv * 64 * 2;
  AttnArgs a{};
  a.Q = q16; a.K = kv16 + (size_t)(ci * 2 + 0) * per_sel; a.V = kv16 + (size_t)(ci * 2 + 1) * per_sel; a.O = ctx16;
  a.q_item_stride = a.o_item_stride = (long long)Q * H; a.q_ld = a.o_ld = H;
  a.k_item_stride = a.v_item_stride = (long long)c.heads * kv * 64; a.k_head_stride = a.v_head_stride = (long long)kv * 64; a.k_ld = a.v_ld = 64;
  a.items = items; a.heads = c.heads; a.q_rows = Q; a.kv_len = kv; a.scale = 0.125f; a.nsplit = nsplit; a.part = part; a.lse = lse;
  return a;
}
int kv_project(const mra_qformer* h, const void* enc, int N, int kv, void* kv_cache, hipStream_t stream);
}
```

Before: 4896.

## Fuse cross query projection with Q' fold and compute row factors inside P.enc GEMM

Adds a fold_query kernel that runs the cross-attention query projection and the Wk fold (Q') in one launch. The query tile stays in LDS, and the kernel splits E across slices so the grid covers the CUs. It also adds a GEMM mode that computes softmax row factors from the partial statistics inside the P.enc GEMM, replacing the separate rowfactor kernel, plus an option to run the context GEMM on the 64x64 tile with K128. A cross_fuse mask selects these paths and defaults to 1 (query fusion only), removing a launch and the qc16 round trip through global memory. The risk is lower parallelism or a slower hand-written kernel compared with the tuned grouped GEMM.

```diff
diff --git a/include/mra.h b/include/mra.h
--- a/include/mra.h
+++ b/include/mra.h
@@ -218,6 +218,11 @@
                           const float* bias, float eps, void* out, int32_t dtype, void* stream);
 int mra_debug_softmax_rows(const float* S, int64_t ld_s, void* P, int64_t ld_p, int32_t rows, int32_t kv, int32_t kvp, float scale, int32_t dtype,
                            void* stream);
+int mra_debug_fold_query(const void* x, const int64_t* x_view, size_t x_bytes, const void* w_q, size_t w_q_bytes, const float* b_q, size_t b_q_bytes,
+                         const void* w_k, size_t w_k_bytes, void* q_prime, size_t q_prime_bytes, int32_t rows, int32_t H, int32_t E, int32_t Q,
+                         int32_t heads, int32_t dtype, void* stream);
+int64_t mra_debug_fold_query_launches(void);
+int64_t mra_debug_fold_rowfactor_launches(void);
 int mra_debug_fold_rowfactor(const float* stat_m, const float* stat_l, float* factors, int32_t rows, int32_t R, int32_t ntiles, void* P, int64_t ld_p,
                              int32_t tile_cols, int32_t kvp, int32_t* hist, void* stream);
 int mra_debug_softmax_rescale(void* P, int64_t ld_p, const float* stat_m, const float* stat_l, int32_t rows, int32_t ntiles, int32_t tile_cols,
@@ -260,6 +265,7 @@
   float* col_scale; int64_t cs_bs; int32_t col_stats; float cs_eps;
   uint64_t col_scale_bytes;
   void* aux; uint64_t aux_bytes;
+  int32_t k128, ps_stats;
 } mra_gemm_desc;
 int mra_debug_gemm(const mra_gemm_desc* probs, int32_t nprob, int32_t epilogue, int32_t dtype, void* stream);
 int mra_debug_gemm_plan(const mra_gemm_desc* probs, int32_t nprob, int32_t epilogue, int32_t dtype, int32_t cus, int32_t* out);
diff --git a/mraudio_amd/_lib.py b/mraudio_amd/_lib.py
--- a/mraudio_amd/_lib.py
+++ b/mraudio_amd/_lib.py
@@ -57,6 +57,7 @@
         ("col_scale", C.c_void_p), ("cs_bs", C.c_int64), ("col_stats", C.c_int32), ("cs_eps", C.c_float),
         ("col_scale_bytes", C.c_uint64),
         ("aux", C.c_void_p), ("aux_bytes", C.c_uint64),
+        ("k128", C.c_int32), ("ps_stats", C.c_int32),
     ]
 
 
@@ -166,6 +167,10 @@
                                         C.c_void_p, C.c_int32, C.c_void_p]),
     "mra_debug_softmax_rows": (C.c_int, [C.c_void_p, C.c_int64, C.c_void_p, C.c_int64, C.c_int32, C.c_int32, C.c_int32, C.c_float, C.c_int32,
                                          C.c_void_p]),
+    "mra_debug_fold_query": (C.c_int, [C.c_void_p, C.c_void_p, C.c_size_t, C.c_void_p, C.c_size_t, C.c_void_p, C.c_size_t, C.c_void_p, C.c_size_t,
+                                       C.c_void_p, C.c_size_t, C.c_int32, C.c_int32, C.c_int32, C.c_int32, C.c_int32, C.c_int32, C.c_void_p]),
+    "mra_debug_fold_query_launches": (C.c_int64, []),
+    "mra_debug_fold_rowfactor_launches": (C.c_int64, []),
     "mra_debug_fold_rowfactor": (C.c_int, [C.c_void_p, C.c_void_p, C.c_void_p, C.c_int32, C.c_int32, C.c_int32, C.c_void_p, C.c_int64, C.c_int32,
                                            C.c_int32, C.c_void_p, C.c_void_p]),
     "mra_debug_softmax_rescale": (C.c_int, [C.c_void_p, C.c_int64, C.c_void_p, C.c_void_p, C.c_int32, C.c_int32, C.c_int32, C.c_int32, C.c_int32,
diff --git a/mraudio_amd/csrc/fold.hip b/mraudio_amd/csrc/fold.hip
--- a/mraudio_amd/csrc/fold.hip
+++ b/mraudio_amd/csrc/fold.hip
@@ -1,3 +1,5 @@
+#include <atomic>
+
 #include "kernels.h"
 #include "mra_common.h"
 
@@ -187,6 +189,231 @@
   }
 }
 
+struct FoldQueryArgs {
+  const void* X; RowView xv;
+  const void* Wq;
+  const float* bq;
+  const void* Wk;
+  void* QP;
+  int M, H, E, Q, heads, mtiles, blocks_per_slice;
+};
+
+template <typename T>
+__global__ void __launch_bounds__(256) fold_query_kernel(const FoldQueryArgs a) {
+  constexpr int ROWB = 128, TM = 128, NT = 256;
+  constexpr int QH_BYTES = TM * ROWB;
+  constexpr int BUF1 = (64 + TM) * ROWB;
+  constexpr int WK_BYTES = 128 * ROWB, WK_GROUP = 3;
+  constexpr int P1 = QH_BYTES, WK0 = QH_BYTES, OUT = QH_BYTES + WK_GROUP * WK_BYTES;
+  static_assert(2 * BUF1 <= WK_GROUP * WK_BYTES, "phase 1 fits in what phase 2 uses");
+  extern __shared__ __attribute__((aligned(16))) char smem[];
+  using V8 = typename Vec8<T>::type;
+  using V4 = typename Vec4<T>::type;
+  const int tid = threadIdx.x, lane = tid & 63;
+  const int wave = __builtin_amdgcn_readfirstlane(tid >> 6);
+  const int mt = blockIdx.x % a.mtiles, rest = blockIdx.x / a.mtiles;
+  const int head = rest % a.heads, slice = rest / a.heads;
+  const int m0 = mt * TM, M = a.M, H = a.H, E = a.E;
+  const int lm = lane & 15, ln = (lane >> 4) * 4;
+
+  const char* srcW[2];
+  const char* srcX[4];
+#pragma unroll
+  for (int i = 0; i < 2; ++i) {
+    const int q = tid + i * NT;
+    const int row = q >> 3, c = (q & 7) ^ ((row >> 1) & 7);
+    srcW[i] = (const char*)a.Wq + ((long long)(head * 64 + row) * H + c * 8) * 2;
+  }
+#pragma unroll
+  for (int i = 0; i < 4; ++i) {
+    const int q = tid + i * NT;
+    const int row = q >> 3, c = (q & 7) ^ ((row >> 1) & 7);
+    const int m = min(m0 + row, M - 1);
+    const int item = m / a.xv.rpi, r = m - item * a.xv.rpi;
+    srcX[i] = (const char*)a.X + ((long long)item * a.xv.item_stride + (long long)r * a.xv.ld + c * 8) * 2;
+  }
+  const int wave_q0 = wave * 64;
+  auto stage1 = [&](int buf, int kt) {
+    char* base = smem + P1 + buf * BUF1;
+    const long long koff = (long long)kt * ROWB;
+#pragma unroll
+    for (int i = 0; i < 2; ++i) glds16(srcW[i] + koff, base + (wave_q0 + i * NT) * 16);
+#pragma unroll
+    for (int i = 0; i < 4; ++i) glds16(srcX[i] + koff, base + 64 * ROWB + (wave_q0 + i * NT) * 16);
+  };
+  int foff[2];
+#pragma unroll
+  for (int ks = 0; ks < 2; ++ks) foff[ks] = lm * ROWB + (((4 * ks + (lane >> 4)) ^ ((lm >> 1) & 7)) << 4);
+  {
+    const int wn0 = (wave >> 1) * 32, wm0 = (wave & 1) * 64;
+    f32x4 acc[2][4];
+#pragma unroll
+    for (int i = 0; i < 2; ++i)
+#pragma unroll
+      for (int j = 0; j < 4; ++j) acc[i][j] = f32x4{0.f, 0.f, 0.f, 0.f};
+    f32x4 bv[2];
+#pragma unroll
+    for (int i = 0; i < 2; ++i) {
+      bv[i] = f32x4{0.f, 0.f, 0.f, 0.f};
+      if (a.bq) bv[i] = *reinterpret_cast<const f32x4*>(a.bq + head * 64 + wn0 + i * 16 + ln);
+    }
+    const int nk = H / 64;
+    stage1(0, 0);
+    for (int kt = 0; kt < nk; ++kt) {
+      asm volatile("s_waitcnt vmcnt(0)" ::: "memory");
+      __syncthreads();
+      if (kt + 1 < nk) stage1((kt + 1) & 1, kt + 1);
+      const char* wb = smem + P1 + (kt & 1) * BUF1 + wn0 * ROWB;
+      const char* xb = smem + P1 + (kt & 1) * BUF1 + 64 * ROWB + wm0 * ROWB;
+#pragma unroll
+      for (int ks = 0; ks < 2; ++ks) {
+        V8 wa[2], xa[4];
+#pragma unroll
+        for (int i = 0; i < 2; ++i) wa[i] = lds_read8<T>(wb + i * 16 * ROWB + foff[ks]);
+#pragma unroll
+        for (int j = 0; j < 4; ++j) xa[j] = lds_read8<T>(xb + j * 16 * ROWB + foff[ks]);
+#pragma unroll
+        for (int i = 0; i < 2; ++i)
+#pragma unroll
+          for (int j = 0; j < 4; ++j) acc[i][j] = mfma16<T>(wa[i], xa[j], acc[i][j]);
+      }
+    }
+#pragma unroll
+    for (int i = 0; i < 2; ++i) {
+      const int d = wn0 + i * 16 + ln;
+#pragma unroll
+      for (int j = 0; j < 4; ++j) {
+        const int ml = wm0 + j * 16 + lm;
+        const f32x4 v = acc[i][j] + bv[i];
+        V4 o;
+#pragma unroll
+        for (int e = 0; e < 4; ++e) o[e] = from_f32<T>(v[e]);
+        *reinterpret_cast<V4*>(smem + ml * ROWB + (((d >> 3) ^ ((ml >> 1) & 7)) << 4) + (d & 4) * 2) = o;
+      }
+    }
+  }
+  __syncthreads();
+
+  const int nblk = (E + 127) / 128;
+  const int b0 = slice * a.blocks_per_slice, b1 = min(b0 + a.blocks_per_slice, nblk);
+  if (b0 >= b1) return;
+  const char* wk = (const char*)a.Wk + (long long)head * E * 64 * 2;
+  int wrow[4], wchunk[4];
+#pragma unroll
+  for (int i = 0; i < 4; ++i) {
+    const int q = tid + i * NT;
+    wrow[i] = q >> 3;
+    wchunk[i] = ((q & 7) ^ ((wrow[i] >> 1) & 7)) * 16;
+  }
+  const int wm0 = wave * 32;
+  V8 xa[2][2];
+#pragma unroll
+  for (int ks = 0; ks < 2; ++ks)
+#pragma unroll
+    for (int j = 0; j < 2; ++j) xa[ks][j] = lds_read8<T>(smem + (wm0 + j * 16) * ROWB + foff[ks]);
+  long long rowoff[4];
+  bool live[4];
+#pragma unroll
+  for (int u = 0; u < 4; ++u) {
+    const int row = (lane >> 3) + u * 8;
+    const int m = m0 + wm0 + row;
+    live[u] = m < M;
+    const int mc = live[u] ? m : M - 1;
+    const int item = mc / a.Q, qq = mc - item * a.Q;
+    rowoff[u] = (((long long)item * a.heads + head) * a.Q + qq) * E + ((lane & 7) ^ (row & 7)) * 8;
+  }
+  char* st = smem + OUT + wave * (32 * 128);
+  for (int g0 = b0; g0 < b1; g0 += WK_GROUP) {
+    const int g1 = min(g0 + WK_GROUP, b1);
+    if (g0 > b0) __syncthreads();
+    for (int blk = g0; blk < g1; ++blk) {
+      char* base = smem + WK0 + (blk - g0) * WK_BYTES;
+#pragma unroll
+      for (int i = 0; i < 4; ++i) glds16(wk + (long long)min(blk * 128 + wrow[i], E - 1) * ROWB + wchunk[i], base + (wave_q0 + i * NT) * 16);
+    }
+    asm volatile("s_waitcnt vmcnt(0)" ::: "memory");
+    __syncthreads();
+    for (int hb = 2 * g0; hb < 2 * g1; ++hb) {
+      const int nb = hb * 64;
+      if (nb >= E) break;
+      f32x4 acc[4][2];
+#pragma unroll
+      for (int i = 0; i < 4; ++i)
+#pragma unroll
+        for (int j = 0; j < 2; ++j) acc[i][j] = f32x4{0.f, 0.f, 0.f, 0.f};
+      const char* wb = smem + WK0 + (hb - 2 * g0) * (64 * ROWB);
+#pragma unroll
+      for (int ks = 0; ks < 2; ++ks) {
+        V8 wa[4];
+#pragma unroll
+        for (int i = 0; i < 4; ++i) wa[i] = lds_read8<T>(wb + i * 16 * ROWB + foff[ks]);
+#pragma unroll
+        for (int i = 0; i < 4; ++i)
+#pragma unroll
+          for (int j = 0; j < 2; ++j) acc[i][j] = mfma16<T>(wa[i], xa[ks][j], acc[i][j]);
+      }
+#pragma unroll
+      for (int i = 0; i < 4; ++i) {
+        const int d = i * 16 + ln;
+#pragma unroll
+        for (int j = 0; j < 2; ++j) {
+          const int ml = j * 16 + lm;
+          V4 o;
+#pragma unroll
+          for (int e = 0; e < 4; ++e) o[e] = from_f32<T>(acc[i][j][e]);
+          *reinterpret_cast<V4*>(st + ml * 128 + (((d >> 3) ^ (ml & 7)) << 4) + ((d >> 2) & 1) * 8) = o;
+        }
+      }
+      asm volatile("s_waitcnt lgkmcnt(0)" ::: "memory");
+#pragma unroll
+      for (int u = 0; u < 4; ++u) {
+        const V8 val = *reinterpret_cast<const V8*>(st + (lane + u * 64) * 16);
+        if (live[u]) *reinterpret_cast<V8*>((T*)a.QP + nb + rowoff[u]) = val;
+      }
+      asm volatile("s_waitcnt lgkmcnt(0)" ::: "memory");
+    }
+  }
+}
+
+std::atomic<long long> g_fold_query_launches, g_fold_rowfactor_launches;
+
+int device_cus() {
+  static std::atomic<int> memo[64];
+  int dev = 0;
+  if (hipGetDevice(&dev) != hipSuccess || dev < 0 || dev >= 64) return 256;
+  int cus = memo[dev].load(std::memory_order_relaxed);
+  if (!cus) {
+    if (hipDeviceGetAttribute(&cus, hipDeviceAttributeMultiprocessorCount, dev) != hipSuccess || cus <= 0) cus = 256;
+    memo[dev].store(cus, std::memory_order_relaxed);
+  }
+  return cus;
+}
+
+}
+
+long long fold_rowfactor_launch_count() { return g_fold_rowfactor_launches.load(std::memory_order_relaxed); }
+long long fold_query_launch_count() { return g_fold_query_launches.load(std::memory_order_relaxed); }
+
+int launch_fold_query(const void* X, RowView xv, const void* Wq, const float* bq, const void* Wk, void* QP, int M, int H, int E, int Q, int heads,
+                      int op_dtype, hipStream_t stream) {
+  if (M <= 0) return 0;
+  if (!X || !Wq || !Wk || !QP || H < 64 || H % 64 || E < 64 || E % 64 || Q <= 0 || M % Q || heads <= 0 || xv.rpi <= 0 || (xv.ld & 7) || (xv.item_stride & 7)) return -1;
+  FoldQueryArgs a{X, xv, Wq, bq, Wk, QP, M, H, E, Q, heads, (M + 127) / 128, 0};
+  const int nblk = (E + 127) / 128, pairs = a.mtiles * heads, cus = device_cus();
+  int slices = (cus + pairs - 1) / pairs;
+  if (slices > nblk) slices = nblk;
+  a.blocks_per_slice = (nblk + slices - 1) / slices;
+  if (a.blocks_per_slice > 3) a.blocks_per_slice = a.blocks_per_slice / 3 * 3;
+  slices = (nblk + a.blocks_per_slice - 1) / a.blocks_per_slice;
+  constexpr size_t lds = 128 * 128 + 3 * 128 * 128 + 4 * 32 * 128;
+  const void* fn = op_dtype == OP_F16 ? (const void*)fold_query_kernel<f16> : (const void*)fold_query_kernel<bf16>;
+  if (!ensure_lds(fn, lds)) return -3;
+  const dim3 grid(pairs * slices);
+  if (op_dtype == OP_F16) hipLaunchKernelGGL(fold_query_kernel<f16>, grid, dim3(256), lds, stream, a);
+  else hipLaunchKernelGGL(fold_query_kernel<bf16>, grid, dim3(256), lds, stream, a);
+  if (hipGetLastError() != hipSuccess) return -4;
+  g_fold_query_launches.fetch_add(1, std::memory_order_relaxed);
+  return 0;
 }
 
 int launch_softmax_rows(const float* S, long long ld_s, void* P, long long ld_p, int rows, int kv, int kvp, float scale, int op_dtype,
@@ -217,7 +444,9 @@
   else
     hipLaunchKernelGGL(fold_rowfactor_kernel<false>, dim3((rows + 3) / 4), dim3(256), 0, stream, stat_m, stat_l, factors, rows, R, ntiles,
                        (unsigned short*)P, ld_p, tile_cols, kvp, (int*)nullptr);
-  return hipGetLastError() == hipSuccess ? 0 : -4;
+  if (hipGetLastError() != hipSuccess) return -4;
+  g_fold_rowfactor_launches.fetch_add(1, std::memory_order_relaxed);
+  return 0;
 }
 
 int launch_softmax_rescale(void* P, long long ld_p, const float* stat_m, const float* stat_l, int rows, int ntiles, int tile_cols, int kvp,
diff --git a/mraudio_amd/csrc/gemm.hip b/mraudio_amd/csrc/gemm.hip
--- a/mraudio_amd/csrc/gemm.hip
+++ b/mraudio_amd/csrc/gemm.hip
@@ -581,13 +581,15 @@
   }
 }
 
-template <typename T, int EPI, bool NODMA = false, int TN = 256, int TM = 256, int WGM = 4, bool NTW = false, bool WKM = false, bool PSC = false, int CS = 0>
+template <typename T, int EPI, bool NODMA = false, int TN = 256, int TM = 256, int WGM = 4, bool NTW = false, bool WKM = false, bool PSC = false, int CS = 0, bool PST = false>
 __global__ void __launch_bounds__(768) gemm_ws_kernel(const GemmArgs args) {
   constexpr int BK = 64, ROWB = BK * 2;
   constexpr int WGN = 8 / WGM, WTN = TN / WGN, WTM = TM / WGM, FN = WTN / 16, FM = WTM / 16;
   constexpr int BUF = (TN + TM) * ROWB;
   constexpr int PS_TILE = 176, GT_OFF = 2 * BUF, GT_SLICE = 2048;
   static_assert(!PSC || (TM <= 512 && PS_TILE % 8 == 0), "factor slices hold 512 rows; an 8-k fragment piece never straddles a tile");
+  static_assert(!PST || (PSC && TM % 64 == 0), "statistics-fed factors: a mode of PSC; whole waves of rows");
+  constexpr int ST_OFF = GT_OFF + 4 * GT_SLICE;
   constexpr int NCHUNK = (TN + TM) * 8, NLD = (NCHUNK + 255) / 256;
   constexpr bool STAGED = (EPI == EPI_OP || EPI == EPI_GELU_OP || EPI == EPI_KV || EPI == EPI_RES_OP) && TN % 64 == 0;
   static_assert(WTN % 16 == 0 && WTM % 16 == 0 && TN % 16 == 0 && NCHUNK % 64 == 0, "tile must split over the waves; whole waves per DMA piece");
@@ -601,6 +603,29 @@
   const GemmProb& P = pick_tile<TN, TM>(args, n0, m0);
   const int K = P.K, M = P.M;
   const int nk = K / BK;
+  auto row_stats = [&]() {
+    if constexpr (PST) {
+      float* mrow = reinterpret_cast<float*>(smem + ST_OFF);
+      float* rinv = mrow + 512;
+      const int nt = P.ps_ntiles;
+      for (int r = wave; r < TM; r += 12) {
+        const long long row = (long long)P.batch_row0 + min(m0 + r, M - 1);
+        const float* sm = P.stat_m + row * nt;
+        const float* sl = P.stat_l + row * nt;
+        float m = -3.0e38f;
+        for (int t = lane; t < nt; t += 64) m = fmaxf(m, sm[t]);
+        m = wave_max(m);
+        float l = 0.f;
+        for (int t = lane; t < nt; t += 64) l += __builtin_amdgcn_exp2f(sm[t] - m) * sl[t];
+        l = wave_sum(l);
+        const float inv = 1.0f / l;
+        if (lane == 0) { mrow[r] = m; rinv[r] = inv; }
+      }
+      asm volatile("s_waitcnt lgkmcnt(0)" ::: "memory");
+      __builtin_amdgcn_s_barrier();
+      asm volatile("" ::: "memory");
+    }
+  };
 
   if (wave >= 8) {
     const int lt = tid - 512;
@@ -647,6 +672,21 @@
       if constexpr (PSC) {
         if (wave != 8) return;
         const int t_hi = (kt * BK + BK - 1) / PS_TILE;
+        if constexpr (PST) {
+          const float* mrow = reinterpret_cast<const float*>(smem + ST_OFF);
+          const float* rinv = mrow + 512;
+          for (; gt_next <= t_hi; ++gt_next) {
+            const int tt = min(gt_next, P.ps_ntiles - 1);
+            float* dg = reinterpret_cast<float*>(smem + GT_OFF + (gt_next & 3) * GT_SLICE);
+#pragma unroll
+            for (int k = 0; k < TM / 64; ++k) {
+              const int r = lane + 64 * k;
+              const float smt = P.stat_m[((long long)P.batch_row0 + min(m0 + r, M - 1)) * P.ps_ntiles + tt];
+              dg[r] = __builtin_amdgcn_exp2f(smt - mrow[r]) * rinv[r];
+            }
+          }
+          return;
+        }
         for (; gt_next <= t_hi; ++gt_next) {
           const char* sg = (const char*)(P.pscale + (long long)min(gt_next, P.ps_ntiles - 1) * 512) + lane * 16;
           char* dg = smem + GT_OFF + (gt_next & 3) * GT_SLICE;
@@ -667,9 +707,22 @@
 #pragma unroll
     for (int i = 0; i < NWS; ++i) cmean[i] = cm2[i] = 0.f;
     stage(0, 0);
+    row_stats();
     stage_factors(0);
     for (int kt = 0; kt < nk; ++kt) {
       asm volatile("s_waitcnt vmcnt(0)" ::: "memory");
+      if constexpr (PST) {
+        const int pad0 = P.ps_ntiles * PS_TILE;
+        if (kt * BK + BK > pad0) {
+#pragma unroll
+          for (int i = 0; i < NLD; ++i) {
+            const int q = lt + i * 256;
+            if (q >= TN * 8 && q < NCHUNK && kt * BK + (((q & 7) ^ ((q >> 4) & 7)) << 3) >= pad0)
+              *reinterpret_cast<i32x4*>(smem + (kt & 1) * BUF + q * 16) = i32x4{0, 0, 0, 0};
+          }
+        }
+        asm volatile("s_waitcnt lgkmcnt(0)" ::: "memory");
+      }
       __builtin_amdgcn_s_barrier();
       asm volatile("" ::: "memory");
       if (kt + 1 < nk && !(NODMA && kt >= 1)) { stage((kt + 1) & 1, kt + 1); stage_factors(kt + 1); }
@@ -759,6 +812,7 @@
       for (int j = 0; j < FM; ++j) acc[i][j] = f32x4{0.f, 0.f, 0.f, 0.f};
   }
 
+  row_stats();
   for (int kt = 0; kt < nk; ++kt) {
     __builtin_amdgcn_s_barrier();
     asm volatile("" ::: "memory");
@@ -1544,6 +1598,7 @@
     case GF_WS_128x384: return with_epi(EpiWs128{}, epi, [&](auto e) { return go(gemm_ws_kernel<T, e(), false, 128, 384>); });
     case GF_WS_176x384:
       if (a.p[0].w_ld > 0) {
+        if (a.p[0].ps_stats) return go(gemm_ws_kernel<T, EPI_OP, false, 176, 384, 8, true, true, true, 0, true>);
         if (a.p[0].pscale) return go(gemm_ws_kernel<T, EPI_OP, false, 176, 384, 8, true, true, true>);
         return go(gemm_ws_kernel<T, EPI_OP, false, 176, 384, 8, true, true>);
       }
@@ -1600,7 +1655,7 @@
   bool even = true, deep = true;
   for (int g = 0; g < ngroups; ++g) {
     even = even && probs[g].K % 128 == 0;
-    deep = deep && probs[g].K % 128 == 0 && probs[g].K >= 2048;
+    deep = deep && probs[g].K % 128 == 0 && (probs[g].K >= 2048 || probs[g].k128);
   }
   if (tile == GT_256) {
     if (g_variant == 1) return GF_V1_256;
@@ -1657,6 +1712,7 @@
   if (p.w_ld && (!(d.allow & T_WLD) || epi != EPI_OP || (p.w_ld & 7) || p.k_rows <= 0 || p.N % d.tn)) return false;
   if (p.w_kwrap && (!(d.allow & T_KWRAP) || p.w_kwrap < 0 || p.w_ld || 2 * p.w_kwrap * 64 != p.K)) return false;
   if (p.col_scale && (epi != EPI_SOFTPART || family != GF_WS_176x384 || p.w_ld || ngroups != 1)) return false;
+  if (p.ps_stats && (p.pscale || !p.stat_m || !p.stat_l || !p.w_ld || p.M > d.tm || p.ps_ntiles <= 0 || p.K > p.ps_ntiles * d.tn + 4 * d.tn || ngroups != 1)) return false;
   if (p.pscale && (!p.w_ld || p.M > d.tm || p.ps_ntiles <= 0 || p.K > p.ps_ntiles * d.tn + 4 * d.tn)) return false;
   return true;
 }
@@ -1715,7 +1771,7 @@
   a.dbg = g_dbg;
   a.order = g_order ? g_order : probs[0].order;
   pl.threads = d.threads;
-  pl.lds = d.lds + (a.p[0].pscale ? 4 * 2048 : 0);
+  pl.lds = d.lds + (a.p[0].pscale || a.p[0].ps_stats ? 4 * 2048 : 0) + (a.p[0].ps_stats ? 2 * 2048 : 0);
   pl.persistent = pl.family == GF_P8_256 && a.p[0].persist && ngroups == 1 && a.p[0].batch <= 1 && has_epi(epi_mask(EpiP8Persist{}), epi) && pl.cus >= 8 && tiles > pl.cus;
   pl.grid = pl.persistent ? pl.cus & ~7 : tiles;
   return 0;
diff --git a/mraudio_amd/csrc/kernels.h b/mraudio_amd/csrc/kernels.h
--- a/mraudio_amd/csrc/kernels.h
+++ b/mraudio_amd/csrc/kernels.h
@@ -84,6 +84,8 @@
   int tile_begin;
   int mtiles, ntiles;
   int batch_row0;
+  int k128;
+  int ps_stats;
 };
 
 constexpr int GEMM_MAX_GROUPS = 4;
@@ -204,6 +206,10 @@
                         hipStream_t stream);
 int launch_fold_rowfactor(const float* stat_m, const float* stat_l, float* factors, int rows, int R, int ntiles, void* P, long long ld_p, int tile_cols,
                           int kvp, hipStream_t stream, int* hist = nullptr);
+int launch_fold_query(const void* X, RowView xv, const void* Wq, const float* bq, const void* Wk, void* QP, int M, int H, int E, int Q, int heads,
+                      int op_dtype, hipStream_t stream);
+long long fold_rowfactor_launch_count();
+long long fold_query_launch_count();
 int launch_softmax_rescale(void* P, long long ld_p, const float* stat_m, const float* stat_l, int rows, int ntiles, int tile_cols, int kvp,
                            int op_dtype, hipStream_t stream, int* hist = nullptr);
 int launch_transpose_pad(const void* src, void* dst, int R, int C, int ld_d, long long src_bs, long long dst_bs, int batch, int op_dtype,
diff --git a/mraudio_amd/csrc/mra_abi.hip b/mraudio_amd/csrc/mra_abi.hip
--- a/mraudio_amd/csrc/mra_abi.hip
+++ b/mraudio_amd/csrc/mra_abi.hip
@@ -137,6 +137,9 @@
   bool softpart;
   bool inreg;
   bool raw;
+  bool fuse_query;
+  bool stat_factors;
+  bool ctx_64;
   int scores_tile, penc_tile;
 };
 
@@ -154,7 +157,11 @@
   x.inreg = (h->inreg_rescale || probe) && x.softpart && x.kmajor;
   x.scores_tile = R == 384 ? GT_WS_176x384 : GT_128;
   x.penc_tile = x.kmajor ? GT_WS_176x384 : (R == 384 ? h->fold_tile : GT_128);
-  x.raw = raw && x.form == CrossPlan::FOLD && x.softpart && x.kmajor && x.inreg && !precise && !probe;
+  const bool default_fold = x.form == CrossPlan::FOLD && x.softpart && x.kmajor && x.inreg && !precise && !probe;
+  x.raw = raw && default_fold;
+  x.fuse_query = (h->cross_fuse & 1) && default_fold && c.hidden == c.heads * 64 && c.enc_width % 64 == 0;
+  x.stat_factors = (h->cross_fuse & 2) && default_fold;
+  x.ctx_64 = (h->cross_fuse & 4) && default_fold && c.enc_width % 128 == 0;
   return x;
 }
 
@@ -293,7 +300,7 @@
     return rc ? chk(rc, "cross attention") : MRA_OK;
   }
   const bool timed = ci == 0 && h->kv_ev0 && h->kv_ev1;
-  if (timed) (void)hipEventRecord(h->kv_ev0, stream);
+  if (timed && !x.fuse_query) (void)hipEventRecord(h->kv_ev0, stream);
   int* hist = x.probe ? h->auto_hist + (size_t)ci * 256 : nullptr;
   GemmProb d{};
   if (x.precise) {
@@ -307,7 +314,7 @@
     if (rc) return chk(rc, "fold q' gemm (split precision)");
     rc = launch_split_rows(w.qp32, plain(N * R, E), N * R, E, E, 2, w.qp16, op, stream);
     if (rc) return chk(rc, "split q'");
-  } else {
+  } else if (!x.fuse_query) {
     d.A = w.qc16; d.a = qc_rows; d.a_bs = 64;
     d.W = x.raw ? fold_raw_wk(h, ci) : h->arena_f + (size_t)ci * H * E * esz; d.w_bs = (long long)E * 64;
     d.C = w.qp16; d.c = items_view((long long)R * E, Q, E); d.c_bs_bytes = (long long)Q * E * esz;
@@ -342,7 +349,8 @@
       }
       rc = launch_gemm(&sc, 1, EPI_SOFTPART, op, stream);
       if (rc) return chk(rc, "fold scores gemm (softmax partials)");
-      if (x.inreg) {
+      if (x.stat_factors) {
+      } else if (x.inreg) {
         rc = launch_fold_rowfactor(sc.stat_m, sc.stat_l, w.gfac, N * R, R, ntiles, w.p16, kvp, 176, kvp, stream, hist);
         if (rc) return chk(rc, "fold row factors");
       } else {
@@ -366,7 +374,8 @@
     pv.C = w.u16; pv.c = plain(R, E); pv.c_bs_bytes = (long long)R * E * esz;
     pv.M = R; pv.N = E; pv.K = kvp; pv.batch = N;
     pv.tile_cfg = x.penc_tile;
-    if (x.inreg) { pv.pscale = w.gfac; pv.ps_ntiles = ntiles; }
+    if (x.stat_factors) { pv.stat_m = sc.stat_m; pv.stat_l = sc.stat_l; pv.ps_stats = 1; pv.ps_ntiles = ntiles; }
+    else if (x.inreg) { pv.pscale = w.gfac; pv.ps_ntiles = ntiles; }
     rc = launch_gemm(&pv, 1, EPI_OP, op, stream);
     if (rc) return chk(rc, "fold p.enc gemm");
   }
@@ -377,6 +386,7 @@
   if (x.raw) { cx.W = fold_raw_wv(h, ci); cx.bias = fold_raw_bv(h, ci); }
   cx.C = w.ctx16; cx.c = qc_rows; cx.c_bs_bytes = 64 * esz;
   cx.M = N * Q; cx.N = 64; cx.K = E; cx.batch = c.heads; cx.tile_cfg = E % 128 == 0 && N * Q >= 512 ? GT_K128_64x128 : GT_64;
+  if (x.ctx_64 && cx.tile_cfg == GT_K128_64x128) { cx.tile_cfg = GT_64; cx.k128 = 1; }
   rc = launch_gemm(&cx, 1, EPI_OP, op, stream);
   if (rc) return chk(rc, "fold context gemm");
   if (timed) (void)hipEventRecord(h->kv_ev1, stream);
@@ -718,13 +728,24 @@
         rc = launch_gemm(&p, 1, EPI_F32, op, stream);
       } else {
         GemmProb p[2] = {};
-        for (int l = 0; l < nl; ++l) {
-          p[l].A = lanes[l].w.hB16; p[l].a = q_view;
-          p[l].W = Lw[l]->wcq; p[l].bias = Lw[l]->bcq;
-          p[l].C = lanes[l].w.qc16; p[l].c = qc_rows;
-          p[l].M = N * Q; p[l].N = H; p[l].K = H;
+        int ng = 0;
+        rc = 0;
+        for (int l = 0; l < nl && !rc; ++l) {
+          const Lane& x = lanes[l];
+          if (x.plan.fuse_query) {
+            const int ci = Lw[l]->cross_index, E = x.h->cfg.enc_width;
+            const void* wk = x.plan.raw ? fold_raw_wk(x.h, ci) : x.h->arena_f + (size_t)ci * H * E * esz;
+            if (ci == 0 && x.h->kv_ev0 && x.h->kv_ev1) (void)hipEventRecord(x.h->kv_ev0, stream);
+            rc = launch_fold_query(x.w.hB16, q_view, Lw[l]->wcq, Lw[l]->bcq, wk, x.w.qp16, N * Q, H, E, Q, c.heads, op, stream);
+            continue;
+          }
+          p[ng].A = x.w.hB16; p[ng].a = q_view;
+          p[ng].W = Lw[l]->wcq; p[ng].bias = Lw[l]->bcq;
+          p[ng].C = x.w.qc16; p[ng].c = qc_rows;
+          p[ng].M = N * Q; p[ng].N = H; p[ng].K = H;
+          ++ng;
         }
-        rc = launch_gemm(p, nl, EPI_OP, op, stream);
+        if (!rc && ng) rc = launch_gemm(p, ng, EPI_OP, op, stream);
       }
       if (rc) return chk(rc, "cross q gemm");
       for (int l = 0; l < nl; ++l)
@@ -1245,6 +1266,12 @@
     h->chain_ring = value;
     return MRA_OK;
   }
+  if (key == "cross_fuse") {
+    if (value < 0 || (value & ~7))
+      return fail(MRA_EINVAL, "cross_fuse is a mask of 1 (query projection and Q' in one launch), 2 (row factors inside the P.enc launch) and 4 (context GEMM on the 64 x 64 tile)");
+    h->cross_fuse = value;
+    return MRA_OK;
+  }
   if (key == "multi_core") {
     if (value < 0 || value > 1) return fail(MRA_EINVAL, "multi_core is 0 (attn_kernel with kv_share) or 1 (shared-stream core)");
     h->multi_core = value;
@@ -1675,6 +1702,15 @@
   p.batch = d.batch; p.a_bs = d.a_bs; p.w_bs = d.w_bs; p.c_bs_bytes = d.c_bs_bytes; p.bias_bs = d.bias_bs;
   p.n_ragged = d.n_ragged; p.w_ld = d.w_ld; p.k_rows = d.k_rows; p.w_kwrap = d.w_kwrap;
   p.tile_cfg = d.tile_cfg; p.persist = d.persist;
+  if (d.k128 < 0 || d.k128 > 1 || d.ps_stats < 0 || d.ps_stats > 1) return "k128 and ps_stats are 0 or 1";
+  if (d.ps_stats) {
+    if (epi != EPI_OP || d.pscale || !d.w_ld) return "ps_stats goes with EPI_OP over K-major weights (w_ld) and without pscale";
+    if (!d.stat_m || !d.stat_l || !dbg_aligned(d.stat_m, 4) || !dbg_aligned(d.stat_l, 4)) return "ps_stats needs stat_m and stat_l (4-byte aligned)";
+    if (d.M > 384 || d.ps_ntiles <= 0) return "ps_stats needs M <= 384 (one row tile) and ps_ntiles > 0";
+    p.stat_m = d.stat_m; p.stat_l = d.stat_l; p.ps_stats = 1; p.ps_ntiles = d.ps_ntiles;
+  }
+  if (d.k128 && (d.tile_cfg != GT_64 || d.K % 128)) return "k128 goes with tile_cfg GT_64 and K % 128 == 0";
+  p.k128 = d.k128;
   if (epi == EPI_KV) {
     if (d.kv_tokens <= 0 || d.kv_items <= 0 || d.kv_heads <= 0 || d.kv_heads > 1024) return "EPI_KV needs kv_tokens, kv_items and kv_heads > 0";
     if (d.N % (d.kv_heads * 64)) return "EPI_KV: N must be a multiple of kv_heads * 64";
@@ -1790,6 +1826,10 @@
   if (epi == EPI_SOFTPART) {
     const u128 n = (u128)nb * (u128)d.M * (u128)ntiles;
     if (!dbg_fits(n, 4, 0, d.stat_m_bytes) || !dbg_fits(n, 4, 0, d.stat_l_bytes)) return "stat_m / stat_l: batch * M * ntiles floats leave their sizes";
+  }
+  if (p.ps_stats) {
+    const u128 n = (u128)nb * (u128)d.M * (u128)d.ps_ntiles;
+    if (!dbg_fits(n, 4, 0, d.stat_m_bytes) || !dbg_fits(n, 4, 0, d.stat_l_bytes)) return "ps_stats: batch * M * ps_ntiles floats of stat_m / stat_l leave their sizes";
   }
   if (p.pscale && !dbg_fits((u128)nb * (u128)d.ps_ntiles * 512, 4, 0, d.pscale_bytes)) return "pscale: batch * ps_ntiles * 512 floats leave pscale_bytes";
   if (p.col_scale && !dbg_fits((u128)d.N + (u128)(nb - 1) * (u128)d.cs_bs, 4, 0, d.col_scale_bytes)) return "col_scale: N floats and the batch stride leave col_scale_bytes";
@@ -1863,4 +1903,29 @@
   return MRA_OK;
 }
 
-}
+int mra_debug_fold_query(const void* x, const int64_t* x_view, size_t x_bytes, const void* w_q, size_t w_q_bytes, const float* b_q, size_t b_q_bytes,
+                         const void* w_k, size_t w_k_bytes, void* q_prime, size_t q_prime_bytes, int32_t rows, int32_t H, int32_t E, int32_t Q,
+                         int32_t heads, int32_t dtype, void* stream) {
+  int op;
+  if (rows < 0) return fail(MRA_EINVAL, "negative rows");
+  if (!dbg_op(dtype, &op)) return fail(MRA_EINVAL, "dtype must be f16 or bf16");
+  if (H < 64 || H % 64 || E < 64 || E % 64 || Q <= 0 || heads <= 0 || heads > 1024 || rows % Q)
+    return fail(MRA_EINVAL, "need H and E positive multiples of 64, Q > 0, 0 < heads <= 1024, rows % Q == 0");
+  RowView xv;
+  if (!dbg_view8(x_view, &xv) || xv.ld < H) return fail(MRA_EINVAL, "bad row view of x: strides multiples of 8, row stride >= H");
+  if (rows == 0) return MRA_OK;
+  if (!x || !w_q || !w_k || !q_prime) return fail(MRA_EINVAL, "null argument");
+  if (!dbg_aligned(x, 16) || !dbg_aligned(w_q, 16) || !dbg_aligned(w_k, 16) || !dbg_aligned(q_prime, 16) || !dbg_aligned(b_q, 16))
+    return fail(MRA_EINVAL, "misaligned buffer");
+  if (!dbg_fits(dbg_extent(xv, rows, H), 2, 0, x_bytes)) return fail(MRA_EINVAL, "x: the view and H leave x_bytes");
+  if (!dbg_fits((u128)heads * 64 * (u128)H, 2, 0, w_q_bytes)) return fail(MRA_EINVAL, "w_q: heads * 64 rows of H leave w_q_bytes");
+  if (b_q && !dbg_fits((u128)heads * 64, 4, 0, b_q_bytes)) return fail(MRA_EINVAL, "b_q: heads * 64 floats leave b_q_bytes");
+  if (!dbg_fits((u128)heads * (u128)E * 64, 2, 0, w_k_bytes)) return fail(MRA_EINVAL, "w_k: heads blocks of [E][64] leave w_k_bytes");
+  if (!dbg_fits((u128)rows * (u128)heads * (u128)E, 2, 0, q_prime_bytes)) return fail(MRA_EINVAL, "q_prime: rows * heads * E elements leave q_prime_bytes");
+  return chk(launch_fold_query(x, xv, w_q, b_q, w_k, q_prime, rows, H, E, Q, heads, op, as_stream(stream)), "fold_query");
+}
+
+int64_t mra_debug_fold_query_launches(void) { return fold_query_launch_count(); }
+int64_t mra_debug_fold_rowfactor_launches(void) { return fold_rowfactor_launch_count(); }
+
+}
diff --git a/mraudio_amd/csrc/mra_handle.h b/mraudio_amd/csrc/mra_handle.h
--- a/mraudio_amd/csrc/mra_handle.h
+++ b/mraudio_amd/csrc/mra_handle.h
@@ -142,6 +142,7 @@
   int cross_mode = 0;
   int chain_ring = 7;
   int train_ring = 4;
+  int cross_fuse = 1;
   int multi_core = 1;
   int cross_precise = 0;
   float* wk32 = nullptr;
```

New measurement: 4957 (median of 6 runs). 1.2% higher.
